# ebu/libear

Measured on AMD Instinct MI355X. Metric: Msamples/s, higher is better.
Workload: dtype f32 io / f16x2-split MFMA, f32 accumulate

## Files before the change

include/earhip.h:

```cpp
#ifndef EARHIP_H
#define EARHIP_H

#include <stddef.h>
#include <stdint.h>

#ifdef __cplusplus
extern "C" {
#endif

#define EARHIP_VERSION 100

#define EARHIP_OK 0
#define EARHIP_INVALID_ARGUMENT 1
#define EARHIP_INTERNAL_ERROR 2
#define EARHIP_DEVICE_ERROR 3
#define EARHIP_NOT_IMPLEMENTED 4
#define EARHIP_UNKNOWN_LAYOUT 5
#define EARHIP_ADM_ERROR 6

int earhip_version(void);
const char *earhip_last_error(void);
int earhip_device_count(int *count);

typedef struct earhip_ctx earhip_ctx;
// ... 97 lines not shown
                          double *elevation, int *is_lfe);
int earhip_layout_channel_ranges(const char *layout, int index, double azimuth_range[2],
                                 double elevation_range[2]);
int earhip_design_decorrelators_for_layout(const char *layout, int without_lfe, float *out);

typedef struct earhip_panner earhip_panner;
int earhip_panner_create(earhip_ctx *ctx, const char *layout, earhip_panner **out);
int earhip_panner_create_positions(earhip_ctx *ctx, const char *layout, int n_channels,
                                   const double *azimuth, const double *elevation,
                                   earhip_panner **out);
int earhip_panner_destroy(earhip_panner *p);
int earhip_panner_num_channels(const earhip_panner *p, int *n_channels);
int earhip_panner_calculate(earhip_panner *p, size_t npos, const double *azimuth,
                            const double *elevation, const double *distance, const double *gain,
                            const double *diffuse, float *direct, float *diffuse_out);
int earhip_panner_calculate_device(earhip_panner *p, size_t npos, const double *azimuth,
                                   const double *elevation, const double *distance,
                                   const double *gain, const double *diffuse, float *direct,
                                   float *diffuse_out);

int earhip_panner_calculate_extent(earhip_panner *p, size_t npos, const double *azimuth,
                                   const double *elevation, const double *distance,
                                   const double *width, const double *height, const double *depth,
                                   const double *gain, const double *diffuse, float *direct,
                                   float *diffuse_out);
int earhip_panner_calculate_extent_device(earhip_panner *p, size_t npos, const double *azimuth,
                                          const double *elevation, const double *distance,
                                          const double *width, const double *height,
                                          const double *depth, const double *gain,
                                          const double *diffuse, float *direct, float *diffuse_out);
int earhip_panner_missed(earhip_panner *p, unsigned *count);

int earhip_hoa_decode_matrix(earhip_ctx *ctx, const char *layout, int n_coef, const int *orders,
                             const int *degrees, const char *normalization, float *out);
int earhip_hoa_decode_matrix_positions(earhip_ctx *ctx, const char *layout, int n_channels,
                                       const double *azimuth, const double *elevation, int n_coef,
                                       const int *orders, const int *degrees,
                                       const char *normalization, float *out);

typedef struct earhip_direct_speakers earhip_direct_speakers;

typedef struct earhip_ds_metadata {
  int n_labels;
  const char *const *labels;
  int cartesian;
  double azimuth, elevation, distance;
  int has_azimuth_min, has_azimuth_max, has_elevation_min, has_elevation_max, has_distance_min,
      has_distance_max;
  double azimuth_min, azimuth_max, elevation_min, elevation_max, distance_min, distance_max;
  int screen_edge_lock_horizontal, screen_edge_lock_vertical;
  int has_low_pass, has_high_pass;
  double low_pass, high_pass;
  const char *audio_pack_format_id;
} earhip_ds_metadata;

int earhip_direct_speakers_create(earhip_ctx *ctx, const char *layout, int n_subst,
                                  const char *const *from, const char *const *to,
                                  earhip_direct_speakers **out);
int earhip_direct_speakers_create_positions(earhip_ctx *ctx, const char *layout, int n_channels,
                                            const double *azimuth, const double *elevation,
                                            int n_subst, const char *const *from,
                                            const char *const *to, earhip_direct_speakers **out);
int earhip_direct_speakers_destroy(earhip_direct_speakers *ds);
int earhip_direct_speakers_num_channels(const earhip_direct_speakers *ds, int *n_channels);
int earhip_direct_speakers_calculate(earhip_direct_speakers *ds, size_t n,
                                     const earhip_ds_metadata *md, float *gains,
                                     int *warnings_out);
int earhip_direct_speakers_missed(earhip_direct_speakers *ds, unsigned *count);

int earhip_conversion_to_polar(size_t n, const double *x, const double *y, const double *z,
                               const double *width, const double *height, const double *depth,
                               double *azimuth, double *elevation, double *distance,
                               double *width_out, double *height_out, double *depth_out);
int earhip_conversion_to_cartesian(size_t n, const double *azimuth, const double *elevation,
                                   const double *distance, const double *width,
                                   const double *height, const double *depth, double *x, double *y,
                                   double *z, double *width_out, double *height_out,
                                   double *depth_out);
int earhip_conversion_to_polar_device(earhip_ctx *ctx, size_t n, const double *x, const double *y,
                                      const double *z, const double *width, const double *height,
                                      const double *depth, double *azimuth, double *elevation,
                                      double *distance, double *width_out, double *height_out,
                                      double *depth_out, int *status);
int earhip_conversion_to_cartesian_device(earhip_ctx *ctx, size_t n, const double *azimuth,
                                          const double *elevation, const double *distance,
                                          const double *width, const double *height,
                                          const double *depth, double *x, double *y, double *z,
                                          double *width_out, double *height_out, double *depth_out,
                                          int *status);

typedef struct earhip_render earhip_render;

typedef struct earhip_render_config {
  int n_objects;
  int n_out;
  int block_size;
  int n_buses;
  const float *decorrelators;
  int n_taps;
  int delay;
  int max_blocks;
} earhip_render_config;

int earhip_render_create(earhip_ctx *ctx, const earhip_render_config *cfg,
                         earhip_render **out);
int earhip_render_destroy(earhip_render *r);
int earhip_render_set_object_points(earhip_render *r, int object, int npoints,
                                    const int64_t *times, const float *direct,
                                    const float *diffuse);
int earhip_render_commit(earhip_render *r);
int earhip_render_scratch_regrows(const earhip_render *r, long *count);
int earhip_render_reset(earhip_render *r, int64_t sample_time);
int earhip_render_process_device(earhip_render *r, size_t nblocks,
                                 const float *in_dev, size_t in_stride,
                                 float *out_dev, size_t out_stride);
int earhip_render_process(earhip_render *r, size_t nblocks, const float *const *in,
                          float *const *out);
typedef enum {
  EARHIP_PCM_S16 = 1,
  EARHIP_PCM_S24 = 2,
  EARHIP_PCM_S32 = 3,
  EARHIP_PCM_F32 = 4
} earhip_pcm_format;
int earhip_render_process_frames(earhip_render *r, size_t nblocks, const void *frames,
                                 earhip_pcm_format fmt, int frame_channels, int first_channel,
                                 float *const *out, int out_interleaved);
int earhip_render_process_frames_device(earhip_render *r, size_t nblocks, const void *frames_dev,
                                        earhip_pcm_format fmt, int frame_channels, int first_channel,
                                        float *out_dev, size_t out_stride, int out_interleaved);
typedef struct earhip_pcm_out {
  earhip_pcm_format format;
  int dither;
  uint32_t seed;
} earhip_pcm_out;
int earhip_render_process_frames_pcm(earhip_render *r, size_t nblocks, const void *frames,
                                     earhip_pcm_format fmt, int frame_channels, int first_channel,
                                     void *out_frames, const earhip_pcm_out *out);
int earhip_render_process_frames_pcm_device(earhip_render *r, size_t nblocks, const void *frames_dev,
                                            earhip_pcm_format fmt, int frame_channels,
                                            int first_channel, void *out_dev, size_t out_frame_bytes,
                                            size_t out_first_byte, const earhip_pcm_out *out);
int earhip_render_output_levels(earhip_render *r, float *peak, uint64_t *clipped, int reset);
int earhip_render_enable_timing(earhip_render *r, int enable);
int earhip_render_get_timing(earhip_render *r, double out[6]);
int earhip_render_gain_kernel(const earhip_render *r, int *kind);
int earhip_render_hinge_standby(earhip_render *r, int *standby);
int earhip_render_hinge_robust(earhip_render *r, int *robust);
int earhip_render_wide_form(earhip_render *r, int *wide);
int earhip_render_last_plan(const earhip_render *r, int out[4]);
int earhip_render_last_list_layout(const earhip_render *r, int *paired);
int earhip_render_last_tail_blocks(const earhip_render *r, int *blocks);
int earhip_render_last_host_chunks(const earhip_render *r, int *chunks);
int earhip_render_scratch_bytes(const earhip_render *r, size_t *bytes);

typedef struct earhip_comm earhip_comm;
int earhip_comm_unique_id(void *id128);
int earhip_comm_create(earhip_ctx *ctx, int rank, int world, const void *id128, earhip_comm **out);
int earhip_comm_destroy(earhip_comm *comm);
int earhip_comm_channel_range(int n_out, int rank, int world, int *padded_rows, int *lo, int *hi);
int earhip_render_exchange_device(earhip_comm *comm, int slot, const float *partial_dev,
                                  float *owned_dev, size_t rows_per_rank, size_t row_stride);
int earhip_comm_gather_device(earhip_comm *comm, int slot, const float *owned_dev, float *full_dev,
                              size_t rows_per_rank, size_t row_stride, int root);
int earhip_comm_wait(earhip_comm *comm, int slot);
int earhip_comm_last_exchange_ms(earhip_comm *comm, int slot, double *ms);
int earhip_comm_info(earhip_comm *comm, int info[4]);
int earhip_comm_link_probe(earhip_comm *comm, size_t bytes, int shift, int reps, double *GBps);

#ifdef __cplusplus
}
#endif
#endif
```

libear_amd/capi.py:

```python
import ctypes as C
import os

import numpy as np

from .build import lib_path

f32p = C.POINTER(C.c_float)
i64p = C.POINTER(C.c_int64)
pp_f32 = C.POINTER(f32p)

OK, INVALID_ARGUMENT, INTERNAL_ERROR, DEVICE_ERROR, NOT_IMPLEMENTED, UNKNOWN_LAYOUT, ADM_ERROR = 0, 1, 2, 3, 4, 5, 6


class EarHipError(Exception):
    def __init__(self, code, msg):
        super().__init__(msg)
        self.code = code


class InvalidArgument(EarHipError, ValueError):
    """maps to ear::invalid_argument"""


class InternalError(EarHipError, RuntimeError):
# ... 686 lines not shown
        self.h = C.c_void_p()
        check(load().earhip_render_create(ctx.h, C.byref(cfg), C.byref(self.h)))

    def set_object_points(self, obj, times, direct, diffuse=None):
        t = np.ascontiguousarray(times, dtype=np.int64)
        d = _f32(direct).reshape(len(t), self.N)
        f = _f32(diffuse).reshape(len(t), self.N) if diffuse is not None else None
        check(load().earhip_render_set_object_points(self.h, obj, len(t), _ptr(t, i64p), _ptr(d),
                                                     _ptr(f) if f is not None else None))

    def commit(self):
        check(load().earhip_render_commit(self.h))

    def reset(self, sample_time=0):
        check(load().earhip_render_reset(self.h, C.c_int64(sample_time)))

    def process(self, x):
        x = _f32(x).reshape(self.M, -1)
        nblocks = x.shape[1] // self.B
        assert nblocks * self.B == x.shape[1]
        out = np.empty((self.N, x.shape[1]), np.float32)
        check(load().earhip_render_process(self.h, C.c_size_t(nblocks), _chan_ptrs(x), _chan_ptrs(out)))
        return out

    def process_into(self, x, out):
        assert x.dtype == np.float32 and out.dtype == np.float32 and x.flags["C_CONTIGUOUS"] and out.flags["C_CONTIGUOUS"]
        nblocks = x.shape[1] // self.B
        assert x.shape == (self.M, nblocks * self.B) and out.shape == (self.N, nblocks * self.B)
        check(load().earhip_render_process(self.h, C.c_size_t(nblocks), _chan_ptrs(x), _chan_ptrs(out)))
        return out

    def process_device(self, nblocks, in_ptr, in_stride, out_ptr, out_stride):
        check(load().earhip_render_process_device(self.h, C.c_size_t(nblocks), C.c_void_p(in_ptr),
                                                  C.c_size_t(in_stride), C.c_void_p(out_ptr),
                                                  C.c_size_t(out_stride)))

    def _frames_shape(self, x, fmt):
        code, dtype, cols = pcm_format(fmt)
        assert x.dtype == dtype and x.ndim == 2 and x.flags["C_CONTIGUOUS"], (x.dtype, dtype, x.shape)
        assert x.shape[1] % cols == 0
        frames, channels = x.shape[0], x.shape[1] // cols
        nblocks = frames // self.B
        assert nblocks * self.B == frames, "frames must be whole blocks"
        return code, nblocks, channels

    def process_frames(self, x, fmt, first_channel=0, interleaved_out=False):
        x = np.ascontiguousarray(x)
        frames = x.shape[0]
        out = np.empty((frames, self.N) if interleaved_out else (self.N, frames), np.float32)
        return self.process_frames_into(x, out, fmt, first_channel, interleaved_out)

    def process_frames_into(self, x, out, fmt, first_channel=0, interleaved_out=False):
        code, nblocks, channels = self._frames_shape(x, fmt)
        frames = nblocks * self.B
        assert out.dtype == np.float32 and out.flags["C_CONTIGUOUS"]
        assert out.shape == ((frames, self.N) if interleaved_out else (self.N, frames)), out.shape
        ptrs = (f32p * 1)(_ptr(out)) if interleaved_out else _chan_ptrs(out)
        check(load().earhip_render_process_frames(self.h, C.c_size_t(nblocks), C.c_void_p(x.ctypes.data), C.c_int(code),
                                                  C.c_int(channels), C.c_int(first_channel), ptrs, int(bool(interleaved_out))))
        return out

    def process_frames_device(self, nblocks, frames_ptr, fmt, frame_channels, first_channel, out_ptr, out_stride,
                              interleaved_out=False):
        code = pcm_format(fmt)[0] if isinstance(fmt, str) else int(fmt)
        check(load().earhip_render_process_frames_device(self.h, C.c_size_t(nblocks), C.c_void_p(frames_ptr), C.c_int(code),
                                                         C.c_int(frame_channels), C.c_int(first_channel), C.c_void_p(out_ptr),
                                                         C.c_size_t(out_stride), int(bool(interleaved_out))))

    def process_frames_pcm(self, x, fmt, first_channel=0, out_fmt="s16", dither=False, seed=0):
        x = np.ascontiguousarray(x)
        _, dtype, cols = pcm_format(out_fmt)
        out = np.empty((x.shape[0], self.N * cols), dtype)
        return self.process_frames_pcm_into(x, out, fmt, first_channel, out_fmt, dither, seed)

    def process_frames_pcm_into(self, x, out, fmt, first_channel=0, out_fmt="s16", dither=False, seed=0):
        code, nblocks, channels = self._frames_shape(x, fmt)
        ocode, dtype, cols = pcm_format(out_fmt)
        assert out.dtype == dtype and out.flags["C_CONTIGUOUS"] and out.shape == (nblocks * self.B, self.N * cols), out.shape
        spec = PcmOut(ocode, int(dither), int(seed) & 0xFFFFFFFF)
        check(load().earhip_render_process_frames_pcm(self.h, C.c_size_t(nblocks), C.c_void_p(x.ctypes.data), C.c_int(code),
                                                      C.c_int(channels), C.c_int(first_channel), C.c_void_p(out.ctypes.data),
                                                      C.byref(spec)))
        return out

    def process_frames_pcm_device(self, nblocks, frames_ptr, fmt, frame_channels, first_channel, out_ptr, out_frame_bytes,
                                  out_first_byte=0, out_fmt="s16", dither=False, seed=0):
        code = pcm_format(fmt)[0] if isinstance(fmt, str) else int(fmt)
        ocode = pcm_format(out_fmt)[0] if isinstance(out_fmt, str) else int(out_fmt)
        spec = PcmOut(ocode, int(dither), int(seed) & 0xFFFFFFFF)
        check(load().earhip_render_process_frames_pcm_device(self.h, C.c_size_t(nblocks), C.c_void_p(frames_ptr), C.c_int(code),
                                                             C.c_int(frame_channels), C.c_int(first_channel), C.c_void_p(out_ptr),
                                                             C.c_size_t(out_frame_bytes), C.c_size_t(out_first_byte),
                                                             C.byref(spec)))

    def output_levels(self, reset=False):
        peak, clipped = np.zeros(self.N, np.float32), np.zeros(self.N, np.uint64)
        check(load().earhip_render_output_levels(self.h, _ptr(peak), C.c_void_p(clipped.ctypes.data), int(bool(reset))))
        return peak, clipped

    def enable_timing(self, on=True):
        check(load().earhip_render_enable_timing(self.h, int(on)))

    def get_timing(self):
        out = (C.c_double * 6)()
        check(load().earhip_render_get_timing(self.h, out))
        return {"gain_mix_ms": out[0], "gain_mix_launches": out[1], "decor_ms": out[2],
                "decor_launches": out[3], "prep_ms": out[4], "prep_launches": out[5]}

    def gain_kernel(self):
        kind = C.c_int(-1)
        check(load().earhip_render_gain_kernel(self.h, C.byref(kind)))
        return kind.value

    def hinge_standby(self):
        flag = C.c_int(0)
        check(load().earhip_render_hinge_standby(self.h, C.byref(flag)))
        return bool(flag.value)

    def hinge_robust(self):
        flag = C.c_int(0)
        check(load().earhip_render_hinge_robust(self.h, C.byref(flag)))
        return bool(flag.value)

    def wide_form(self):
        flag = C.c_int(1)
        check(load().earhip_render_wide_form(self.h, C.byref(flag)))
        return None if flag.value < 0 else bool(flag.value)

    def scratch_bytes(self):
        v = C.c_size_t(0)
        check(load().earhip_render_scratch_bytes(self.h, C.byref(v)))
        return v.value

    def scratch_regrows(self):
        v = C.c_long(0)
        check(load().earhip_render_scratch_regrows(self.h, C.byref(v)))
        return v.value

    def last_tail_blocks(self):
        v = C.c_int(0)
        check(load().earhip_render_last_tail_blocks(self.h, C.byref(v)))
        return v.value

    def last_host_chunks(self):
        v = C.c_int(0)
        check(load().earhip_render_last_host_chunks(self.h, C.byref(v)))
        return v.value

    def last_list_layout(self):
        v = C.c_int(0)
        check(load().earhip_render_last_list_layout(self.h, C.byref(v)))
        return None if v.value < 0 else bool(v.value)

    def last_plan(self):
        out = (C.c_int * 4)()
        check(load().earhip_render_last_plan(self.h, out))
        return {"kernel": out[0], "tile": out[1], "ntiles": out[2], "gsplit": out[3]}

    def close(self):
        if self.h:
            load().earhip_render_destroy(self.h)
            self.h = C.c_void_p()
```

libear_amd/csrc/api_core.hip:

```cpp
#include <cctype>
#include <cerrno>
#include <cmath>
#include <cstdlib>
#include <string>
#include <memory>
#include <mutex>

#include "common.h"
#include "curves.h"
#include "gain_kernels.h"
#include "gain_mfma.h"
#include "gain_h2.h"
#include "gain_h2_t1.h"
#include "gain_p2.h"
#include "gain_hg.h"
#include "gain_f32g.h"

namespace earhip {

static_assert(kSplitTile == 256, "MixLaunch::tile() and tiles_aligned(256, ...) assume the 4-wave tile");

static thread_local std::string g_last_error;
void set_last_error(const std::string &msg) { g_last_error = msg; }

size_t mix_lds_bytes(const ColumnPlan &cp, const MixLaunch &ml) {
  if (ml.wsplit <= 1 || ml.split || ml.pieces || ml.hinge) return 0;
  if (ml.mfma) return (size_t)cp.mgroups * ml.tpw * cp.nct * 16 * ml.tile() * sizeof(float);
  return (size_t)cp.ngroups * cp.nout * ml.tile() * sizeof(float);
}

template <int NCT, int NRT>
static void launch_mfma_t(const GainMixParams &P, dim3 grid, dim3 block, size_t lds,
                          hipStream_t s) {
  hipLaunchKernelGGL((k_gain_mix_mfma<NCT, NRT>), grid, block, lds, s, P);
}

template <int NOUT, int SPL, bool STRICT>
static void launch_mix_t(const GainMixParams &P, dim3 grid, dim3 block, size_t lds,
                         hipStream_t s) {
  hipLaunchKernelGGL((k_gain_mix<NOUT, SPL, STRICT>), grid, block, lds, s, P);
}

void launch_gain_mix(earhip_ctx *ctx, const CurveSet &cs, const MixLaunch &ml, bool strict,
                     int64_t t_call, int nsamples, const float *in_dev, size_t in_stride,
                     float *out_dev, size_t out_stride, size_t part_stride, SegDesc *desc,
                     hipEvent_t *ev) {
  const ColumnPlan &cp = cs.plan();
  const PointStore ps = cs.device();
  const int M = cs.M();
  const bool slots = ml.mfma && !ml.split && !ml.pieces && !ml.hinge && !ml.f32grid;
  if (slots && M > kMaxSlotObjects) fail_internal("slot lists address objects with 16 bits");
  if (ev) EARHIP_HIP(hipEventRecord(ev[0], ctx->stream));
  const bool fused_prep = slots && (size_t)ps.npoints <= (size_t)8 * M;
  LevelProbe probe;
  unsigned *level_cur = nullptr, *level_next = nullptr;
  unsigned *wide_cur = nullptr, *wide_next = nullptr;
  unsigned *gate = nullptr;
  ctx->last_gate_idx = -1;
  ctx->last_wide_idx = -1;
  unsigned *const record = ctx->record_slot;
  ctx->record_slot = nullptr;
  const bool hg_robust = ml.hinge && ctx->get(OPT_HG_ROBUST, 1) != 0;
  if ((ml.split || ml.pieces || ml.hinge) && ctx->x_scale_auto && in_stride % 4 == 0 && ((uintptr_t)in_dev & 15) == 0) {
    if (!ctx->level.p) ctx->level.alloc_zero(4, ctx->stream), ctx->lazy_allocs++;
    level_cur = ctx->level.p + ctx->level_idx;
    level_next = ctx->level.p + (ctx->level_idx ^ 1);
    if ((size_t)ml.ntiles * ml.gsplit >= 2 * (size_t)ctx->num_cus) wide_cur = ctx->level.p + 2 + ctx->level_idx;
    wide_next = ctx->level.p + 2 + (ctx->level_idx ^ 1);
    gate = ctx->level.p + 2 + ctx->level_idx;
    ctx->last_gate_idx = ml.hinge ? ctx->level_idx : -1;
    ctx->last_hinge_robust = hg_robust;
    ctx->last_wide_idx = wide_cur ? ctx->level_idx : -1;
    ctx->level_idx ^= 1;
    if (ctx->obj_level_cap < M) {
      EARHIP_HIP(hipStreamSynchronize(ctx->stream));
      ctx->obj_level_cap = M + M / 2 + 64;
      ctx->obj_level.alloc_zero(2 * (size_t)ctx->obj_level_cap, ctx->stream);
      ctx->lazy_allocs++;
    }
    probe.obj_level = ctx->obj_level.p;
    probe.level = level_cur;
    const int probe_runs = [&] {
      const int v = ctx->get(OPT_PROBE_RUNS);
      return v >= 1 && v <= 64 && (v & (v - 1)) == 0 ? v : 16;
    }();
    hipLaunchKernelGGL(k_level_probe, dim3((M + kProbeObjects - 1) / kProbeObjects), dim3(64 * kProbeObjects), 0, ctx->stream, in_dev,
                       in_stride, nsamples, M, level_cur, ctx->obj_level.p, ctx->obj_level_cap, probe_runs);
  }
  PieceLists pl;
  pl.pieces = reinterpret_cast<Piece *>(desc);
  pl.M = M;
  pl.paired = ml.paired ? 1 : 0;
  const int ptile = ml.hinge ? 64 * ml.pw : ml.tile();
  const int pnt = ml.hinge ? (nsamples + ptile - 1) / ptile : ml.ntiles;
  pl.slots = cs.piece_cap(ptile, ml.paired);
  pl.count = reinterpret_cast<int *>(pl.pieces + (size_t)pl.cap() * pnt);
  pl.ovf = pl.count + (size_t)8 * pnt;
  unsigned *slow_cur = nullptr, *slow_next = nullptr;
  if (ml.split) {
    if (ctx->tile_slow_cap < (size_t)ml.ntiles) {
      EARHIP_HIP(hipStreamSynchronize(ctx->stream));
      ctx->tile_slow_cap = std::max<size_t>(2 * (size_t)ml.ntiles, 1024);
      ctx->tile_slow.alloc_zero(2 * ctx->tile_slow_cap, ctx->stream);
      ctx->lazy_allocs++;
    }
    slow_cur = ctx->tile_slow.p + (size_t)ctx->tile_slow_idx * ctx->tile_slow_cap;
    slow_next = ctx->tile_slow.p + (size_t)(ctx->tile_slow_idx ^ 1) * ctx->tile_slow_cap;
    ctx->tile_slow_idx ^= 1;
  }
  HingeLists hl = hinge_lists(desc, M, ml.ntiles);
  if (ml.hinge) {
    if (M > kMaxHingeCached || (ml.tile() != 256 && ml.tile() != 512)) fail_internal("hinge lists: object count or tile out of range");
    if (!ps.kink_row0) fail_internal("hinge kernel: the curve set has no kink rows");
    if (!hinge_addressable(M, in_stride, nsamples, (size_t)ps.kink_row0 + ps.rows, ps.row)) fail_internal("hinge kernel: buffers beyond its 32-bit offsets");
    unsigned *obj_lv = probe.obj_level;
    if (gate) hipLaunchKernelGGL(k_hinge_gate, dim3((M + 255) / 256), dim3(256), 0, ctx->stream, obj_lv, ctx->obj_level_cap, M, level_cur, gate, wide_cur != nullptr, hg_robust);
    int tpw = 1;
    const size_t cached_max = std::min((size_t)kMaxHingeCached, ctx->hinge_build_lds / sizeof(HingeCached));
    if ((size_t)M > cached_max) fail_internal("hinge lists: more objects than the builder's LDS holds on this device");
    while (tpw < 8 && ml.ntiles / (2 * tpw) >= ctx->num_cus && (size_t)M * (2 * tpw) <= cached_max) tpw *= 2;
    if (ctx->has(OPT_HBUILD_TPW)) {
      const int v = ctx->get(OPT_HBUILD_TPW);
      if ((v == 1 || v == 2 || v == 4 || v == 8) && (size_t)M * v <= cached_max) tpw = v;
    }
    const HingeCached *stage = nullptr;
    if (ctx->get(OPT_BUILD_2K, 0) != 0) {
      HingeCached *st = reinterpret_cast<HingeCached *>(desc) + hinge_units((size_t)M, (size_t)ml.ntiles);
      stage = st;
      const dim3 cgrid((ml.ntiles + 63) / 64, (M + kClassifyObjects - 1) / kClassifyObjects);
      if (ml.tile() == 256)
        hipLaunchKernelGGL((k_hinge_classify<4>), cgrid, dim3(64 * kClassifyObjects), 0, ctx->stream, ps, M, ml.ntiles, t_call, t_call + nsamples, st,
                           obj_lv, level_cur, hg_robust ? nullptr : gate, hg_robust ? gate : nullptr);
      else
        hipLaunchKernelGGL((k_hinge_classify<8>), cgrid, dim3(64 * kClassifyObjects), 0, ctx->stream, ps, M, ml.ntiles, t_call, t_call + nsamples, st,
                           obj_lv, level_cur, hg_robust ? nullptr : gate, hg_robust ? gate : nullptr);
      if (!ctx->has(OPT_HBUILD_TPW)) {
        tpw = 1;
        while (tpw < 8 && ml.ntiles / (2 * tpw) >= 2 * ctx->num_cus) tpw *= 2;
      }
    }
    const dim3 bgrid((ml.ntiles + tpw - 1) / tpw);
    const size_t lds = stage ? 0 : sizeof(HingeCached) * (size_t)M * tpw;
#define EARHIP_HBUILD_ONE(T_, NW_)                                                                                    \
  hipLaunchKernelGGL((k_hinge_build<T_, NW_>), bgrid, dim3(kHingeBuildThreads), lds, ctx->stream, ps, M, ml.ntiles, t_call, \
                     t_call + nsamples, hl, obj_lv, level_cur, hg_robust ? nullptr : gate, hg_robust ? gate : nullptr, stage);
#define EARHIP_HBUILD_CASE(T_)                                                                                        \
  if (tpw == T_) {                                                                                                    \
    if (ml.tile() == 256) EARHIP_HBUILD_ONE(T_, 4)                                                                    \
    else EARHIP_HBUILD_ONE(T_, 8)                                                                                     \
  }
    EARHIP_HBUILD_CASE(1) EARHIP_HBUILD_CASE(2) EARHIP_HBUILD_CASE(4) EARHIP_HBUILD_CASE(8)
#undef EARHIP_HBUILD_CASE
#undef EARHIP_HBUILD_ONE
  }
  const bool one_pass = ml.pieces || ml.hinge;
  if (ml.pieces || (ml.hinge && gate && !hg_robust)) {
    if (M > kMaxPieceObjects || ptile > kPieceMaxTile) fail_internal("piece lists: object index or tile out of range");
    unsigned *obj_lv = probe.obj_level;
    int tpw = 1;
    while (tpw < 8 && pnt / (2 * tpw) >= ctx->num_cus) tpw *= 2;
    if (ctx->has(OPT_BUILD_TPW)) {
      const int v = ctx->get(OPT_BUILD_TPW);
      if (v == 1 || v == 2 || v == 4 || v == 8) tpw = v;
    }
    const dim3 bgrid((pnt + tpw - 1) / tpw);
    PairRec *stage = nullptr;
    if (ctx->has(OPT_BUILD_2K) ? ctx->get(OPT_BUILD_2K) != 0 : ml.paired) {
      stage = reinterpret_cast<PairRec *>(desc) + piece_units((size_t)M, (size_t)pnt, (size_t)pl.slots);
      hipLaunchKernelGGL(k_piece_classify, dim3((pnt + 63) / 64, (M + kClassifyObjects - 1) / kClassifyObjects), dim3(64 * kClassifyObjects), 0,
                         ctx->stream, ps, M, pnt, ptile, t_call, t_call + nsamples, pl.paired, stage, obj_lv, level_cur,
                         ml.hinge ? gate : nullptr);
    }
#define EARHIP_BUILD_CASE(T_)                                                                                          \
  if (tpw == T_)                                                                                                       \
    hipLaunchKernelGGL(k_piece_build<T_>, bgrid, dim3(kBuildThreads), 0, ctx->stream, ps, M, pnt, ptile, t_call, \
                       t_call + nsamples, pl, obj_lv, level_cur, ml.hinge ? gate : nullptr, ctx->obj_level_cap, wide_cur, stage);
    EARHIP_BUILD_CASE(1) EARHIP_BUILD_CASE(2) EARHIP_BUILD_CASE(4) EARHIP_BUILD_CASE(8)
#undef EARHIP_BUILD_CASE
  }
  if (!fused_prep && !one_pass) {
    const dim3 ogrid((M + 15) / 16);
    QuietMark qm;
    if (probe.obj_level) {
      qm.obj_level = probe.obj_level, qm.cap = ctx->obj_level_cap, qm.level = level_cur;
      qm.wide = ml.split ? wide_cur : nullptr;
    }
    if (ml.ntiles >= 2048)
      hipLaunchKernelGGL(k_seg_prep<4>, dim3((ml.ntiles + 63) / 64, ogrid.x), dim3(256), 0, ctx->stream, ps, M,
                         ml.ntiles, ml.tile(), t_call, t_call + nsamples, desc, qm, slow_cur);
    else
      hipLaunchKernelGGL(k_seg_prep<2>, dim3((ml.ntiles + 31) / 32, ogrid.x), dim3(256), 0, ctx->stream, ps, M,
                         ml.ntiles, ml.tile(), t_call, t_call + nsamples, desc, qm, slow_cur);
  }
  SlotLists sl;
  sl.slots = reinterpret_cast<Slot *>(desc + (size_t)M * ml.ntiles);
  sl.count = reinterpret_cast<int *>(sl.slots + (size_t)kTileSlots * M * ml.ntiles);
  sl.ovf = sl.count + (size_t)4 * ml.ntiles;
  sl.M = M;
  if (slots)
    hipLaunchKernelGGL(k_slot_list, dim3(ml.ntiles), dim3(256), 0, ctx->stream, ps, M, ml.tile(),
                       t_call, t_call + nsamples, fused_prep ? nullptr : desc, sl);
  if (ev) EARHIP_HIP(hipEventRecord(ev[1], ctx->stream));
  GainMixParams P;
  P.mode_word = gate;
  P.record = gate ? record : nullptr;
  P.sl = sl;
  P.in = in_dev;
  P.in_stride = in_stride;
  P.out = out_dev;
  P.out_stride = out_stride;
  P.part_stride = part_stride;
  P.desc = desc;
  P.ps = ps;
  P.t_call = t_call;
  P.nsamples = nsamples;
  P.ntiles = ml.ntiles;
  P.M = M;
  P.ncols = cs.ncols();
  P.ngroups = ml.mfma ? cp.mgroups : cp.ngroups;
  P.wsplit = ml.wsplit;
  P.tiles_per_wg = ml.mfma ? ml.tpw : 1;
  P.vec_ok = (in_stride % 4 == 0 && out_stride % 4 == 0 && part_stride % 4 == 0 &&
              ((uintptr_t)in_dev & 15) == 0 && ((uintptr_t)out_dev & 15) == 0)
                 ? 1
                 : 0;
  const dim3 grid(ml.mfma ? (ml.ntiles + ml.tpw - 1) / ml.tpw : ml.ntiles, ml.gsplit,
                  ml.mfma ? cp.mnz : cp.nz);
  const dim3 block(64 * P.ngroups * P.tiles_per_wg * ml.wsplit);
  const size_t lds = mix_lds_bytes(cp, ml);
  if (ev) EARHIP_HIP(hipEventRecord(ev[2], ctx->stream));
  bool launched = false;
  if (ml.hinge) {
    const dim3 bgrid(ml.ntiles, ml.gsplit, cp.mnz * cp.mgroups);
    const float xs = std::ldexp(1.0f, ctx->x_scale_log2);
    const float *gs = cs.column_scales();
#define EARHIP_HG_LAUNCH(NCT_, NW_)                                                                                  \
  hipLaunchKernelGGL((k_gain_mix_hg<NCT_, NW_>), bgrid, dim3(64 * NW_), 0, ctx->stream, P, hl, xs, gs, level_cur,     \
                     level_next, wide_cur, wide_next, hg_robust ? nullptr : gate, hg_robust ? gate : nullptr);
#define EARHIP_HG_CASE(NCT_)                                                                                          \
  if (cp.nct == NCT_) {                                                                                               \
    if (ml.tile() == 256) EARHIP_HG_LAUNCH(NCT_, 4)                                                                   \
    else EARHIP_HG_LAUNCH(NCT_, 8)                                                                                    \
  }
    EARHIP_HG_CASE(1) EARHIP_HG_CASE(2) EARHIP_HG_CASE(3)
#undef EARHIP_HG_CASE
#undef EARHIP_HG_LAUNCH
    launched = true;
  }
  if (ml.pieces || (ml.hinge && gate && !hg_robust)) {
    int wgs = std::max(8, (ctx->num_cus * (ml.pw == 4 ? 2 : 1) / std::max(1, ml.gsplit * cp.mnz * cp.mgroups)) & ~7);
    if (ctx->has(OPT_P2_WGS)) wgs = ctx->get(OPT_P2_WGS) > 0 ? ctx->get(OPT_P2_WGS) : pnt;
    if (!p2_persistent(cp.nct, ml.pw, ml.paired)) wgs = pnt;
    const dim3 bgrid(std::min(pnt, wgs), ml.gsplit, cp.mnz * cp.mgroups);
    const float xs = std::ldexp(1.0f, ctx->x_scale_log2);
    const float *gs = cs.column_scales();
#define EARHIP_P2_LAUNCH(NCT_, NW_, PR_)                                                                             \
  hipLaunchKernelGGL((k_gain_mix_p2<NCT_, NW_, PR_>), bgrid, dim3(64 * NW_), 0, ctx->stream, P, pl, xs, gs,         \
                     level_cur, level_next, wide_cur, wide_next, ml.hinge ? gate : nullptr, pnt);
#define EARHIP_P2_CASE(NCT_, PR_)                                                                                   \
  if (cp.nct == NCT_ && ml.paired == PR_) {                                                                         \
    if (ml.pw == 4) EARHIP_P2_LAUNCH(NCT_, 4, PR_)                                                                  \
    else EARHIP_P2_LAUNCH(NCT_, 8, PR_)                                                                             \
  }
    EARHIP_P2_CASE(1, false) EARHIP_P2_CASE(2, false) EARHIP_P2_CASE(3, false)
    EARHIP_P2_CASE(1, true) EARHIP_P2_CASE(2, true) EARHIP_P2_CASE(3, true)
#undef EARHIP_P2_CASE
#undef EARHIP_P2_LAUNCH
    launched = true;
  }
  if (ml.f32grid) {
    if (nsamples % kF32GridTile != 0) fail_internal("f32 grid kernel: the call is not whole tiles");
    const dim3 bgrid(ml.ntiles, ml.gsplit, cp.mnz * cp.mgroups);
#define EARHIP_F32G_CASE(NCT_)                                                                       \
  if (cp.nct == NCT_) hipLaunchKernelGGL((k_gain_mix_f32g<NCT_>), bgrid, dim3(512), 0, ctx->stream, P, ps.zero_row);
    EARHIP_F32G_CASE(1) EARHIP_F32G_CASE(2) EARHIP_F32G_CASE(3)
#undef EARHIP_F32G_CASE
    launched = true;
  }
  if (ml.split) {
    const int per_cu = ml.tile() == 512 ? 1 : (cp.nct == 1 ? 3 : 2);
    int wgs = std::max(8, (ctx->num_cus * per_cu / std::max(1, ml.gsplit * cp.mnz * cp.mgroups)) & ~7);
    if (ctx->has(OPT_H2_WGS)) wgs = std::max(1, ctx->get(OPT_H2_WGS));
    wgs = std::max(wgs, ((ml.ntiles + 63) / 64 + 7) & ~7);
    P.tile_runs = ctx->has(OPT_H2_RUNS) ? (ctx->get(OPT_H2_RUNS) != 0) : 0;
    if (!h2_persistent(cp.nct, ml.tile() == 512 ? 8 : 4)) wgs = ml.ntiles;
    const dim3 bgrid(std::min(ml.ntiles, wgs), ml.gsplit, cp.mnz * cp.mgroups);
    const float xs = std::ldexp(1.0f, ctx->x_scale_log2);
    const float *gs = cs.column_scales();
    const bool two_launches = ctx->get(OPT_H2_PAIR, 0) != 0;
#define EARHIP_H2_LAUNCH(NCT_, NW_, WIDE_)                                                                          \
  hipLaunchKernelGGL((k_gain_mix_h2<NCT_, NW_, WIDE_>), bgrid, dim3(64 * NW_), 0, ctx->stream, P, ps.zero_row, xs,  \
                     gs, level_cur, level_next, slow_cur, slow_next, wide_cur, wide_next);
#define EARHIP_H2T1_LAUNCH(NCT_, NW_, WIDE_)                                                                        \
  hipLaunchKernelGGL((k_gain_mix_h2_t1<NCT_, NW_, WIDE_>), bgrid, dim3(64 * NW_), 0, ctx->stream, P, ps.zero_row, xs, \
                     gs, level_cur, level_next, slow_cur, slow_next, wide_cur, wide_next);
#define EARHIP_H2_CASE(NCT_)                                                                                        \
  if (cp.nct == NCT_) {                                                                                             \
    if (ml.tile() == 512) {                                                                                         \
      if (wide_cur && !two_launches) EARHIP_H2_LAUNCH(NCT_, 8, 2)                                                   \
      else {                                                                                                        \
        if (wide_cur) EARHIP_H2_LAUNCH(NCT_, 8, 0)                                                                  \
        EARHIP_H2_LAUNCH(NCT_, 8, 1)                                                                                \
      }                                                                                                             \
    } else if (NCT_ == 1) {                                                                                         \
      if (wide_cur) EARHIP_H2_LAUNCH(1, 4, 0)                                                                       \
      EARHIP_H2_LAUNCH(1, 4, 1)                                                                                     \
    } else {                                                                                                        \
      if (wide_cur) EARHIP_H2T1_LAUNCH(NCT_, 4, false)                                                              \
      EARHIP_H2T1_LAUNCH(NCT_, 4, true)                                                                             \
    }                                                                                                               \
  }
    EARHIP_H2_CASE(1) EARHIP_H2_CASE(2) EARHIP_H2_CASE(3)
#undef EARHIP_H2_CASE
#undef EARHIP_H2_LAUNCH
#undef EARHIP_H2T1_LAUNCH
    launched = true;
  }
#define EARHIP_MIX_CASE(NOUT_, SPL_, STRICT_)                                   \
  if (cp.nout == NOUT_ && ml.spl == SPL_ && strict == STRICT_) {                 \
    launch_mix_t<NOUT_, SPL_, STRICT_>(P, grid, block, lds, ctx->stream);        \
    launched = true;                                                             \
  }
#define EARHIP_MFMA_CASE(NCT_, NRT_)                                            \
  if (slots && cp.nct == NCT_ && ml.nrt == NRT_) {                                          \
    launch_mfma_t<NCT_, NRT_>(P, grid, block, lds, ctx->stream);                 \
    launched = true;                                                             \
  }
  EARHIP_MFMA_CASE(1, 8) EARHIP_MFMA_CASE(2, 8) EARHIP_MFMA_CASE(3, 8)
  EARHIP_MFMA_CASE(1, 4) EARHIP_MFMA_CASE(2, 4) EARHIP_MFMA_CASE(3, 4)
#undef EARHIP_MFMA_CASE
  if (!ml.mfma && !launched) {
  EARHIP_MIX_CASE(8, 4, false) EARHIP_MIX_CASE(8, 4, true)
  EARHIP_MIX_CASE(16, 4, false) EARHIP_MIX_CASE(16, 4, true)
  EARHIP_MIX_CASE(24, 4, false) EARHIP_MIX_CASE(24, 4, true)
  EARHIP_MIX_CASE(8, 2, false) EARHIP_MIX_CASE(8, 2, true)
  EARHIP_MIX_CASE(16, 2, false) EARHIP_MIX_CASE(16, 2, true)
  EARHIP_MIX_CASE(24, 2, false) EARHIP_MIX_CASE(24, 2, true)
  }
#undef EARHIP_MIX_CASE
  if (!launched) fail_internal("no gain_mix instantiation for this column plan");
  if (ev) EARHIP_HIP(hipEventRecord(ev[3], ctx->stream));
  EARHIP_HIP(hipGetLastError());
}

void reserve_call_words(earhip_ctx *ctx, int M, size_t max_samples) {
  if (!ctx->level.p) ctx->level.alloc_zero(4, ctx->stream);
  const size_t ntiles = (max_samples + 255) / 256;
  const bool grow_obj = ctx->obj_level_cap < M, grow_tiles = ctx->tile_slow_cap < ntiles;
  if (grow_obj || grow_tiles) EARHIP_HIP(hipStreamSynchronize(ctx->stream));
  if (grow_obj) {
    ctx->obj_level_cap = M + M / 2 + 64;
    ctx->obj_level.alloc_zero(2 * (size_t)ctx->obj_level_cap, ctx->stream);
  }
  if (grow_tiles) {
    ctx->tile_slow_cap = std::max<size_t>(ntiles + ntiles / 4, 1024);
    ctx->tile_slow.alloc_zero(2 * ctx->tile_slow_cap, ctx->stream);
    ctx->tile_slow_idx = 0;
  }
}

size_t hinge_build_allow_lds(const hipDeviceProp_t &prop) {
  const size_t want = 128 * 1024, dflt = 64 * 1024;
  const size_t device_max = std::max((size_t)prop.sharedMemPerBlock, (size_t)prop.maxSharedMemoryPerMultiProcessor);
  size_t ask = std::min(want, device_max > 4096 ? device_max - 4096 : dflt);
  if (ask <= dflt) return dflt;
  bool ok = true;
#define EARHIP_HBUILD_ATTR(T_, NW_)                                                                       \
  ok = ok && hipFuncSetAttribute(reinterpret_cast<const void *>(&k_hinge_build<T_, NW_>),                 \
                                 hipFuncAttributeMaxDynamicSharedMemorySize, (int)ask) == hipSuccess;
  EARHIP_HBUILD_ATTR(1, 4) EARHIP_HBUILD_ATTR(2, 4) EARHIP_HBUILD_ATTR(4, 4) EARHIP_HBUILD_ATTR(8, 4)
  EARHIP_HBUILD_ATTR(1, 8) EARHIP_HBUILD_ATTR(2, 8) EARHIP_HBUILD_ATTR(4, 8) EARHIP_HBUILD_ATTR(8, 8)
#undef EARHIP_HBUILD_ATTR
  if (!ok) (void)hipGetLastError();
  return ok ? ask : dflt;
}

struct GainStage {
  earhip_ctx *ctx;
  int n_in, n_out;
  CurveSet curves;
  DevBuf<SegDesc> desc;
  DevBuf<float> parts;
  std::vector<float> rows;
  bool force_ramp;
  GainStage(earhip_ctx *c, int ni, int no, bool ramp = false)
      : ctx(c), n_in(ni), n_out(no), curves(ni, no, 1, ramp), force_ramp(ramp) {}

  void run_device(int64_t t_call, int nsamples, const float *in_dev, size_t in_stride,
                  float *out_dev, size_t out_stride) {
    curves.commit(ctx);
    const bool strict = ctx->strict || n_in == 1 || force_ramp;
    MixLaunch ml = plan_mix(ctx, curves.plan(), n_in, nsamples, strict, 32,
                            curves.aligned_tile(t_call), curves.ramp_share(), curves.gain_scale(), curves.point_density_all(),
                            curves.pair_waste(256), curves.pair_waste(512), curves.hinge_exact_share(in_stride, (size_t)nsamples), false,
                            curves.deltas_per_pair(256));
    if (ml.hinge) curves.ensure_kinks(ctx);
    desc.reserve(scratch_units(curves, ml, n_in));
    if (ml.gsplit == 1) {
      launch_gain_mix(ctx, curves, ml, strict, t_call, nsamples, in_dev, in_stride, out_dev,
                      out_stride, 0, desc.p, nullptr);
    } else {
      const size_t row_stride = ((size_t)nsamples + 3) & ~(size_t)3;
      const size_t part_stride = row_stride * n_out;
      parts.reserve(part_stride * ml.gsplit);
      launch_gain_mix(ctx, curves, ml, strict, t_call, nsamples, in_dev, in_stride, parts.p,
                      row_stride, part_stride, desc.p, nullptr);
      hipLaunchKernelGGL(k_sum_parts, dim3((nsamples + 255) / 256, n_out), dim3(256), 0,
                         ctx->stream, parts.p, part_stride, ml.gsplit, row_stride, n_out,
                         nsamples, out_dev, out_stride);
      EARHIP_HIP(hipGetLastError());
    }
  }

  void run_host(int64_t t_call, const float *const *in, float *const *out, int64_t r0,
                int64_t r1) {
    const int n = (int)(r1 - r0);
    if (n <= 0) return;
    const size_t stride = ((size_t)n + 3) & ~(size_t)3;
    ctx->pin_in.reserve(stride * n_in);
    ctx->pin_out.reserve(stride * n_out);
    ctx->dev_in.reserve(stride * n_in);
    ctx->dev_out.reserve(stride * n_out);
    for (int c = 0; c < n_in; c++)
      std::memcpy(ctx->pin_in.p + c * stride, in[c] + r0, sizeof(float) * n);
    EARHIP_HIP(hipMemcpyAsync(ctx->dev_in.p, ctx->pin_in.p, sizeof(float) * stride * n_in,
                              hipMemcpyHostToDevice, ctx->stream));
    run_device(t_call, n, ctx->dev_in.p, stride, ctx->dev_out.p, stride);
    EARHIP_HIP(hipMemcpyAsync(ctx->pin_out.p, ctx->dev_out.p, sizeof(float) * stride * n_out,
                              hipMemcpyDeviceToHost, ctx->stream));
    EARHIP_HIP(hipStreamSynchronize(ctx->stream));
    for (int c = 0; c < n_out; c++)
      std::memcpy(out[c] + r0, ctx->pin_out.p + c * stride, sizeof(float) * n);
  }
};

}

using namespace earhip;

static const char *const kOptNames[OPT_COUNT] = {
    "SPL", "MFMA", "XSCALE", "WAVES", "TPW", "NRT", "H2_TILE", "H2_WGS", "H2_RUNS", "P2_TILE", "P2_PAIRS", "P2_WGS", "HINGE", "HG_TILE", "HBUILD_TPW",
    "BUILD_TPW", "K2_WG", "K2_OWN_BLOCK", "RUN", "GSPLIT", "PROBE_RUNS", "BLOCK_GROUPS", "DEBUG_TIMING", "TAILCUT", "HOST_CHUNK_MB", "HOST_THREADS", "HG_ROBUST", "BUILD_2K", "HOST_BIND", "HOST_NT", "HOST_FIRST", "H2_PAIR"};

static int parse_option_value(const std::string &key, const char *text) {
  char *end = nullptr;
  errno = 0;
  const long v = std::strtol(text, &end, 10);
  while (end && *end && std::isspace((unsigned char)*end)) end++;
  if (end == text || (end && *end) || errno == ERANGE || v < -(1L << 30) || v > (1L << 30))
    fail_invalid("option '" + key + "': '" + std::string(text) + "' is not an integer");
  return (int)v;
}

void earhip_ctx::apply_options() {
  spl = 4, use_mfma = 3, x_scale_log2 = 14, x_scale_auto = true, max_waves = 4, tiles_per_wg = 4, tiles_per_wg_forced = false, nrt = 8;
  if (has(OPT_SPL) && (get(OPT_SPL) == 2 || get(OPT_SPL) == 4)) spl = get(OPT_SPL);
  if (has(OPT_MFMA)) use_mfma = get(OPT_MFMA);
  if (has(OPT_XSCALE) && get(OPT_XSCALE) >= -64 && get(OPT_XSCALE) <= 64)
    x_scale_log2 = get(OPT_XSCALE), x_scale_auto = false;
  if (has(OPT_WAVES) && get(OPT_WAVES) >= 1 && get(OPT_WAVES) <= 8) max_waves = get(OPT_WAVES);
  if (has(OPT_TPW) && get(OPT_TPW) >= 1 && get(OPT_TPW) <= 8) tiles_per_wg = get(OPT_TPW), tiles_per_wg_forced = true;
  if (has(OPT_NRT) && (get(OPT_NRT) == 4 || get(OPT_NRT) == 8)) nrt = get(OPT_NRT);
}

struct earhip_gain_interp {
  std::unique_ptr<GainStage> stage;
};

struct PolicyCache {
  std::vector<std::unique_ptr<GainStage>> stages;
  GainStage *get(earhip_ctx *ctx, int n_in, int n_out, bool ramp) {
    for (auto &s : stages)
      if (s->n_in == n_in && s->n_out == n_out && s->force_ramp == ramp) return s.get();
    stages.emplace_back(new GainStage(ctx, n_in, n_out, ramp));
    return stages.back().get();
  }
};
static std::vector<std::pair<earhip_ctx *, std::unique_ptr<PolicyCache>>> g_policy;
static std::mutex g_policy_mutex;
static PolicyCache *policy_cache(earhip_ctx *ctx) {
  std::lock_guard<std::mutex> lock(g_policy_mutex);
  for (auto &p : g_policy)
    if (p.first == ctx) return p.second.get();
  g_policy.emplace_back(ctx, std::unique_ptr<PolicyCache>(new PolicyCache));
  return g_policy.back().second.get();
}

static __global__ void k_clock_probe(unsigned long long *out) {
  out[0] = clock64();
  out[1] = wall_clock64();
}

static __global__ void __launch_bounds__(256) k_read_linear(const f32x4 *in, float *out, size_t n4) {
  f32x4 acc = {0.0f, 0.0f, 0.0f, 0.0f};
  size_t i = (size_t)blockIdx.x * 256 + threadIdx.x;
  const size_t step = (size_t)gridDim.x * 256;
  for (; i + 3 * step < n4; i += 4 * step) {
    const f32x4 a = __builtin_nontemporal_load(in + i), b = __builtin_nontemporal_load(in + i + step);
    const f32x4 c = __builtin_nontemporal_load(in + i + 2 * step), d = __builtin_nontemporal_load(in + i + 3 * step);
    acc += (a + b) + (c + d);
  }
  for (; i < n4; i += step) acc += __builtin_nontemporal_load(in + i);
  if (acc[0] + acc[1] + acc[2] + acc[3] == 123.456f) out[0] = 1.0f;
}
static __global__ void __launch_bounds__(256) k_read_rows(const float *in, float *out, int rows, size_t stride) {
  constexpr int DEPTH = 4;
  const int lane = threadIdx.x & 63, w = threadIdx.x >> 6, li = lane & 15, kg = lane >> 4;
  const float *base = in + (size_t)blockIdx.x * 256 + w * 64 + li * 4;
  auto row = [&](int r) { return base + (size_t)min(r, rows - 1) * stride; };
  f32x4 acc = {0.0f, 0.0f, 0.0f, 0.0f};
  f32x4 ring[DEPTH][8];
#pragma unroll
  for (int d = 0; d < DEPTH; d++)
#pragma unroll
    for (int q = 0; q < 8; q++)
      ring[d][q] = __builtin_nontemporal_load((const f32x4 *)row(d * 32 + kg * 8 + q));
  for (int r0 = 0; r0 < rows; r0 += 32 * DEPTH) {
#pragma unroll
    for (int d = 0; d < DEPTH; d++) {
#pragma unroll
      for (int q = 0; q < 8; q++) acc += ring[d][q];
      const int rn = r0 + 32 * DEPTH + d * 32;
      if (rn < rows)
#pragma unroll
        for (int q = 0; q < 8; q++)
          ring[d][q] = __builtin_nontemporal_load((const f32x4 *)row(rn + kg * 8 + q));
    }
  }
  if (acc[0] + acc[1] + acc[2] + acc[3] == 123.456f) out[0] = 1.0f;
}

extern "C" {

int earhip_debug_read_bandwidth(earhip_ctx *ctx, const float *in_dev, size_t rows, size_t stride,
                                size_t nsamples, int reps, double ms[2]) {
  return guarded([&] {
    require(ctx != nullptr && in_dev != nullptr && ms != nullptr, "NULL argument");
    require(rows >= 1 && rows < ((size_t)1 << 24) && reps >= 1 && reps <= 1000, "rows / reps out of range");
    require(stride % 256 == 0 && nsamples % 256 == 0 && nsamples >= 256 && nsamples <= stride &&
                ((uintptr_t)in_dev & 15) == 0,
            "buffer must be 16-byte aligned with stride and nsamples multiples of 256");
    ctx->use();
    if (!ctx->level.p) ctx->level.alloc_zero(4, ctx->stream);
    float *sink = reinterpret_cast<float *>(ctx->level.p);
    hipEvent_t e[4];
    for (auto &x : e) EARHIP_HIP(hipEventCreate(&x));
    const size_t n4 = rows * stride / 4;
    const unsigned lin_blocks = (unsigned)std::min<size_t>((n4 + 255) / 256, (size_t)ctx->num_cus * 32);
    auto linear = [&] {
      hipLaunchKernelGGL(k_read_linear, dim3(lin_blocks), dim3(256), 0, ctx->stream,
                         reinterpret_cast<const f32x4 *>(in_dev), sink, n4);
    };
    auto pattern = [&] {
      hipLaunchKernelGGL(k_read_rows, dim3((unsigned)(nsamples / 256)), dim3(256), 0, ctx->stream, in_dev, sink,
                         (int)rows, stride);
    };
    linear();
    EARHIP_HIP(hipEventRecord(e[0], ctx->stream));
    for (int i = 0; i < reps; i++) linear();
    EARHIP_HIP(hipEventRecord(e[1], ctx->stream));
    pattern();
    EARHIP_HIP(hipEventRecord(e[2], ctx->stream));
    for (int i = 0; i < reps; i++) pattern();
    EARHIP_HIP(hipEventRecord(e[3], ctx->stream));
    EARHIP_HIP(hipGetLastError());
    EARHIP_HIP(hipEventSynchronize(e[3]));
    float t = 0.0f;
    EARHIP_HIP(hipEventElapsedTime(&t, e[0], e[1]));
    ms[0] = (double)t / reps;
    EARHIP_HIP(hipEventElapsedTime(&t, e[2], e[3]));
    ms[1] = (double)t / reps;
    for (auto &x : e) (void)hipEventDestroy(x);
  });
}

int earhip_debug_copy_bandwidth(earhip_ctx *ctx, void *host, size_t bytes, int reps, double ms[2]) {
  return guarded([&] {
    require(ctx != nullptr && host != nullptr && ms != nullptr, "NULL argument");
    require(bytes >= 4 && reps >= 1 && reps <= 1000, "bytes / reps out of range");
    ctx->use();
    DevBuf<char> dev;
    dev.alloc(bytes);
    hipEvent_t e[2];
    for (auto &x : e) EARHIP_HIP(hipEventCreate(&x));
    for (int dir = 0; dir < 2; dir++) {
      auto copy = [&] {
        if (dir == 0) EARHIP_HIP(hipMemcpyAsync(dev.p, host, bytes, hipMemcpyHostToDevice, ctx->stream));
        else EARHIP_HIP(hipMemcpyAsync(host, dev.p, bytes, hipMemcpyDeviceToHost, ctx->stream));
      };
      copy();
      EARHIP_HIP(hipEventRecord(e[0], ctx->stream));
      for (int i = 0; i < reps; i++) copy();
      EARHIP_HIP(hipEventRecord(e[1], ctx->stream));
      EARHIP_HIP(hipEventSynchronize(e[1]));
      float t = 0.0f;
// ... 336 lines not shown
```

libear_amd/csrc/api_render.hip:

```cpp
#include <cmath>
#include <cstdlib>
#include <atomic>
#include <chrono>
#include <condition_variable>
#include <memory>
#include <mutex>
#include <thread>
#include <vector>


#include "common.h"
#include "curves.h"
#include "host_gather.h"
#include "pcm_kernels.h"
#include "pcm_out_kernels.h"
#include "fft_kernels.h"
#include "render_kernels.h"

using namespace earhip;

namespace earhip {
std::vector<cf> make_twiddles(int L) {
  std::vector<cf> tw(L);
  const double pi = 3.14159265358979323846264338327950288;
// ... 218 lines not shown
      (void)hipEventDestroy(ev_in[i]);
      (void)hipEventDestroy(ev_k[i]);
      (void)hipEventDestroy(ev_out[i]);
    }
    (void)hipStreamDestroy(in);
    (void)hipStreamDestroy(out);
  }
};

struct earhip_render {
  earhip_ctx *ctx = nullptr;
  int M = 0, N = 0, B = 0, K = 1, D = 0, T = 0;
  int Bk = 0, Lk = 0;
  int NP = 1;
  std::unique_ptr<CurveSet> curves;
  int64_t t = 0;
  int last_plan[3] = {0, 0, 0};
  int last_paired = -1;
  size_t last_scratch_bytes = 0;
  long scratch_regrows = 0;
  DevBuf<unsigned> rec;
  bool last_gated = false;
  bool last_device_form = false;
  bool last_hg_robust = false;
  int last_kind = -1;
  int run_len = 11;
  bool run_len_set = false;

  DevBuf<SegDesc> desc;
  DevBuf<float> bus;
  int max_gsplit = 1;
  DevBuf<cf> H, tw;
  DevBuf<float> tail[2], dly[2], hist[2];
  DevBuf<float> ztail, zdly, zhist;
  bool fresh = true;
  int cur = 0;
  DevBuf<float> d_in, d_out;
  PinBuf<float> p_in, p_out;
  std::unique_ptr<GatherPool> gather;
  StreamPipe pipe;
  int last_host_chunks = 0;
  PinBuf<unsigned char> p_bytes;
  DevBuf<unsigned char> d_bytes;
  DevBuf<float> d_ilv, d_rows, d_rows_out;
  DevBuf<unsigned char> d_pcm;
  PinBuf<unsigned char> p_pcm;
  DevBuf<unsigned> d_peak;
  DevBuf<unsigned long long> d_clip;
  bool timing = false;
  bool last_timed = false;
  int timing_every = 1;
  long timing_calls = 0;
  hipEvent_t ev[6] = {nullptr, nullptr, nullptr, nullptr, nullptr, nullptr};
  struct Pending { hipEvent_t e[6]; bool has_k2; bool continues; };
  std::vector<Pending> pending;
  std::vector<hipEvent_t> pool;
  double acc_ms[3] = {0, 0, 0};
  double acc_n[3] = {0, 0, 0};

  ~earhip_render() {
    for (auto &p : pending)
      for (auto e : p.e)
        if (e) (void)hipEventDestroy(e);
    for (auto e : pool) (void)hipEventDestroy(e);
  }

  hipEvent_t get_event() {
    if (!pool.empty()) {
      hipEvent_t e = pool.back();
      pool.pop_back();
      return e;
    }
    hipEvent_t e;
    EARHIP_HIP(hipEventCreate(&e));
    return e;
  }

  void drain_timing() {
    EARHIP_HIP(hipStreamSynchronize(ctx->stream));
    for (auto &p : pending) {
      float ms = 0;
      const double one = p.continues ? 0.0 : 1.0;
      EARHIP_HIP(hipEventElapsedTime(&ms, p.e[0], p.e[1]));
      acc_ms[2] += ms; acc_n[2] += one;
      EARHIP_HIP(hipEventElapsedTime(&ms, p.e[2], p.e[3]));
      acc_ms[0] += ms; acc_n[0] += one;
      if (p.has_k2) {
        EARHIP_HIP(hipEventElapsedTime(&ms, p.e[4], p.e[5]));
        acc_ms[1] += ms; acc_n[1] += one;
      }
      for (auto e : p.e)
        if (e) pool.push_back(e);
    }
    pending.clear();
  }

  size_t direct_stride(const float *const *ch, int count, size_t n) const {
    if (ctx->host_ranges.empty() || count < 1) return 0;
    const uintptr_t a0 = (uintptr_t)ch[0];
    const uintptr_t step = count > 1 ? (uintptr_t)ch[1] - a0 : sizeof(float) * n;
    if ((a0 & 15) != 0 || step % 16 != 0 || step < sizeof(float) * n || step > ((uintptr_t)1 << 40)) return 0;
    for (int c = 1; c < count; c++)
      if ((uintptr_t)ch[c] - (uintptr_t)ch[c - 1] != step) return 0;
    return ctx->host_reachable(ch[0], step * (count - 1) + sizeof(float) * n) ? (size_t)(step / sizeof(float)) : 0;
  }

  void reserve_levels() {
    if (d_peak.p) return;
    EARHIP_HIP(hipStreamSynchronize(ctx->stream));
    d_peak.alloc_zero((size_t)kLevelSlots * N, ctx->stream);
    d_clip.alloc_zero((size_t)kLevelSlots * N, ctx->stream);
  }
  void zero_levels() {
    if (!d_peak.p) return;
    EARHIP_HIP(hipMemsetAsync(d_peak.p, 0, sizeof(unsigned) * kLevelSlots * N, ctx->stream));
    EARHIP_HIP(hipMemsetAsync(d_clip.p, 0, sizeof(unsigned long long) * kLevelSlots * N, ctx->stream));
  }
  void reserve_pcm_out(size_t bytes, bool pinned) {
    reserve_levels();
    d_pcm.reserve(bytes);
    if (pinned) p_pcm.reserve(bytes);
  }

  HostChunkPlan host_plan(size_t nblocks, bool direct) const {
    return plan_host_chunks(nblocks, B, M, direct, ctx->has(OPT_HOST_CHUNK_MB), ctx->get(OPT_HOST_CHUNK_MB), ctx->get(OPT_HOST_FIRST, 0));
  }

  MixLaunch plan_call(size_t nblocks, size_t in_stride) {
    const int nsamples = (int)(nblocks * (size_t)B);
    MixLaunch ml = plan_mix(ctx, curves->plan(), M, nsamples, ctx->strict, max_gsplit, curves->aligned_tile(t),
                            curves->ramp_share(), curves->gain_scale(), curves->point_density_all(), curves->pair_waste(256), curves->pair_waste(512),
                            curves->hinge_exact_share(in_stride, (size_t)nsamples), curves->tiles_aligned(kF32GridTile, t),
                            curves->deltas_per_pair(256));
    const size_t bus_stride = ((size_t)nsamples + 3) & ~(size_t)3;
    while (ml.gsplit > 1 && bus_stride * K * N * ml.gsplit > bus.n) ml.gsplit /= 2;
    return ml;
  }

  size_t last_in_stride = 0;
  void reserve_for_curves() {
    size_t need = 0;
    bool hinge = false;
    const size_t lens[3] = {(size_t)T, (size_t)std::max(1, T / 2), (size_t)1};
    for (size_t nb : lens) {
      const MixLaunch ml = plan_call(nb, last_in_stride ? last_in_stride : nb * (size_t)B);
      need = std::max(need, scratch_units(*curves, ml, M));
      hinge = hinge || ml.hinge;
    }
    if (hinge) curves->ensure_kinks(ctx);
    if (need > desc.n) {
      EARHIP_HIP(hipStreamSynchronize(ctx->stream));
      desc.reserve(need + need / 4);
    }
  }

  int resident_workgroups(const MixLaunch &ml) const {
    if (!(ml.split || ml.pieces || ml.hinge)) return 0;
    return ctx->num_cus * (ml.tile() >= 512 ? 1 : 2);
  }

  void process_device(size_t nblocks, const float *in_dev, size_t in_stride, float *out_dev, size_t out_stride) {
    MixLaunch whole;
    bool have_plan = false;
    if (!ctx->strict && ctx->get(OPT_TAILCUT, 1) != 0 && nblocks >= 2) {
      last_in_stride = in_stride;
      if (curves->dirty()) {
        curves->commit(ctx);
        reserve_for_curves();
      }
      const MixLaunch ml = whole = plan_call(nblocks, in_stride);
      have_plan = true;
      const int W = resident_workgroups(ml);
      if (W > 0 && ml.gsplit == 1 && ml.ntiles > W) {
        const size_t tile = (size_t)ml.tile();
        const size_t full = (size_t)ml.ntiles / (size_t)W, rest = (size_t)ml.ntiles % (size_t)W;
        const size_t main_samples = full * (size_t)W * tile;
        const size_t eighths = (size_t)std::min(std::max(ctx->get(OPT_TAILCUT, 2), 0), 7);
        if (rest > 0 && rest <= (size_t)W * eighths / 8 && main_samples % (size_t)B == 0) {
          const size_t main_blocks = main_samples / (size_t)B;
          process_span(main_blocks, in_dev, in_stride, out_dev, out_stride, false);
          const int kind = last_kind, plan3[3] = {last_plan[0], last_plan[1], last_plan[2]};
          const size_t scratch = last_scratch_bytes;
          const bool gated = last_gated, device_form = last_device_form, hg_robust = last_hg_robust;
          const int paired = last_paired;
          process_span(nblocks - main_blocks, in_dev + main_samples, in_stride, out_dev + main_samples, out_stride, true);
          last_kind = kind;
          last_gated = gated, last_device_form = device_form, last_paired = paired, last_hg_robust = hg_robust;
          for (int i = 0; i < 3; i++) last_plan[i] = plan3[i];
          last_scratch_bytes = scratch;
          last_tail_blocks = (int)(nblocks - main_blocks);
          return;
        }
      }
    }
    last_tail_blocks = 0;
    process_span(nblocks, in_dev, in_stride, out_dev, out_stride, false, have_plan ? &whole : nullptr);
  }
  int last_tail_blocks = 0;

  void process_span(size_t nblocks, const float *in_dev, size_t in_stride, float *out_dev,
                    size_t out_stride, bool continues, const MixLaunch *planned = nullptr) {
    const int nsamples = (int)(nblocks * (size_t)B);
    last_in_stride = in_stride;
    if (curves->dirty()) {
      curves->commit(ctx);
      reserve_for_curves();
    }
    const bool strict = ctx->strict;
    MixLaunch ml = planned ? *planned : plan_call(nblocks, in_stride);
    if (ml.hinge) curves->ensure_kinks(ctx);

    last_kind = ml.f32grid ? 2 : ml.hinge ? 5 : ml.pieces ? 4 : ml.split ? 3 : ml.mfma ? 1 : 0;
    {
      const size_t need = scratch_units(*curves, ml, M);
      if (need > desc.n) {
        EARHIP_HIP(hipStreamSynchronize(ctx->stream));
        desc.reserve(need + need / 2);
        scratch_regrows++;
      }
      last_scratch_bytes = need * 16;
    }
    const size_t bus_stride = ((size_t)nsamples + 3) & ~(size_t)3;
    const size_t part_stride = bus_stride * K * N;
    if (part_stride * ml.gsplit > bus.n) fail_internal("bus buffer too small for this launch plan");
    last_paired = (ml.pieces || ml.hinge) ? (ml.paired ? 1 : 0) : -1;
    last_plan[0] = ml.tile();
    last_plan[1] = ml.ntiles;
    last_plan[2] = ml.gsplit;
    Pending pd;
    hipEvent_t *evp = nullptr;
    const bool timed = timing && (continues ? last_timed : (timing_calls++ % timing_every) == 0);
    last_timed = timed;
    if (timed) {
      for (int i = 0; i < 6; i++) pd.e[i] = get_event();
      pd.has_k2 = K == 2;
      pd.continues = continues;
      evp = pd.e;
    }
    const long lazy_before = ctx->lazy_allocs;
    ctx->record_slot = rec.p + (continues ? 1 : 0);
    if (K == 1) {
      if (ml.gsplit == 1) {
        launch_gain_mix(ctx, *curves, ml, strict, t, nsamples, in_dev, in_stride, out_dev,
                        out_stride, 0, desc.p, evp);
      } else {
        launch_gain_mix(ctx, *curves, ml, strict, t, nsamples, in_dev, in_stride, bus.p,
                        bus_stride, part_stride, desc.p, evp);
        hipLaunchKernelGGL(k_sum_parts, dim3((nsamples + 255) / 256, N), dim3(256), 0,
                           ctx->stream, bus.p, part_stride, ml.gsplit, bus_stride, N, nsamples,
                           out_dev, out_stride);
        EARHIP_HIP(hipGetLastError());
      }
    } else {
      launch_gain_mix(ctx, *curves, ml, strict, t, nsamples, in_dev, in_stride, bus.p,
                      bus_stride, part_stride, desc.p, evp);
      DecorParams P;
      P.bus = bus.p;
      P.bus_stride = bus_stride;
      P.part_stride = part_stride;
      P.nparts = ml.gsplit;
      const bool wave_k2 = Lk == 1024 && NP == 1 && !ctx->get(OPT_K2_WG);
      const int kblocks = (int)(nblocks * (size_t)(B / Bk));
      if (wave_k2 && ml.gsplit > 1) {
        if (evp) EARHIP_HIP(hipEventRecord(evp[4], ctx->stream));
        hipLaunchKernelGGL(k_sum_parts, dim3((nsamples + 255) / 256, K * N), dim3(256), 0, ctx->stream, bus.p,
                           part_stride, ml.gsplit, bus_stride, K * N, nsamples, bus.p, bus_stride);
        EARHIP_HIP(hipGetLastError());
        P.nparts = 1;
      }
      P.out = out_dev;
      P.out_stride = out_stride;
      P.tw = tw.p;
      P.dly_in = fresh ? zdly.p : dly[cur].p;
      P.dly_out = dly[cur ^ 1].p;
      P.N = N;
      P.T = kblocks;
      const int R = wave_k2 && !run_len_set ? wave_run_len(kblocks, N, ctx->num_cus) : run_len;
      P.R = R;
      P.D = D;
      P.hist_len = (NP - 1) * Bk;
      P.hist_in = fresh ? zhist.p : hist[cur].p;
      P.hist_out = hist[cur ^ 1].p;
      const dim3 grid((unsigned)((kblocks + R - 1) / R), N);
      if (evp && P.nparts == ml.gsplit) EARHIP_HIP(hipEventRecord(evp[4], ctx->stream));
      for (int part = 0; part < NP; part++) {
        P.H = H.p + (size_t)part * N * Lk;
        P.tail_in = (fresh ? ztail.p : tail[cur].p) + (fresh ? 0 : (size_t)part * N * Bk);
        P.tail_out = tail[cur ^ 1].p + (size_t)part * N * Bk;
        P.shift = part * Bk;
        P.accumulate = part > 0 ? 1 : 0;
        if (wave_k2) {
          hipLaunchKernelGGL(k_decorrelate_wave, dim3((grid.x + kDecorWaves - 1) / kDecorWaves, grid.y), dim3(64 * kDecorWaves),
                             0, ctx->stream, P);
          EARHIP_HIP(hipGetLastError());
        } else {
          launch_decor(Lk, P, grid, ctx->stream, true);
        }
      }
      if (evp) EARHIP_HIP(hipEventRecord(evp[5], ctx->stream));
      cur ^= 1;
      fresh = false;
    }
    if (timed) pending.push_back(pd);
    last_gated = ctx->last_gate_idx >= 0;
    last_device_form = ctx->last_wide_idx >= 0;
    last_hg_robust = last_gated && ctx->last_hinge_robust;
    if (ctx->lazy_allocs != lazy_before) scratch_regrows++;
    t += nsamples;
  }
};

extern "C" {

int earhip_render_create(earhip_ctx *ctx, const earhip_render_config *cfg, earhip_render **out) {
  return guarded([&] {
    require(ctx != nullptr && cfg != nullptr && out != nullptr, "NULL argument");
    require(cfg->n_objects >= 1 && cfg->n_out >= 1, "n_objects and n_out must be >= 1");
    require(cfg->n_buses == 1 || cfg->n_buses == 2, "n_buses must be 1 or 2");
    FftShape shape;
    require(cfg->block_size >= 16 && cfg->block_size <= 4096 && fft_make_shape(2 * cfg->block_size, &shape),
            "block_size must be in [16, 4096]");
    require(cfg->max_blocks >= 1, "max_blocks must be >= 1");
    require((int64_t)cfg->max_blocks * cfg->block_size < ((int64_t)1 << 30),
            "max_blocks * block_size too large");
    require(cfg->delay >= 0, "delay must be >= 0");
    if (cfg->n_buses == 2) {
      require(cfg->decorrelators != nullptr && cfg->n_taps >= 1,
              "n_buses == 2 needs decorrelator filters");
      require((cfg->n_taps + cfg->block_size - 1) / cfg->block_size <= 64,
              "decorrelator filters of more than 64 blocks are not supported by the fused render "
              "(use BlockConvolver)");
    } else {
      require(cfg->delay == 0, "delay needs n_buses == 2");
    }
    ctx->use();
    std::unique_ptr<earhip_render> r(new earhip_render);
    r->ctx = ctx;
    r->M = cfg->n_objects;
    r->N = cfg->n_out;
    r->B = cfg->block_size;
    r->K = cfg->n_buses;
    r->D = cfg->delay;
    r->T = cfg->max_blocks;
    r->Bk = r->B;
    if (r->K == 2 && r->B > 512 && r->B % 512 == 0 && cfg->n_taps <= 512 && !ctx->get(OPT_K2_OWN_BLOCK)) r->Bk = 512;
    r->Lk = 2 * r->Bk;
    if (r->Lk == 2048) r->run_len = 7;
    if (ctx->has(OPT_RUN)) {
      const int v = ctx->get(OPT_RUN);
      if (v >= 1 && v <= 255) r->run_len = v | 1, r->run_len_set = true;
    }
    r->curves.reset(new CurveSet(r->M, r->K * r->N, r->K, false));
    const size_t max_samples = (size_t)r->T * r->B;
    reserve_call_words(ctx, r->M, max_samples);
    r->rec.alloc_zero(2, ctx->stream);
    const size_t min_tile = (size_t)std::min(16 * ctx->nrt, std::min(64 * ctx->spl, 256));
    const size_t max_tiles = (max_samples + min_tile - 1) / min_tile;
    r->desc.alloc((size_t)r->M * ((max_samples + 255) / 256) + 1);
    (void)max_tiles;
    r->max_gsplit = 16;
    if (ctx->has(OPT_GSPLIT)) {
      const int v = ctx->get(OPT_GSPLIT);
      if (v >= 1 && v <= 32) r->max_gsplit = v;
    }
    r->bus.alloc_zero((size_t)r->K * r->N * bus_samples_bound(ctx, max_samples, r->max_gsplit), ctx->stream);
    if (r->K == 2) {
      const auto tw = make_twiddles(r->Lk);
      r->tw.alloc(r->Lk);
      EARHIP_HIP(hipMemcpy(r->tw.p, tw.data(), sizeof(cf) * r->Lk, hipMemcpyHostToDevice));
      r->NP = (cfg->n_taps + r->Bk - 1) / r->Bk;
      const size_t rows = (size_t)r->NP * r->N;
      std::vector<float> parts(rows * r->Bk, 0.0f);
      for (int n = 0; n < r->N; n++)
        for (int t = 0; t < cfg->n_taps; t++)
          parts[((size_t)(t / r->Bk) * r->N + n) * r->Bk + t % r->Bk] = cfg->decorrelators[(size_t)n * cfg->n_taps + t];
      DevBuf<float> taps;
      taps.alloc(parts.size());
      EARHIP_HIP(hipMemcpy(taps.p, parts.data(), sizeof(float) * parts.size(), hipMemcpyHostToDevice));
      r->H.alloc(rows * r->Lk);
      launch_spectrum(r->Lk, taps.p, r->Bk, r->Bk, r->tw.p, r->H.p, (int)rows, ctx->stream);
      EARHIP_HIP(hipStreamSynchronize(ctx->stream));
      std::vector<cf> h(rows * r->Lk);
      EARHIP_HIP(hipMemcpy(h.data(), r->H.p, sizeof(cf) * h.size(), hipMemcpyDeviceToHost));
      for (size_t n = 0; n < rows; n++) {
        cf *hn = h.data() + n * r->Lk;
        hn[0].y = 0.0f;
        hn[r->Bk].y = 0.0f;
        for (int k = 1; k < r->Bk; k++) hn[r->Lk - k] = cf_conj(hn[k]);
      }
      EARHIP_HIP(hipMemcpy(r->H.p, h.data(), sizeof(cf) * h.size(), hipMemcpyHostToDevice));
      const size_t hist_n = (size_t)r->N * std::max((r->NP - 1) * r->Bk, 1);
      for (int i = 0; i < 2; i++) {
        r->tail[i].alloc_zero(rows * r->Bk, ctx->stream);
        r->dly[i].alloc_zero((size_t)r->N * std::max(r->D, 1), ctx->stream);
        r->hist[i].alloc_zero(hist_n, ctx->stream);
        if (i == 0) {
          r->ztail.alloc_zero((size_t)r->N * r->Bk, ctx->stream);
          r->zdly.alloc_zero((size_t)r->N * std::max(r->D, 1), ctx->stream);
          r->zhist.alloc_zero(hist_n, ctx->stream);
        }
      }
    }
    EARHIP_HIP(hipStreamSynchronize(ctx->stream));
    *out = r.release();
  });
}

int earhip_render_destroy(earhip_render *r) {
// ... 465 lines not shown
}

int earhip_render_output_levels(earhip_render *r, float *peak, uint64_t *clipped, int reset) {
  return guarded([&] {
    require(r != nullptr, "render must not be NULL");
    require(peak != nullptr && clipped != nullptr, "peak and clipped must not be NULL");
    earhip_ctx *ctx = r->ctx;
    ctx->use();
    EARHIP_HIP(hipStreamSynchronize(ctx->stream));
    if (!r->d_peak.p) {
      for (int c = 0; c < r->N; c++) peak[c] = 0.f, clipped[c] = 0;
      return;
    }
    const size_t cnt = (size_t)kLevelSlots * r->N;
    std::vector<unsigned> pk(cnt);
    std::vector<unsigned long long> cl(cnt);
    EARHIP_HIP(hipMemcpy(pk.data(), r->d_peak.p, sizeof(unsigned) * cnt, hipMemcpyDeviceToHost));
    EARHIP_HIP(hipMemcpy(cl.data(), r->d_clip.p, sizeof(unsigned long long) * cnt, hipMemcpyDeviceToHost));
    for (int c = 0; c < r->N; c++) {
      unsigned m = 0;
      uint64_t sum = 0;
      for (int k = 0; k < kLevelSlots; k++) m = std::max(m, pk[(size_t)k * r->N + c]), sum += cl[(size_t)k * r->N + c];
      std::memcpy(&peak[c], &m, sizeof(float));
      clipped[c] = sum;
    }
    if (reset) r->zero_levels();
  });
}

int earhip_debug_k2_prof(earhip_ctx *ctx, unsigned long long *out64) {
  return guarded([&] {
    require(ctx != nullptr && out64 != nullptr, "NULL argument");
#ifdef EARHIP_K2_PROF
    ctx->use();
    EARHIP_HIP(hipStreamSynchronize(ctx->stream));
    EARHIP_HIP(hipMemcpyFromSymbol(out64, HIP_SYMBOL(g_k2_prof), sizeof(unsigned long long) * 64));
#else
    fail_invalid("this build has no K2 phase stamps (-DEARHIP_K2_PROF)");
#endif
  });
}

int earhip_render_enable_timing(earhip_render *r, int enable) {
  return guarded([&] {
    require(r != nullptr, "render must not be NULL");
    r->ctx->use();
    if (r->timing) r->drain_timing();
    r->timing = enable != 0;
    r->timing_every = enable > 1 ? enable : 1;
    r->timing_calls = 0;
    for (int i = 0; i < 3; i++) r->acc_ms[i] = r->acc_n[i] = 0;
  });
}

int earhip_render_get_timing(earhip_render *r, double out[6]) {
  return guarded([&] {
    require(r != nullptr && out != nullptr, "NULL argument");
    r->ctx->use();
    r->drain_timing();
    out[0] = r->acc_ms[0]; out[1] = r->acc_n[0];
    out[2] = r->acc_ms[1]; out[3] = r->acc_n[1];
    out[4] = r->acc_ms[2]; out[5] = r->acc_n[2];
  });
}

int earhip_render_gain_kernel(const earhip_render *r, int *kind) {
  return guarded([&] {
    require(r != nullptr && kind != nullptr, "NULL argument");
    *kind = r->last_kind;
  });
}

int earhip_render_hinge_standby(earhip_render *r, int *standby) {
  return guarded([&] {
    require(r != nullptr && standby != nullptr, "NULL argument");
    *standby = 0;
    earhip_ctx *ctx = r->ctx;
    if (r->last_kind != 5 || !r->last_gated || r->last_hg_robust) return;
    ctx->use();
    unsigned word = 0;
    EARHIP_HIP(hipMemcpyAsync(&word, r->rec.p, sizeof(word), hipMemcpyDeviceToHost, ctx->stream));
    EARHIP_HIP(hipStreamSynchronize(ctx->stream));
    if (!(word & kModeRecorded)) fail_internal("no gain kernel recorded the call's mode word");
    *standby = (word & kGateHingeUnsafe) ? 1 : 0;
  });
}

int earhip_render_hinge_robust(earhip_render *r, int *robust) {
  return guarded([&] {
    require(r != nullptr && robust != nullptr, "NULL argument");
    *robust = 0;
    earhip_ctx *ctx = r->ctx;
    if (r->last_kind != 5 || !r->last_hg_robust) return;
    ctx->use();
    unsigned word = 0;
    EARHIP_HIP(hipMemcpyAsync(&word, r->rec.p, sizeof(word), hipMemcpyDeviceToHost, ctx->stream));
    EARHIP_HIP(hipStreamSynchronize(ctx->stream));
    if (!(word & kModeRecorded)) fail_internal("no gain kernel recorded the call's mode word");
    *robust = hinge_span_exceeded(word, r->M) ? 1 : 0;
  });
}

int earhip_render_wide_form(earhip_render *r, int *wide) {
  return guarded([&] {
    require(r != nullptr && wide != nullptr, "NULL argument");
    *wide = 1;
    earhip_ctx *ctx = r->ctx;
    if (r->last_kind < 3) *wide = -1;
    if (r->last_kind < 3 || !r->last_device_form) return;
    ctx->use();
    unsigned word = 0;
    EARHIP_HIP(hipMemcpyAsync(&word, r->rec.p, sizeof(word), hipMemcpyDeviceToHost, ctx->stream));
    EARHIP_HIP(hipStreamSynchronize(ctx->stream));
    if (!(word & kModeRecorded)) fail_internal("no gain kernel recorded the call's mode word");
    *wide = (word & 1u) ? 1 : 0;
  });
}

int earhip_render_scratch_bytes(const earhip_render *r, size_t *bytes) {
  return guarded([&] {
    require(r != nullptr && bytes != nullptr, "NULL argument");
    *bytes = r->last_scratch_bytes;
  });
}

int earhip_render_scratch_regrows(const earhip_render *r, long *count) {
  return guarded([&] {
    require(r != nullptr && count != nullptr, "NULL argument");
    *count = r->scratch_regrows;
  });
}

int earhip_render_last_tail_blocks(const earhip_render *r, int *blocks) {
  return guarded([&] {
    require(r != nullptr && blocks != nullptr, "NULL argument");
    *blocks = r->last_tail_blocks;
  });
}

int earhip_render_last_host_chunks(const earhip_render *r, int *chunks) {
  return guarded([&] {
    require(r != nullptr && chunks != nullptr, "NULL argument");
    *chunks = r->last_host_chunks;
  });
}

int earhip_render_last_list_layout(const earhip_render *r, int *paired) {
  return guarded([&] {
    require(r != nullptr && paired != nullptr, "NULL argument");
    *paired = r->last_paired;
  });
}

int earhip_render_last_plan(const earhip_render *r, int out[4]) {
  return guarded([&] {
    require(r != nullptr && out != nullptr, "NULL argument");
    out[0] = r->last_kind;
    for (int i = 0; i < 3; i++) out[1 + i] = r->last_plan[i];
  });
}

}
```

libear_amd/csrc/common.h:

```cpp
#pragma once

#include <hip/hip_runtime.h>

#include <cstdint>
#include <cstdio>
#include <string>
#include <vector>

#include "../../include/earhip.h"

namespace earhip {

struct Error {
  int code;
  std::string msg;
};

void set_last_error(const std::string &msg);

template <typename F>
int guarded(F &&f) {
  try {
    f();
    return EARHIP_OK;
  } catch (const Error &e) {
    set_last_error(e.msg);
    return e.code;
  } catch (const std::bad_alloc &) {
    set_last_error("out of host memory");
    return EARHIP_INTERNAL_ERROR;
  } catch (const std::exception &e) {
    set_last_error(e.what());
    return EARHIP_INTERNAL_ERROR;
  }
}

[[noreturn]] inline void fail_invalid(const std::string &m) {
  throw Error{EARHIP_INVALID_ARGUMENT, m};
}
[[noreturn]] inline void fail_internal(const std::string &m) {
  throw Error{EARHIP_INTERNAL_ERROR, "internal error: " + m};
}
inline void require(bool ok, const char *m) {
  if (!ok) fail_invalid(m);
}

#define EARHIP_HIP(expr)                                                        \
  do {                                                                          \
    hipError_t e_ = (expr);                                                     \
    if (e_ != hipSuccess)                                                       \
      throw ::earhip::Error{EARHIP_DEVICE_ERROR,                                \
                            std::string("internal error: HIP: ") +              \
                                hipGetErrorString(e_) + " in " #expr};          \
  } while (0)

inline bool is_pow2(size_t v) { return v && !(v & (v - 1)); }

template <typename T>
struct DevBuf {
  T *p = nullptr;
  size_t n = 0;
  DevBuf() = default;
  DevBuf(const DevBuf &) = delete;
  DevBuf &operator=(const DevBuf &) = delete;
  ~DevBuf() { release(); }
  void release() {
    if (p) (void)hipFree(p);
    p = nullptr;
    n = 0;
  }
  void alloc(size_t count) {
    release();
    if (count == 0) count = 1;
    EARHIP_HIP(hipMalloc((void **)&p, count * sizeof(T)));
    n = count;
  }
  void alloc_zero(size_t count, hipStream_t s) {
    alloc(count);
    EARHIP_HIP(hipMemsetAsync(p, 0, n * sizeof(T), s));
  }
  void reserve(size_t count) {
    if (count > n) alloc(count);
  }
};

template <typename T>
struct PinBuf {
  T *p = nullptr;
  size_t n = 0;
  PinBuf() = default;
  PinBuf(const PinBuf &) = delete;
  PinBuf &operator=(const PinBuf &) = delete;
  ~PinBuf() {
    if (p) (void)hipHostFree(p);
  }
  void reserve(size_t count) {
    if (count <= n) return;
    if (p) (void)hipHostFree(p);
    p = nullptr;
    n = 0;
    EARHIP_HIP(hipHostMalloc((void **)&p, count * sizeof(T), hipHostMallocDefault));
    n = count;
  }
};

}

struct earhip_vbs;
namespace earhip {
void vbs_orphan(earhip_vbs *v);
}

namespace earhip {
enum Opt {
  OPT_SPL, OPT_MFMA, OPT_XSCALE, OPT_WAVES, OPT_TPW, OPT_NRT,
  OPT_H2_TILE, OPT_H2_WGS, OPT_H2_RUNS, OPT_P2_TILE, OPT_P2_PAIRS, OPT_P2_WGS, OPT_HINGE, OPT_HG_TILE, OPT_HBUILD_TPW, OPT_BUILD_TPW,
  OPT_K2_WG, OPT_K2_OWN_BLOCK, OPT_RUN, OPT_GSPLIT,
  OPT_PROBE_RUNS, OPT_BLOCK_GROUPS, OPT_DEBUG_TIMING, OPT_TAILCUT, OPT_HOST_CHUNK_MB, OPT_HOST_THREADS, OPT_HG_ROBUST, OPT_BUILD_2K,
  OPT_HOST_BIND, OPT_HOST_NT, OPT_HOST_FIRST, OPT_H2_PAIR, OPT_COUNT
};
struct OptVal {
  bool set = false;
  int v = 0;
};
}

struct earhip_ctx {
  earhip::OptVal opt[earhip::OPT_COUNT];
  bool has(earhip::Opt o) const { return opt[o].set; }
  int get(earhip::Opt o, int dflt = 0) const { return opt[o].set ? opt[o].v : dflt; }
  void apply_options();
  int device = 0;
  hipStream_t stream = nullptr;
  bool own_stream = false;
  bool strict = false;
  int spl = 4;
  int use_mfma = 3;
  int x_scale_log2 = 14;
  bool x_scale_auto = true;
  earhip::DevBuf<unsigned> level;
  int level_idx = 0;
  int last_gate_idx = -1;
  bool last_hinge_robust = false;
  int last_wide_idx = -1;
  earhip::DevBuf<unsigned> tile_slow;
  size_t tile_slow_cap = 0;
  int tile_slow_idx = 0;
  earhip::DevBuf<unsigned> obj_level;
  int obj_level_cap = 0;
  long lazy_allocs = 0;
  unsigned *record_slot = nullptr;
  int max_waves = 4;
  int tiles_per_wg = 4;
  bool tiles_per_wg_forced = false;
  int nrt = 8;
  int num_cus = 256;
  size_t hinge_build_lds = 64 * 1024;
  struct HostRange {
    const char *base;
    size_t bytes;
    bool owned;
  };
  std::vector<HostRange> host_ranges;
  std::vector<earhip_vbs *> pinned_adapters;
  bool host_reachable(const void *p, size_t bytes) const {
    const char *c = static_cast<const char *>(p);
    for (const auto &r : host_ranges)
      if (c >= r.base && c + bytes <= r.base + r.bytes) return true;
    return false;
  }
  earhip::PinBuf<float> pin_in, pin_out;
  earhip::DevBuf<float> dev_in, dev_out, dev_pts;
  void use() const { EARHIP_HIP(hipSetDevice(device)); }
};

namespace earhip {
int panner_create(earhip_ctx *ctx, const char *layout, int n_channels, const double *azimuth, const double *elevation,
                  earhip_panner **out, bool with_extent);
}
```

libear_amd/csrc/curves.h:

```cpp
#pragma once

#include <chrono>
#include <cmath>
#include <cstdio>
#include <cstdlib>

#include <algorithm>
#include <cstring>
#include <vector>

#include "common.h"
#include "gain_kernels.h"
#include "gain_p2.h"
#include "gain_hg.h"
#include "gain_f32g.h"

namespace earhip {

struct ColumnPlan {
  int nout = 24;
  int ngroups = 1;
  int nz = 1;
  int nct = 1;
  int mgroups = 1;
// ... 113 lines not shown
    }
    if (!o.dirty) o.dirty = true, dirty_list_.push_back(m);
  }

  void commit(earhip_ctx *ctx) {
    if (dirty_list_.empty()) return;
#ifdef EARHIP_COMMIT_TIMING
    static double acc[6] = {0, 0, 0, 0, 0, 0};
    static long ncalls = 0;
    auto now = [] { return std::chrono::duration<double, std::micro>(std::chrono::steady_clock::now().time_since_epoch()).count(); };
    double tq = now();
    auto lap = [&](int i) { const double t = now(); acc[i] += t - tq; tq = t; };
    struct Print { ~Print() { if (ncalls) fprintf(stderr, "commit timing (us/call over %ld): sync %.2f regions %.2f mirror+stats %.2f finish %.2f upload %.2f tail %.2f\n", ncalls, acc[0]/ncalls, acc[1]/ncalls, acc[2]/ncalls, acc[3]/ncalls, acc[4]/ncalls, acc[5]/ncalls); } };
    static Print printer;
    ncalls++;
#define EARHIP_LAP(i) lap(i)
#else
#define EARHIP_LAP(i)
#endif
    const size_t row = (size_t)plan_.row;
    if (staged_) EARHIP_HIP(hipEventSynchronize(staged_));
    EARHIP_LAP(0);
    bool full_upload = !uploaded_once_;
    for (int m : dirty_list_) {
      Obj &o = obj_[m];
      const int n = (int)o.t.size();
      if (n > o.cap) {
        abandoned_ += (size_t)o.cap;
        o.cap = std::max(16, n + n / 2);
        o.off = (int)arena_used_;
        arena_used_ += (size_t)o.cap;
      }
    }
    if (abandoned_ > arena_used_ / 2 && abandoned_ > 4096) {
      arena_used_ = 2;
      abandoned_ = 0;
      for (int m = 0; m < M_; m++) {
        Obj &o = obj_[m];
        o.cap = std::max(16, (int)o.t.size() + (int)o.t.size() / 2);
        o.off = (int)arena_used_;
        arena_used_ += (size_t)o.cap;
        if (!o.dirty) o.dirty = true, dirty_list_.push_back(m);
      }
      full_upload = true;
    }
    if (arena_used_ >= ((size_t)1 << 31)) fail_invalid("too many interpolation points");
    if (arena_used_ > arena_cap_) {
      const size_t cap = arena_used_ + arena_used_ / 2 + 64;
      EARHIP_HIP(hipStreamSynchronize(ctx->stream));
      PinBuf<int64_t> nt;
      PinBuf<uint8_t> nf;
      PinBuf<PointRec> nr;
      PinBuf<float> ng;
      nt.reserve(cap), nf.reserve(cap), nr.reserve(cap), ng.reserve(cap * row);
      if (arena_cap_) {
        std::memcpy(nt.p, h_time_.p, arena_cap_ * sizeof(int64_t));
        std::memcpy(nf.p, h_flat_.p, arena_cap_);
        std::memcpy(nr.p, h_rec_.p, arena_cap_ * sizeof(PointRec));
        std::memcpy(ng.p, h_gain_.p, arena_cap_ * row * sizeof(float));
      } else {
        std::memset(ng.p, 0, 2 * row * sizeof(float));
        std::memset(nt.p, 0, 2 * sizeof(int64_t));
        std::memset(nf.p, 0, 2);
        std::memset(nr.p, 0, 2 * sizeof(PointRec));
      }
      std::swap(h_time_.p, nt.p), std::swap(h_time_.n, nt.n);
      std::swap(h_flat_.p, nf.p), std::swap(h_flat_.n, nf.n);
      std::swap(h_rec_.p, nr.p), std::swap(h_rec_.n, nr.n);
      std::swap(h_gain_.p, ng.p), std::swap(h_gain_.n, ng.n);
      d_time_.alloc(cap), d_flat_.alloc(cap), d_rec_.alloc(cap), d_gain_.alloc(cap * row * (kinks_ ? 2 : 1));
      arena_cap_ = cap;
      full_upload = true;
    }
    if (!h_off_.p) {
      h_off_.reserve(M_), h_cnt_.reserve(M_), h_changed_.reserve(M_), h_gcol_.reserve(row), h_hdr_.reserve(M_);
      d_off_.alloc(M_), d_cnt_.alloc(M_), d_gcol_.alloc(row), d_hdr_.alloc(M_);
    }
    EARHIP_LAP(1);
    const float old_scale = gain_scale();
    bool cmax_shrunk = false;
    for (int m : dirty_list_) {
      Obj &o = obj_[m];
      const int n = (int)o.t.size();
      h_off_.p[m] = o.off;
      h_cnt_.p[m] = n;
      h_hdr_.p[m] = ObjHdr{o.off, n, o.t[0], o.t[n - 1], 0};
      std::memcpy(h_time_.p + o.off, o.t.data(), (size_t)n * sizeof(int64_t));
      std::memcpy(h_flat_.p + o.off, o.flat.data(), (size_t)n);
      std::memcpy(h_gain_.p + (size_t)o.off * row, o.g.data(), (size_t)n * row * sizeof(float));
      for (int k = 0; k < n; k++) {
        PointRec &r = h_rec_.p[o.off + k];
        r.time = o.t[k];
        const int64_t len = k ? o.t[k] - o.t[k - 1] : 0;
        r.scale = len > 0 ? 1.0f / (float)len : 0.0f;
        r.flat = o.flat[k];
      }
      float *cm = obj_cmax_.data() + (size_t)m * row;
      if (o.has_stats) cmax_shrunk = retire(o.st, cm) || cmax_shrunk;
      o.st = stats_of(o, cm);
      admit(o.st, cm);
      o.has_stats = true;
    }
    if (cmax_shrunk) {
      for (size_t c = 0; c < row; c++) {
        if (!shrunk_cols_[c]) continue;
        shrunk_cols_[c] = 0;
        float v = 0.0f;
        for (int m = 0; m < M_; m++) {
          const float a = obj_cmax_[(size_t)m * row + c];
          v = a <= v ? v : a;
        }
        cmax_[c] = v;
      }
    }
    EARHIP_LAP(2);
    finish_stats();
    const float set_scale = gain_scale();
    bool gcol_changed = !uploaded_once_ || set_scale != old_scale;
    for (size_t c = 0; c < row; c++) {
      const float cm = cmax_[c];
      int e;
      std::frexp(cm, &e);
      const float v = (cm >= 1e-30f && cm < 1e30f) ? std::ldexp(1.0f, 14 - e) : (set_scale > 0.0f ? set_scale : 1.0f);
      gcol_changed = gcol_changed || v != h_gcol_.p[c];
      h_gcol_.p[c] = v;
    }
    EARHIP_LAP(3);
    if (gcol_changed) EARHIP_HIP(hipMemcpyAsync(d_gcol_.p, h_gcol_.p, row * sizeof(float), hipMemcpyHostToDevice, ctx->stream));
    if (full_upload || dirty_list_.size() > (size_t)M_ / 4) {
      EARHIP_HIP(hipMemcpyAsync(d_off_.p, h_off_.p, M_ * sizeof(int32_t), hipMemcpyHostToDevice, ctx->stream));
      EARHIP_HIP(hipMemcpyAsync(d_cnt_.p, h_cnt_.p, M_ * sizeof(int32_t), hipMemcpyHostToDevice, ctx->stream));
      EARHIP_HIP(hipMemcpyAsync(d_hdr_.p, h_hdr_.p, M_ * sizeof(ObjHdr), hipMemcpyHostToDevice, ctx->stream));
      EARHIP_HIP(hipMemcpyAsync(d_time_.p, h_time_.p, arena_used_ * sizeof(int64_t), hipMemcpyHostToDevice, ctx->stream));
      EARHIP_HIP(hipMemcpyAsync(d_flat_.p, h_flat_.p, arena_used_, hipMemcpyHostToDevice, ctx->stream));
      EARHIP_HIP(hipMemcpyAsync(d_rec_.p, h_rec_.p, arena_used_ * sizeof(PointRec), hipMemcpyHostToDevice, ctx->stream));
      EARHIP_HIP(hipMemcpyAsync(d_gain_.p, h_gain_.p, arena_used_ * row * sizeof(float), hipMemcpyHostToDevice, ctx->stream));
    } else {
      for (size_t i = 0; i < dirty_list_.size(); i++) h_changed_.p[i] = dirty_list_[i];
      CurveImage src{h_hdr_.p, h_off_.p, h_cnt_.p, h_time_.p, h_flat_.p, h_rec_.p, h_gain_.p};
      CurveImage dst{d_hdr_.p, d_off_.p, d_cnt_.p, d_time_.p, d_flat_.p, d_rec_.p, d_gain_.p};
      hipLaunchKernelGGL(k_curve_upload, dim3((unsigned)dirty_list_.size()), dim3(256), 0, ctx->stream, src, dst, h_changed_.p,
                         (int)row);
      EARHIP_HIP(hipGetLastError());
    }
    EARHIP_LAP(4);
    if (kinks_) {
      const bool all = full_upload || gcol_changed || dirty_list_.size() > (size_t)M_ / 4;
      if (!all)
        for (size_t i = 0; i < dirty_list_.size(); i++) h_changed_.p[i] = dirty_list_[i];
      derive_kinks(ctx, all ? nullptr : h_changed_.p, all ? M_ : (int)dirty_list_.size());
    }
    if (!staged_) EARHIP_HIP(hipEventCreateWithFlags(&staged_, hipEventDisableTiming));
    EARHIP_HIP(hipEventRecord(staged_, ctx->stream));
    for (int m : dirty_list_) obj_[m].dirty = false;
    dirty_list_.clear();
    uploaded_once_ = true;
    EARHIP_LAP(5);
  }
#undef EARHIP_LAP

  void ensure_kinks(earhip_ctx *ctx) {
    if (kinks_) return;
    kinks_ = true;
    const size_t row = (size_t)plan_.row;
    EARHIP_HIP(hipStreamSynchronize(ctx->stream));
    d_gain_.alloc(arena_cap_ * row * 2);
    EARHIP_HIP(hipMemcpyAsync(d_gain_.p, h_gain_.p, arena_used_ * row * sizeof(float), hipMemcpyHostToDevice, ctx->stream));
    derive_kinks(ctx, nullptr, M_);
    if (!staged_) EARHIP_HIP(hipEventCreateWithFlags(&staged_, hipEventDisableTiming));
    EARHIP_HIP(hipEventRecord(staged_, ctx->stream));
  }
  bool has_kinks() const { return kinks_; }
  bool dirty() const { return !dirty_list_.empty(); }

  bool tiles_aligned(int tile, int64_t t_call) const {
    const int64_t d = t_call >= t_ref_ ? t_call - t_ref_ : t_ref_ - t_call;
    return d % tile == 0 && grid_ % (uint64_t)tile == 0;
  }

  int aligned_tile(int64_t t_call) const {
    const int grids[2] = {512, 256};
    for (int gi = 0; gi < 2; gi++) {
      const int64_t G = grids[gi];
      const int si = 1 - gi;
      int off_grid_limit = M_ / 64;
      if (ramp_share() < 0.5) {
        const double deltas = deltas_per_pair(si ? 512 : 256);
        off_grid_limit = (int)(M_ * std::min(1.0 / 64, deltas / 200.0));
      }
      if (tiles_aligned((int)G, t_call)) return (int)G;
      if (grid_off_[gi] <= off_grid_limit && (((t_call - grid_phase_[gi]) % G) + G) % G == 0) return (int)G;
    }
    return 0;
  }

  double deltas_per_pair(int tile) const {
    const int gi = tile >= 512 ? 1 : 0;
    return tot_.tiles[gi] > 0 ? tot_.incid[gi] / tot_.tiles[gi] * moving_share() : 0.0;
  }
  double moving_share() const { return M_ > 0 ? (double)tot_.moving / M_ : 0.0; }
  double point_density_all() const { return point_density() * moving_share(); }
  double ramp_share() const { return tot_.span > 0 ? tot_.ramp / tot_.span : 0.0; }
  double point_density() const { return tot_.span > 0 ? tot_.npts / tot_.span : 0.0; }
  double pair_waste(int tile) const {
    const int gi = tile >= 512 ? 1 : 0;
    return (tot_.incid[gi] - tot_.touched[gi]) / std::max(1.0, tot_.tiles[gi] + tot_.incid[gi]);
  }
  double hinge_exact_share(size_t in_stride, size_t nsamples) const {
    if (force_ramp_ || !hinge_addressable((size_t)M_, in_stride, nsamples, 2 * arena_cap_, (size_t)plan_.row)) return 2.0;
    return tot_.span > 0 ? std::min(1.0, tot_.bad / std::max(1.0, tot_.span / kHingeTile)) : 0.0;
  }

  int piece_cap(int tile, bool paired) const {
    const int gi = tile >= 512 ? 1 : 0;
    const long slots = paired ? (long)((M_ + 63) & ~63) + 2 * tot_.sum_r7[gi] : (long)M_ + tot_.sum_r15[gi];
    return (int)std::min<long>(slots + 128, (long)kPieceCapPerObject * M_ + 128);
  }

  float gain_scale() const {
    if (!(gain_max_ < 1e30f)) return 0.0f;
    if (gain_max_ < 1e-18f) return 1.0f;
    int e;
    std::frexp(gain_max_, &e);
    return std::ldexp(1.0f, 14 - e);
  }

  const float *column_scales() const { return d_gcol_.p; }

  PointStore device() const {
    PointStore ps;
    ps.hdr = d_hdr_.p;
    ps.off = d_off_.p;
    ps.cnt = d_cnt_.p;
    ps.time = d_time_.p;
    ps.flat = d_flat_.p;
    ps.rec = d_rec_.p;
    ps.gain = d_gain_.p;
    ps.row = plan_.row;
    ps.bus_cols = ncols_ / nbus_;
    ps.nbus = nbus_;
    ps.zero_row = 0;
    ps.npoints = (int)tot_.points;
    ps.rows = (int)arena_used_;
    ps.kink_row0 = kinks_ ? (int)arena_cap_ : 0;
    ps.force_ramp = force_ramp_ ? 1 : 0;
    return ps;
  }

 private:
  void derive_kinks(earhip_ctx *ctx, const int32_t *objects, int count) {
    const size_t row = (size_t)plan_.row;
    uint32_t *kink = reinterpret_cast<uint32_t *>(d_gain_.p + arena_cap_ * row);
    EARHIP_HIP(hipMemsetAsync(kink, 0, 2 * row * sizeof(uint32_t), ctx->stream));
    hipLaunchKernelGGL(k_kink_rows, dim3((unsigned)count), dim3(256), 0, ctx->stream, d_off_.p, d_cnt_.p, d_rec_.p, d_gain_.p, kink,
                       d_gcol_.p, objects, (int)row, nbus_);
    EARHIP_HIP(hipGetLastError());
  }
  struct ObjStats {
    uint64_t gcd = 0;
    int64_t first = 0;
    int64_t phase[2] = {-1, -1};
    double span = 0, ramp = 0, npts = 0, bad = 0, points = 0;
    double incid[2] = {0, 0}, touched[2] = {0, 0}, tiles[2] = {0, 0};
    int maxr[2] = {0, 0};
  };
  struct Obj {
    std::vector<int64_t> t;
    std::vector<float> g;
    std::vector<uint8_t> flat;
    int off = 0, cap = 0;
    bool dirty = false, has_stats = false;
    ObjStats st;
  };

  ObjStats stats_of(const Obj &o, float *cm) const {
    ObjStats s;
    const auto &t = o.t;
    const size_t row = (size_t)plan_.row, n = t.size();
    const int allflat = (1 << nbus_) - 1;
    s.first = t[0];
    s.points = (double)n;
    for (size_t k = 1; k < n && s.gcd != 1; k++) {
      uint64_t a = (uint64_t)(t[k] - t[k - 1]), b = s.gcd;
      while (a) {
        const uint64_t r = b % a;
        b = a;
        a = r;
      }
      s.gcd = b;
    }
    const int64_t grids[2] = {512, 256};
    for (int gi = 0; gi < 2; gi++) {
      const int64_t G = grids[gi];
      const int64_t p0 = ((t[0] % G) + G) % G;
      bool same = s.gcd % (uint64_t)G == 0;
      s.phase[gi] = same ? p0 : -1;
    }
    for (size_t k = 1; k < n; k++) {
      const int64_t len = t[k] - t[k - 1];
      const bool is_ramp = (o.flat[k] & allflat) != allflat;
      s.span += (double)len;
      if (is_ramp) s.ramp += (double)len;
      if (len < kHingeMinLen) s.bad += is_ramp ? 1.0 + (double)len / kHingeTile : 0.5;
    }
    if (n > 1) s.npts = (double)(n - 1);
    for (int gi = 0; gi < 2; gi++) {
      const int64_t T = gi ? 512 : 256;
      auto tile_of = [T](int64_t a) { return a >= 0 ? a / T : -((-a + T - 1) / T); };
      if (n > 1) s.tiles[gi] = (double)(t.back() - t.front()) / (double)T;
      int64_t last_tile = INT64_MIN;
      for (size_t k = 1; k < n; k++) {
        if ((o.flat[k] & allflat) == allflat) continue;
        const int64_t a = t[k] > t[k - 1] ? t[k - 1] : t[k] - 1, b = t[k];
        const int64_t ta = tile_of(a), tb = tile_of(b - 1);
        s.incid[gi] += (double)(tb - ta + 1);
        s.touched[gi] += (double)(tb - ta + 1) - (ta == last_tile ? 1.0 : 0.0);
        last_tile = tb;
      }
    }
    for (int gi = 0; gi < 2; gi++) {
      const int64_t T = gi ? 512 : 256;
      auto is_r = [&](size_t k) { return (o.flat[k] & allflat) != allflat; };
      auto ra = [&](size_t k) { return t[k] > t[k - 1] ? t[k - 1] : t[k] - 1; };
      int best = 0, inside = 0;
      size_t j = 1;
      for (size_t i = 1; i < n; i++) {
        if (!is_r(i)) continue;
        if (j < i) j = i, inside = 0;
        while (j < n && (!is_r(j) || ra(j) < t[i] - 1 + T)) {
          if (is_r(j)) inside++;
          j++;
        }
        best = std::max(best, inside);
        inside--;
      }
      s.maxr[gi] = force_ramp_ ? 1 : best;
    }
    for (size_t c = 0; c < row; c++) cm[c] = 0.0f;
    for (size_t k = 0; k < n; k++) {
      const float *g = o.g.data() + k * row;
      for (size_t c = 0; c < row; c++) {
        const float a = std::fabs(g[c]);
        cm[c] = a <= cm[c] ? cm[c] : a;
      }
    }
    return s;
  }
  bool retire(const ObjStats &s, const float *cm) {
    tot_.span -= s.span, tot_.ramp -= s.ramp, tot_.npts -= s.npts, tot_.bad -= s.bad, tot_.points -= s.points;
    tot_.moving -= s.npts > 0 ? 1 : 0;
    for (int gi = 0; gi < 2; gi++) {
      tot_.incid[gi] -= s.incid[gi], tot_.touched[gi] -= s.touched[gi], tot_.tiles[gi] -= s.tiles[gi];
      tot_.sum_r15[gi] -= std::min(s.maxr[gi], kPieceMaxPerObject), tot_.sum_r7[gi] -= std::min(s.maxr[gi], kPairMaxPerObject);
      if (s.phase[gi] >= 0) phases_[gi].add(s.phase[gi], -1);
    }
    grid_stale_ = true;
    bool shrunk = false;
    for (size_t c = 0; c < cmax_.size(); c++) {
      const bool was_max = cm[c] != cm[c] || (cm[c] > 0.0f && !(cm[c] < cmax_[c]));
      if (was_max) shrunk_cols_[c] = 1, shrunk = true;
    }
    return shrunk;
  }
  void admit(const ObjStats &s, const float *cm) {
    tot_.span += s.span, tot_.ramp += s.ramp, tot_.npts += s.npts, tot_.bad += s.bad, tot_.points += s.points;
    tot_.moving += s.npts > 0 ? 1 : 0;
    for (int gi = 0; gi < 2; gi++) {
      tot_.incid[gi] += s.incid[gi], tot_.touched[gi] += s.touched[gi], tot_.tiles[gi] += s.tiles[gi];
      tot_.sum_r15[gi] += std::min(s.maxr[gi], kPieceMaxPerObject), tot_.sum_r7[gi] += std::min(s.maxr[gi], kPairMaxPerObject);
      if (s.phase[gi] >= 0) phases_[gi].add(s.phase[gi], +1);
    }
    grid_stale_ = true;
    for (size_t c = 0; c < cmax_.size(); c++) cmax_[c] = cm[c] <= cmax_[c] ? cmax_[c] : cm[c];
  }
  void finish_stats() {
    if (grid_stale_) {
      t_ref_ = obj_[0].st.first;
      uint64_t g = 0;
      auto fold = [&g](uint64_t a) {
        uint64_t b = g;
        while (a) {
          const uint64_t r = b % a;
          b = a;
          a = r;
        }
        g = b;
      };
      for (int m = 0; m < M_ && g != 1; m++) {
        const ObjStats &s = obj_[m].st;
        fold(s.gcd);
        fold((uint64_t)(s.first >= t_ref_ ? s.first - t_ref_ : t_ref_ - s.first));
      }
      grid_ = g;
      grid_stale_ = false;
    }
    for (int gi = 0; gi < 2; gi++) {
      int64_t best = 0;
      int best_n = 0;
      for (const auto &kv : phases_[gi].items)
        if (kv.second > best_n) best_n = kv.second, best = kv.first;
      grid_phase_[gi] = best;
      grid_off_[gi] = M_ - best_n;
    }
    float gmax = 0.0f;
    for (float v : cmax_) gmax = v <= gmax ? gmax : v;
    gain_max_ = gmax;
  }

  int M_, ncols_, nbus_;
  bool force_ramp_;
  ColumnPlan plan_;
  std::vector<Obj> obj_;
  std::vector<int> dirty_list_;
  bool uploaded_once_ = false;
  size_t arena_used_ = 2, arena_cap_ = 0, abandoned_ = 0;
  struct Totals {
    double span = 0, ramp = 0, npts = 0, bad = 0, points = 0;
    long moving = 0;
    double incid[2] = {0, 0}, touched[2] = {0, 0}, tiles[2] = {0, 0};
    long sum_r15[2] = {0, 0}, sum_r7[2] = {0, 0};
  } tot_;
  struct PhaseCounts {
    std::vector<std::pair<int64_t, int>> items;
    void add(int64_t phase, int d) {
      for (size_t i = 0; i < items.size(); i++)
        if (items[i].first == phase) {
          items[i].second += d;
          if (items[i].second <= 0) items[i] = items.back(), items.pop_back();
          return;
        }
      if (d > 0) items.emplace_back(phase, d);
    }
  } phases_[2];
  std::vector<float> obj_cmax_;
  std::vector<float> cm_scratch_;
  std::vector<uint8_t> shrunk_cols_;
  bool grid_stale_ = true;
  int64_t t_ref_ = 0;
  uint64_t grid_ = 0;
  int64_t grid_phase_[2] = {0, 0};
  int grid_off_[2] = {0, 0};
  std::vector<float> cmax_;
  float gain_max_ = 0;
  DevBuf<int32_t> d_off_, d_cnt_;
  DevBuf<ObjHdr> d_hdr_;
  PinBuf<ObjHdr> h_hdr_;
  DevBuf<int64_t> d_time_;
  DevBuf<uint8_t> d_flat_;
  DevBuf<PointRec> d_rec_;
  DevBuf<float> d_gcol_, d_gain_;
  bool kinks_ = false;
  PinBuf<float> h_gcol_, h_gain_;
  PinBuf<int32_t> h_off_, h_cnt_, h_changed_;
  PinBuf<int64_t> h_time_;
  PinBuf<uint8_t> h_flat_;
  PinBuf<PointRec> h_rec_;
  hipEvent_t staged_ = nullptr;
};

struct MixLaunch {
  bool mfma;
  bool split = false;
  bool wide = false;
  bool pieces = false;
  int pw = 2;
  bool paired = false;
  bool f32grid = false;
  bool hinge = false;
  int hinge_tile = 512;
  int spl;
  int nrt;
  int ntiles, wsplit, gsplit;
  int tpw = 1;
  int tile() const { return f32grid ? kF32GridTile : hinge ? hinge_tile : pieces ? 64 * pw : split ? (wide ? 512 : 256) : mfma ? 16 * nrt : 64 * spl; }
};

inline MixLaunch plan_mix(const earhip_ctx *ctx, const ColumnPlan &cp, int M, int nsamples,
                          bool strict, int max_gsplit, int aligned_tile = 0, double ramp_share = 1.0,
                          float gain_scale = 0.0f, double point_density = 0.0, double pair_waste256 = 1.0,
                          double pair_waste512 = 1.0, double hinge_exact_share = 2.0, bool grid512_strict = false,
                          double deltas256 = 0.0) {
  const bool aligned = aligned_tile >= 256;
  MixLaunch L;
  L.mfma = !strict && ctx->use_mfma;
  L.split = L.mfma && M >= 32 && gain_scale > 0.0f && ctx->use_mfma != 5 && ctx->use_mfma != 6 &&
            (ctx->use_mfma == 4 || (ctx->use_mfma == 3 && aligned));
  const int forced = ctx->get(OPT_H2_TILE);
  L.pieces = L.mfma && !L.split && M >= 32 && M <= kMaxPieceObjects && gain_scale > 0.0f &&
             (ctx->use_mfma == 3 || ctx->use_mfma == 5 || ctx->use_mfma == 6);
  if ((ctx->use_mfma == 5 || ctx->use_mfma == 6) && L.pieces) L.split = false;
  if (L.pieces) {
    const int ptile = ctx->get(OPT_P2_TILE);
    const double kPairWaste = 0.06;
    const double kMostlyRamping = cp.nct == 3 && M <= 1024 ? 0.7 : 0.5;
    const bool paired_by_rule = pair_waste256 < kPairWaste && ramp_share < kMostlyRamping;
    L.paired = paired_by_rule;
    if (ctx->has(OPT_P2_PAIRS)) L.paired = ctx->get(OPT_P2_PAIRS) != 0;
    const bool long_call = nsamples / 512 >= 2 * ctx->num_cus;
    L.pw = ptile == 512 ? 8 : ptile == 256 ? 4 : (L.paired && long_call && pair_waste512 < kPairWaste) ? 8 : 4;
    const double kHingeExact = 0.005, kHingeRamps = 0.5;
    const int hinge_max = (int)std::min((size_t)kMaxHingeCached, ctx->hinge_build_lds / 16);
    L.hinge = M <= hinge_max && hinge_exact_share <= kHingeExact && ramp_share >= kHingeRamps && !(paired_by_rule && L.paired);
    if (ctx->has(OPT_HINGE)) L.hinge = ctx->get(OPT_HINGE) != 0 && M <= hinge_max && hinge_exact_share <= 1.0;
    if (ctx->use_mfma == 6) L.hinge = M <= hinge_max && hinge_exact_share <= 1.0;
    if (ctx->use_mfma == 5) L.hinge = false;
    if (L.hinge && !ctx->has(OPT_HINGE) && ctx->use_mfma == 3 && cp.nct == 3 && deltas256 > 0.0 && point_density > 0.0) {
      const double hinge_est = 0.56 + 0.077 * (point_density * 512.0), lists_est = 0.151 + 0.238 * (1.0 + deltas256);
      if (lists_est < 0.97 * hinge_est) L.hinge = false;
    }
    if (L.hinge) {
      if (ctx->has(OPT_HG_TILE)) L.hinge_tile = ctx->get(OPT_HG_TILE) == 256 ? 256 : 512;
      L.pieces = false, L.paired = false, L.pw = 4;
    }
  }
  L.wide = L.split && aligned_tile >= 512 && forced != 256 && (forced == 512 || nsamples / 512 >= 2 * ctx->num_cus);
  L.f32grid = L.mfma && !L.split && !L.pieces && !L.hinge && ctx->use_mfma == 1 && grid512_strict && gain_scale > 0.0f &&
              nsamples % kF32GridTile == 0 && M >= 16;
  if (L.mfma && !L.split && !L.pieces && !L.hinge && !L.f32grid && M > kMaxSlotObjects) L.mfma = false;
  L.spl = ctx->spl;
  L.nrt = ctx->nrt;
  L.ntiles = (nsamples + L.tile() - 1) / L.tile();
  if (L.split || L.pieces || L.hinge || L.f32grid) {
    L.wsplit = 1;
    L.tpw = 1;
    int g = 1;
    const int nz = cp.mnz * cp.mgroups;
    while (g < max_gsplit && L.ntiles * nz * g < 2 * ctx->num_cus && M / (g * 2) >= 64) g *= 2;
    L.gsplit = g;
    return L;
  }
  if (strict) {
    L.wsplit = 1;
    L.gsplit = 1;
    return L;
  }
  const int groups = L.mfma ? cp.mgroups : cp.ngroups;
  if (L.mfma) L.tpw = std::max(1, std::min(std::min(ctx->tiles_per_wg, L.ntiles), ctx->max_waves / groups));
  if (L.mfma && !ctx->tiles_per_wg_forced) L.tpw = std::max(1, std::min(L.tpw, (ctx->max_waves / groups) / std::max(1, (M + 127) / 128)));
  L.wsplit = std::max(1, std::min(std::max(1, ctx->max_waves / (groups * L.tpw)), std::max(1, M / 8)));
  const int per_wg = std::max(1, M / L.wsplit);
  int g = 1;
  const int want = 2 * ctx->num_cus;
  while (g < max_gsplit && (L.ntiles / L.tpw) * (L.mfma ? cp.mnz : cp.nz) * g < want && per_wg / (g * 2) >= 8) g *= 2;
  L.gsplit = g;
  return L;
}

inline size_t bus_samples_bound(const earhip_ctx *ctx, size_t max_samples, int max_gsplit) {
  const size_t pad = (max_samples + 3) & ~(size_t)3;
  const size_t tpw_max = (size_t)std::max(1, std::min(ctx->tiles_per_wg, ctx->max_waves));
  const size_t split_tiles = (size_t)4 * ctx->num_cus + max_gsplit;
  const size_t split = std::max(split_tiles * 512, split_tiles * tpw_max * 16 * (size_t)ctx->nrt) + 4 * (size_t)max_gsplit;
  return std::max(pad, std::min(pad * (size_t)max_gsplit, split));
}

size_t mix_lds_bytes(const ColumnPlan &cp, const MixLaunch &ml);
void reserve_call_words(earhip_ctx *ctx, int M, size_t max_samples);

inline size_t scratch_units(const CurveSet &cs, const MixLaunch &ml, int M) {
  const size_t nt = (size_t)ml.ntiles;
  if (ml.hinge) {
    const size_t pnt = nt * (size_t)std::max(1, ml.tile() / (64 * ml.pw));
    return std::max(hinge_units((size_t)M, nt) + (size_t)M * nt,
                    piece_units((size_t)M, pnt, (size_t)cs.piece_cap(64 * ml.pw, ml.paired)) + (size_t)M * pnt);
  }
  if (ml.pieces) return piece_units((size_t)M, nt, (size_t)cs.piece_cap(ml.tile(), ml.paired)) + (size_t)M * nt;
  if (ml.split || ml.f32grid || !ml.mfma) return (size_t)M * nt + 1;
  return desc_units((size_t)M, nt);
}

void launch_gain_mix(earhip_ctx *ctx, const CurveSet &cs, const MixLaunch &ml, bool strict,
                     int64_t t_call, int nsamples, const float *in_dev, size_t in_stride,
                     float *out_dev, size_t out_stride, size_t part_stride, SegDesc *desc,
                     hipEvent_t *ev );

}
```

libear_amd/csrc/gain_h2.h:

```cpp
#pragma once

#include <hip/hip_runtime.h>

#include <type_traits>

#include "gain_kernels.h"
#include "gain_mfma.h"

namespace earhip {

typedef uint32_t u32x4 __attribute__((ext_vector_type(4)));
typedef float f32x2 __attribute__((ext_vector_type(2)));

constexpr int kSplitTile = 256;
constexpr int kSplitChunk = 32;

typedef _Float16 f16x8 __attribute__((ext_vector_type(8)));
typedef _Float16 f16x2_t __attribute__((ext_vector_type(2)));

__device__ __forceinline__ uint32_t pack_f16(float a, float b) {
  const f32x2 v = {a, b};
  return __builtin_bit_cast(uint32_t, __builtin_convertvector(v, f16x2_t));
}
__device__ __forceinline__ float f16_lo(uint32_t u) { return (float)__builtin_bit_cast(f16x2_t, u)[0]; }
__device__ __forceinline__ float f16_hi(uint32_t u) { return (float)__builtin_bit_cast(f16x2_t, u)[1]; }
__device__ __forceinline__ float sub_f16_lo(float v, uint32_t u) {
  float r;
  asm("v_fma_mix_f32 %0, %1, -1.0, %2 op_sel:[0,0,0] op_sel_hi:[1,0,0]" : "=v"(r) : "v"(u), "v"(v));
  return r;
}
__device__ __forceinline__ float sub_f16_hi(float v, uint32_t u) {
  float r;
  asm("v_fma_mix_f32 %0, %1, -1.0, %2 op_sel:[1,0,0] op_sel_hi:[1,0,0]" : "=v"(r) : "v"(u), "v"(v));
  return r;
}

constexpr float kLowPieceScale = 2048.0f;
__device__ __forceinline__ uint32_t scale_f16x2_down(uint32_t h) {
  const f16x2_t k = {(_Float16)0.00048828125f, (_Float16)0.00048828125f};
  return __builtin_bit_cast(uint32_t, __builtin_bit_cast(f16x2_t, h) * k);
}

__device__ __forceinline__ f32x4 mfma_f16(const u32x4 &a, const u32x4 &b, const f32x4 &c) {
  return __builtin_amdgcn_mfma_f32_16x16x32_f16(__builtin_bit_cast(f16x8, a), __builtin_bit_cast(f16x8, b), c,
                                                0, 0, 0);
}

constexpr bool h2_persistent(int nct, int nw) { return nw == 8 || nct == 1; }
template <int NCT, int NW, int FORM>
__global__ void __launch_bounds__(64 * NW, NCT == 1 && NW == 8 ? 2 : (NW == 4 ? 2 : 1))
k_gain_mix_h2(GainMixParams P, int zero_row, float x_scale, const float *__restrict__ gcol, const unsigned *level_cur,
              unsigned *level_next, const unsigned *slow_cur, unsigned *slow_next, const unsigned *wide_cur, unsigned *wide_next) {
  if (FORM != 2 && wide_cur && ((*wide_cur & 1u) != 0u) != (FORM == 1)) return;
  constexpr int NRT = 4, TS = 16 * NRT, CH = kSplitChunk;
  constexpr int NQ = CH / NW;
  constexpr int NFRAG = 2 * NCT * 3;
  __shared__ u32x4 bfrag[2][NFRAG + 6][64];
  constexpr int OP = TS + 4;
  __shared__ __attribute__((aligned(16))) float otile[NW][16 * OP];
  __shared__ float inv_gcol[16 * NCT];
  __shared__ unsigned long long redo_tiles[NW];
  auto body = [&](auto wide_tag) __attribute__((always_inline)) {
  constexpr bool WIDE = decltype(wide_tag)::value;
  if (threadIdx.x < 16 * NCT) inv_gcol[threadIdx.x] = 1.0f / gcol[blockIdx.z * 16 * NCT + threadIdx.x];
  __syncthreads();
  const int lane = threadIdx.x & 63;
  const int w = __builtin_amdgcn_readfirstlane(threadIdx.x >> 6);
  const int li = lane & 15, kg = lane >> 4;
  const int ntl = P.ntiles, gx = gridDim.x;
  const bool runs = P.tile_runs != 0;
  const int run_first = (int)(((int64_t)ntl * blockIdx.x) / gx), run_end = (int)(((int64_t)ntl * (blockIdx.x + 1)) / gx);
  const int vb0 = runs ? run_first : (int)blockIdx.x, vstep = runs ? 1 : gx;
  const int vb_last = runs ? max(run_end - 1, run_first) : ntl - 1;
  const int my_tiles = runs ? run_end - run_first : (ntl - (int)blockIdx.x + gx - 1) / gx;
  auto tile_at = [&](int vb) { return runs ? min(vb, ntl - 1) : xcd_tile(vb, ntl); };
  if (blockIdx.x == 0 && blockIdx.y == 0 && blockIdx.z == 0 && threadIdx.x == 0) {
    if (wide_next) *wide_next = 0u;
    record_mode(P, wide_cur != nullptr);
  }
  if (level_cur) {
    const unsigned lv = *level_cur;
    if (lv) {
      const int E = max(-60, min(20, (int)(lv >> 23) - 127));
      x_scale = __uint_as_float((unsigned)(127 + 7 - E) << 23);
    }
    if (blockIdx.x == 0 && blockIdx.y == 0 && blockIdx.z == 0 && threadIdx.x == 0) *level_next = 0;
  }
  const int nparts = gridDim.y;
  const int part = blockIdx.y;
  const int m_lo = (int)(((int64_t)P.M * part) / nparts);
  const int m_hi = (int)(((int64_t)P.M * (part + 1)) / nparts);
  const int col0 = blockIdx.z * 16 * NCT;
  const float *__restrict__ gain = P.ps.gain;
  const unsigned rowlen = (unsigned)P.ps.row;
  auto tile_first = [&](int t) { return t * (TS * NW) + w * TS; };
  auto tile_length = [&](int t) { return max(0, min(TS, P.nsamples - tile_first(t))); };
  auto opaque_lane = [&]() __attribute__((always_inline)) {
    int l = lane;
    asm volatile("" : "+v"(l));
    return l;
  };

  f32x4 tot0[NRT][NCT], tot1[NRT][NCT];
  auto clear_totals = [&]() {
#pragma unroll
    for (int r = 0; r < NRT; r++)
#pragma unroll
      for (int c = 0; c < NCT; c++) tot0[r][c] = tot1[r][c] = f32x4{0.0f, 0.0f, 0.0f, 0.0f};
  };
  clear_totals();

  auto single_object = [&](int t, int m, float sx, bool sg, int khint = -1) __attribute__((always_inline)) {
    const int tile_s0 = tile_first(t), tile_len = tile_length(t);
    if (tile_len <= 0) return;
    const int64_t tile_t0 = P.t_call + tile_s0, tile_t1 = tile_t0 + tile_len;
    const int ol = opaque_lane(), li = ol & 15, kg = ol >> 4;
    float gsc[NCT];
#pragma unroll
    for (int c = 0; c < NCT; c++) gsc[c] = sg ? gcol[col0 + c * 16 + li] : 1.0f;
    const int base = P.ps.off[m], n = P.ps.cnt[m];
    const float *row = P.in + (size_t)m * P.in_stride + tile_s0;
    const bool is_b = kg & 1;
    const bool slot0 = kg < 2;
    int k;
    if (khint >= 0) {
      k = min(khint, n);
      while (k < n && P.ps.time[base + k] <= tile_t0) k++;
    } else {
      k = upper_bound_time(P.ps.time + base, n, tile_t0);
    }
    int cur = 0;
    while (cur < tile_len) {
      const SegDesc dk = describe_segment(P.ps, base, n, k, tile_t0, tile_t1);
      const int r1 = min(seg_r1(dk.info), tile_len);
      if (r1 > cur) {
        const bool ramp = dk.info & kSegRamp;
        float a[NRT], gv[NCT];
#pragma unroll
        for (int r = 0; r < NRT; r++) {
          const int s = li * NRT + r;
          const float x = row[min(s, tile_len - 1)];
          const float p = (float)(dk.d0 + s) * dk.scale;
          float coef = ramp ? (is_b ? p : 1.0f - p) : (is_b ? 0.0f : 1.0f);
          coef = (slot0 && s >= cur && s < r1) ? coef : 0.0f;
          a[r] = (x * coef) * sx;
        }
        const int grow = dk.row + ((ramp && is_b && slot0) ? 1 : 0);
        const float *gp = gain + (size_t)grow * rowlen + col0 + li;
#pragma unroll
        for (int c = 0; c < NCT; c++) gv[c] = gp[c * 16] * gsc[c];
#pragma unroll
        for (int r = 0; r < NRT; r++)
#pragma unroll
          for (int c = 0; c < NCT; c++)
            tot0[r][c] = __builtin_amdgcn_mfma_f32_16x16x4f32(a[r], gv[c], tot0[r][c], 0, 0, 0);
        cur = r1;
      }
      if (!(dk.info & kSegMulti)) break;
      k++;
    }
  };

  const int nobj = m_hi - m_lo;
  const int nch = (P.vec_ok && nobj >= CH) ? (nobj + CH - 1) / CH : 0;
  auto flush_tile = [&](int t, float inv_x, bool col_scaled) __attribute__((always_inline)) {
    const int tile_s0 = tile_first(t), tile_len = tile_length(t);
    if (tile_len > 0) {
      const int ol = opaque_lane(), li = ol & 15, kg = ol >> 4;
      const float wf0 = (float)(w * TS + kg * 16 - (TS * NW) / 2);
      float inv_gc[NCT];
#pragma unroll
      for (int c = 0; c < NCT; c++) inv_gc[c] = col_scaled ? inv_gcol[c * 16 + li] : 1.0f;
      float *op = P.out + (size_t)blockIdx.y * P.part_stride + tile_s0;
      const bool whole = P.vec_ok && tile_len == TS;
#pragma unroll
      for (int c = 0; c < NCT; c++) {
        if (whole) {
          float *ot = otile[w];
#pragma unroll
          for (int e = 0; e < 4; e++) {
            f32x4 v;
#pragma unroll
            for (int r = 0; r < NRT; r++)
              v[r] = (__builtin_fmaf(wf0 + (float)(4 * e + r), tot1[r][c][e], tot0[r][c][e]) * inv_x) * inv_gc[c];
            *reinterpret_cast<f32x4 *>(ot + li * OP + kg * 16 + e * 4) = v;
          }
#pragma unroll
          for (int j = 0; j < 4; j++) {
            const int cl = 4 * j + kg, col = col0 + c * 16 + cl;
            const f32x4 v = *reinterpret_cast<const f32x4 *>(ot + cl * OP + li * 4);
            if (col < P.ncols) __builtin_nontemporal_store(v, reinterpret_cast<f32x4 *>(op + (size_t)col * P.out_stride + li * 4));
          }
          continue;
        }
        const int col = col0 + c * 16 + li;
        if (col >= P.ncols) continue;
        float *o = op + (size_t)col * P.out_stride;
#pragma unroll
        for (int e = 0; e < 4; e++) {
          const int s = kg * 16 + e * 4;
          f32x4 v;
#pragma unroll
          for (int r = 0; r < NRT; r++)
            v[r] = (__builtin_fmaf(wf0 + (float)(4 * e + r), tot1[r][c][e], tot0[r][c][e]) * inv_x) * inv_gc[c];
          if (P.vec_ok && s + 3 < tile_len) {
            *reinterpret_cast<f32x4 *>(o + s) = v;
          } else {
#pragma unroll
            for (int i = 0; i < 4; i++)
              if (s + i < tile_len) o[s + i] = v[i];
          }
        }
      }

    }
    clear_totals();
  };

  if (lane == 0) redo_tiles[w] = 0ull;
  if (nch > 0) {
    const int nvec = (P.nsamples + 3) & ~3;
    const unsigned xrow = (unsigned)(kg * 8) * (unsigned)P.in_stride * 4u;
    const int xsl = w * TS + li * NRT;
    struct Stage {
      int tile, c;
    };
    int left = my_tiles * nch;
    int vb_c = vb0;
    auto next_stage = [&](const Stage &s) __attribute__((always_inline)) {
      Stage n;
      const bool wrap = s.c + 1 == nch;
      n.c = wrap ? 0 : s.c + 1;
      if (wrap) vb_c = min(vb_c + vstep, vb_last);
      n.tile = wrap ? tile_at(vb_c) : s.tile;
      return n;
    };
    const unsigned bcol_e = (unsigned)(col0 + min(lane, 16 * NCT - 1));
    const float g_scale = gcol[bcol_e];
    const int blane = (w * NQ / 8) * 16 + (lane & 15);
    const int bfr = lane < 16 * NCT ? (lane >> 4) * 3 : NFRAG;
    const int bfr1 = lane < 16 * NCT ? NCT * 3 : 3;
    auto chunk_base = [&](int c) { return min(m_lo + c * CH, m_hi - CH); };

    auto load_x_part = [&](const Stage &st, bool live, f32x4 (&x)[8], int q0, int n) {
      const int ts0 = st.tile * (TS * NW);
      const char *bp = reinterpret_cast<const char *>(P.in + (live ? (size_t)chunk_base(st.c) * P.in_stride + ts0 : 0));
      const size_t rstride = live ? P.in_stride * sizeof(float) : 0;
      const unsigned xo = live ? xrow + 4u * (unsigned)min(xsl, nvec - 4 - ts0) : 0u;
#pragma unroll
      for (int q = 0; q < 8; q++)
        if (q >= q0 && q < q0 + n)
          x[q] = __builtin_nontemporal_load(reinterpret_cast<const f32x4 *>(bp + (size_t)q * rstride + xo));
    };
    auto load_x = [&](const Stage &st, bool live, f32x4 (&x)[8]) { load_x_part(st, live, x, 0, 8); };
    typedef const SegDesc __attribute__((address_space(4))) *ConstDesc;
    struct ChunkDesc {
      SegDesc d[NQ];
    };
    auto load_desc = [&](const Stage &st) {
      ConstDesc dp = (ConstDesc)(P.desc + (size_t)st.tile * P.M + chunk_base(st.c) + w * NQ);
      ChunkDesc D;
#pragma unroll
      for (int q = 0; q < NQ; q++) {
        D.d[q].row = dp[q].row;
        D.d[q].d0 = dp[q].d0;
        D.d[q].scale = dp[q].scale;
        D.d[q].info = dp[q].info;
      }
      return D;
    };
    struct ChunkCoef {
      float p0[NQ], scale[NQ];
    };
    auto load_gains = [&](const ChunkDesc &R, int cc, ChunkCoef &D, float (&S)[NQ], float (&E)[NQ]) {
      const int m0 = chunk_base(cc) + w * NQ;
#pragma unroll
      for (int q = 0; q < NQ; q++) {
        const SegDesc d = R.d[q];
        const bool valid = m0 + q >= m_lo + cc * CH && !(d.info & (kSegMulti | kSegQuiet));
        const unsigned rs = (unsigned)(valid ? d.row : zero_row);
        const unsigned re = (valid && (d.info & kSegRamp)) ? (unsigned)d.row + 1u : rs;
        D.p0[q] = d.scale != 0.0f ? (float)(d.d0 + (TS * NW) / 2) * d.scale : 0.0f;
        D.scale[q] = d.scale;
        const float *rps = gain + (size_t)rs * rowlen, *rpe = gain + (size_t)re * rowlen;
        S[q] = rps[bcol_e];
        E[q] = rpe[bcol_e];
      }
    };
    auto store_b = [&](const ChunkCoef &D, const float (&S)[NQ], const float (&E)[NQ], int buf, int part) {
      uint32_t h[NQ / 2], l[NQ / 2], hs[NQ / 2];
#pragma unroll
      for (int i = 0; i < NQ / 2; i++) {
        float v[2];
#pragma unroll
        for (int j = 0; j < 2; j++) {
          const int q = 2 * i + j;
          v[j] = (part == 0 ? __builtin_fmaf(1.0f - D.p0[q], S[q], D.p0[q] * E[q]) : D.scale[q] * (E[q] - S[q])) *
                 g_scale;
        }
        const uint32_t H = pack_f16(v[0], v[1]);
        h[i] = H;
        l[i] = pack_f16(sub_f16_lo(v[0], H), sub_f16_hi(v[1], H));
        hs[i] = WIDE ? scale_f16x2_down(H) : 0u;
      }
      u32x4 *f = &bfrag[buf][bfr][blane] + (part ? bfr1 * 64 : 0);
      if constexpr (NQ == 8) {
        f[0] = u32x4{h[0], h[1], h[2], h[3]};
        f[64] = u32x4{l[0], l[1], l[2], l[3]};
        if constexpr (WIDE) f[128] = u32x4{hs[0], hs[1], hs[2], hs[3]};
      } else {
        typedef uint32_t u32x2 __attribute__((ext_vector_type(2)));
        u32x2 *g = reinterpret_cast<u32x2 *>(f) + (w & 1);
        g[0] = u32x2{h[0], h[1]};
        g[128] = u32x2{l[0], l[1]};
        if constexpr (WIDE) g[256] = u32x2{hs[0], hs[1]};
      }
    };

    f32x4 X0[8], X1[8];
    ChunkDesc L;
    Stage sa, sb, sc;
    sa.tile = tile_at(vb_c);
    sa.c = 0;
    sb = next_stage(sa);
    sc = next_stage(sb);
    int ka = 0;
    {
      float S[NQ], E[NQ];
      ChunkCoef D;
      L = load_desc(sa);
      load_gains(L, 0, D, S, E);
      load_x(sa, true, X0);
      load_x(sb, left > 1, X1);
      store_b(D, S, E, 0, 0);
      store_b(D, S, E, 0, 1);
      L = load_desc(sb);
    }
    auto chunk = [&](int buf, f32x4 (&xc)[8]) __attribute__((always_inline)) {
      __syncthreads();
      float S[NQ], E[NQ];
      ChunkCoef D;
      load_gains(L, sb.c, D, S, E);
      L = load_desc(sc);
      __builtin_amdgcn_sched_barrier(0);

      u32x4 ah[NRT], al[NRT];
#pragma unroll
      for (int qp = 0; qp < 4; qp++)
#pragma unroll
        for (int rp = 0; rp < NRT; rp += 2) {
          const f32x2 s0 = f32x2{xc[2 * qp][rp], xc[2 * qp][rp + 1]} * x_scale;
          const f32x2 s1 = f32x2{xc[2 * qp + 1][rp], xc[2 * qp + 1][rp + 1]} * x_scale;
          const uint32_t H0 = pack_f16(s0[0], s1[0]), H1 = pack_f16(s0[1], s1[1]);
          constexpr float LOW = WIDE ? kLowPieceScale : 1.0f;
          const f32x2 r0 = f32x2{sub_f16_lo(s0[0], H0), sub_f16_lo(s0[1], H1)} * LOW;
          const f32x2 r1 = f32x2{sub_f16_hi(s1[0], H0), sub_f16_hi(s1[1], H1)} * LOW;
          ah[rp][qp] = H0;
          ah[rp + 1][qp] = H1;
          al[rp][qp] = pack_f16(r0[0], r1[0]);
          al[rp + 1][qp] = pack_f16(r0[1], r1[1]);
        }
      constexpr int XB = 2 * NCT >= 4 ? 4 : 2 * NCT;
      __builtin_amdgcn_sched_barrier(0);
      constexpr int NBLK = 2 * NCT;
      u32x4 b[2][2], b2;
      auto load_b = [&](int blk, u32x4 (&bb)[2]) {
#pragma unroll
        for (int q = 0; q < 2; q++) bb[q] = bfrag[buf][((blk & 1) * NCT + (blk >> 1)) * 3 + q][lane];
      };
      load_b(0, b[0]);
      __builtin_amdgcn_sched_group_barrier(0x100, 2, 0);
#pragma unroll
      for (int blk = 0; blk < NBLK; blk++) {
        u32x4(&bc)[2] = b[blk & 1];
        const int ct = blk >> 1;
        if constexpr (WIDE) b2 = bfrag[buf][((blk & 1) * NCT + (blk >> 1)) * 3 + 2][lane];
        if (blk + 1 < NBLK) load_b(blk + 1, b[(blk + 1) & 1]);
        f32x4(&tt)[NRT][NCT] = (blk & 1) == 0 ? tot0 : tot1;
        if constexpr (WIDE) {
#pragma unroll
          for (int r = 0; r < NRT; r++) tt[r][ct] = mfma_f16(ah[r], bc[1], tt[r][ct]);
#pragma unroll
          for (int r = 0; r < NRT; r++) tt[r][ct] = mfma_f16(al[r], b2, tt[r][ct]);
        } else {
#pragma unroll
          for (int r = 0; r < NRT; r++) tt[r][ct] = mfma_f16(al[r], bc[0], tt[r][ct]);
#pragma unroll
          for (int r = 0; r < NRT; r++) tt[r][ct] = mfma_f16(ah[r], bc[1], tt[r][ct]);
        }
#pragma unroll
        for (int r = 0; r < NRT; r++) tt[r][ct] = mfma_f16(ah[r], bc[0], tt[r][ct]);
        if (blk < XB) load_x_part(sc, left > 2, xc, blk * (8 / XB), 8 / XB);
        const bool conv0 = blk == NBLK - 2, conv1 = blk == NBLK - 1;
        if (conv0) store_b(D, S, E, buf ^ 1, 0);
        if (conv1) store_b(D, S, E, buf ^ 1, 1);
        if constexpr (WIDE) {
          if (blk + 1 < NBLK) __builtin_amdgcn_sched_group_barrier(0x100, 3, 0);
          else __builtin_amdgcn_sched_group_barrier(0x100, 1, 0);
        } else {
          if (blk + 1 < NBLK) __builtin_amdgcn_sched_group_barrier(0x100, 2, 0);
        }
        if (conv0 || conv1) {
#pragma unroll
          for (int k = 0; k < 12; k++) {
            __builtin_amdgcn_sched_group_barrier(0x008, 1, 0);
            __builtin_amdgcn_sched_group_barrier(0x002, 5, 0);
          }
        } else if (blk < XB) {
#pragma unroll
          for (int k = 0; k < 8 / XB; k++) {
            __builtin_amdgcn_sched_group_barrier(0x008, 12 / (8 / XB), 0);
            __builtin_amdgcn_sched_group_barrier(0x002, 2, 0);
            __builtin_amdgcn_sched_group_barrier(0x020, 1, 0);
          }
        } else {
          __builtin_amdgcn_sched_group_barrier(0x008, 12, 0);
        }
      }
    };
    auto tile_end = [&](int t) __attribute__((always_inline)) {
      {
        typedef const unsigned __attribute__((address_space(4))) *ConstWord;
        const bool any_slow = !slow_cur || ((ConstWord)slow_cur)[t] != 0u;
        if (slow_next && blockIdx.y == 0 && blockIdx.z == 0 && threadIdx.x == 0) slow_next[t] = 0u;
        for (int b0 = 0; any_slow && b0 < nobj; b0 += 64) {
          const int ol = opaque_lane();
          const SegDesc db = (P.desc + (size_t)t * P.M)[min(m_lo + b0 + ol, m_hi - 1)];
          unsigned long long multi = __ballot((db.info & (kSegMulti | kSegQuiet)) && b0 + ol < nobj);
          while (multi) {
            const int j = __builtin_ctzll(multi);
            multi &= multi - 1;
            single_object(t, m_lo + b0 + j, x_scale, true, seg_k(__shfl(db.info, j)));
          }
        }
        bool bad = false;
#pragma unroll
        for (int r = 0; r < NRT; r++)
#pragma unroll
          for (int c = 0; c < NCT; c++)
#pragma unroll
            for (int e = 0; e < 4; e++) bad |= !(__builtin_fabsf(tot0[r][c][e]) < INFINITY) || !(__builtin_fabsf(tot1[r][c][e]) < INFINITY);
        if (__ballot(bad)) {
          if (lane == 0) redo_tiles[w] |= 1ull << ka;
          clear_totals();
        } else {
          flush_tile(t, 1.0f / x_scale, true);
        }
        ka++;
      }
    };
    auto advance = [&]() __attribute__((always_inline)) {
      if (sa.c == nch - 1) tile_end(sa.tile);
      sa = sb;
      sb = sc;
      sc = next_stage(sc);
      left--;
    };
#pragma unroll 1
    while (left > 0) {
      chunk(0, X0);
      advance();
      if (left <= 0) break;
      chunk(1, X1);
      advance();
    }
  }
  for (int k = 0; k < my_tiles; k++) {
    if (nch > 0 && !((redo_tiles[w] >> (k & 63)) & 1ull)) continue;
    const int t = tile_at(vb0 + k * vstep);
    if (nch == 0 && slow_next && blockIdx.y == 0 && blockIdx.z == 0 && threadIdx.x == 0) slow_next[t] = 0u;
    for (int m = m_lo; m < m_hi; m++) single_object(t, m, 1.0f, false);
    flush_tile(t, 1.0f, false);
  }
  };
  if constexpr (FORM == 2) {
    if (!wide_cur || (*wide_cur & 1u) != 0u) body(std::true_type{});
    else body(std::false_type{});
  } else {
    body(std::integral_constant<bool, FORM == 1>{});
  }
}

}
```

libear_amd/csrc/gain_h2_t1.h:

```cpp
#pragma once

#include "gain_h2.h"

namespace earhip {

template <int NCT, int NW, bool WIDE>
__global__ void __launch_bounds__(64 * NW, 2)
k_gain_mix_h2_t1(GainMixParams P, int zero_row, float x_scale, const float *__restrict__ gcol, const unsigned *level_cur,
              unsigned *level_next, const unsigned *slow_cur, unsigned *slow_next, const unsigned *wide_cur, unsigned *wide_next) {
  if (wide_cur && ((*wide_cur & 1u) != 0u) != WIDE) return;
  constexpr int NRT = 4, TS = 16 * NRT, CH = kSplitChunk;
  constexpr int NQ = CH / NW;
  constexpr int NFRAG = 2 * NCT * 3;
  __shared__ u32x4 bfrag[2][NFRAG + 6][64];
  constexpr int OP = TS + 4;
  __shared__ __attribute__((aligned(16))) float otile[NW][16 * OP];
  __shared__ float inv_gcol[16 * NCT];
  if (threadIdx.x < 16 * NCT) inv_gcol[threadIdx.x] = 1.0f / gcol[blockIdx.z * 16 * NCT + threadIdx.x];
  __syncthreads();
  const int lane = threadIdx.x & 63;
  const int w = __builtin_amdgcn_readfirstlane(threadIdx.x >> 6);
  const int li = lane & 15, kg = lane >> 4;
  const int wgtile = xcd_tile(blockIdx.x, gridDim.x);
  if (blockIdx.x == 0 && blockIdx.y == 0 && blockIdx.z == 0 && threadIdx.x == 0) {
    if (wide_next) *wide_next = 0u;
    record_mode(P, wide_cur != nullptr);
  }
  if (level_cur) {
    const unsigned lv = *level_cur;
    if (lv) {
      const int E = max(-60, min(20, (int)(lv >> 23) - 127));
      x_scale = __uint_as_float((unsigned)(127 + 7 - E) << 23);
    }
    if (blockIdx.x == 0 && blockIdx.y == 0 && blockIdx.z == 0 && threadIdx.x == 0) *level_next = 0;
  }
  const bool any_slow = !slow_cur || slow_cur[wgtile] != 0u;
  if (slow_next && blockIdx.y == 0 && blockIdx.z == 0 && threadIdx.x == 0) slow_next[wgtile] = 0u;
  const int nparts = gridDim.y;
  const int part = blockIdx.y;
  const int m_lo = (int)(((int64_t)P.M * part) / nparts);
  const int m_hi = (int)(((int64_t)P.M * (part + 1)) / nparts);
  const int col0 = blockIdx.z * 16 * NCT;
  const int tile_s0 = wgtile * (TS * NW) + w * TS;
  const int tile_len = max(0, min(TS, P.nsamples - tile_s0));
  const int64_t tile_t0 = P.t_call + tile_s0;
  const int64_t tile_t1 = tile_t0 + tile_len;
  const SegDesc *__restrict__ dtile = P.desc + (size_t)wgtile * P.M;
  const float *__restrict__ gain = P.ps.gain;
  const unsigned rowlen = (unsigned)P.ps.row;

  f32x4 tot0[NRT][NCT], tot1[NRT][NCT];
  auto clear_totals = [&]() {
#pragma unroll
    for (int r = 0; r < NRT; r++)
#pragma unroll
      for (int c = 0; c < NCT; c++) tot0[r][c] = tot1[r][c] = f32x4{0.0f, 0.0f, 0.0f, 0.0f};
  };
  clear_totals();

  auto single_object = [&](int m, float sx, bool sg, int khint = -1) {
    if (tile_len <= 0) return;
    float gsc[NCT];
#pragma unroll
    for (int c = 0; c < NCT; c++) gsc[c] = sg ? gcol[col0 + c * 16 + li] : 1.0f;
    const int base = P.ps.off[m], n = P.ps.cnt[m];
    const float *row = P.in + (size_t)m * P.in_stride + tile_s0;
    const bool is_b = kg & 1;
    const bool slot0 = kg < 2;
    int k;
    if (khint >= 0) {
      k = min(khint, n);
      while (k < n && P.ps.time[base + k] <= tile_t0) k++;
    } else {
      k = upper_bound_time(P.ps.time + base, n, tile_t0);
    }
    int cur = 0;
    while (cur < tile_len) {
      const SegDesc dk = describe_segment(P.ps, base, n, k, tile_t0, tile_t1);
      const int r1 = min(seg_r1(dk.info), tile_len);
      if (r1 > cur) {
        const bool ramp = dk.info & kSegRamp;
        float a[NRT], gv[NCT];
#pragma unroll
        for (int r = 0; r < NRT; r++) {
          const int s = li * NRT + r;
          const float x = row[min(s, tile_len - 1)];
          const float p = (float)(dk.d0 + s) * dk.scale;
          float coef = ramp ? (is_b ? p : 1.0f - p) : (is_b ? 0.0f : 1.0f);
          coef = (slot0 && s >= cur && s < r1) ? coef : 0.0f;
          a[r] = (x * coef) * sx;
        }
        const int grow = dk.row + ((ramp && is_b && slot0) ? 1 : 0);
        const float *gp = gain + (size_t)grow * rowlen + col0 + li;
#pragma unroll
        for (int c = 0; c < NCT; c++) gv[c] = gp[c * 16] * gsc[c];
#pragma unroll
        for (int r = 0; r < NRT; r++)
#pragma unroll
          for (int c = 0; c < NCT; c++)
            tot0[r][c] = __builtin_amdgcn_mfma_f32_16x16x4f32(a[r], gv[c], tot0[r][c], 0, 0, 0);
        cur = r1;
      }
      if (!(dk.info & kSegMulti)) break;
      k++;
    }
  };

  const int nobj = m_hi - m_lo;
  const int nch = (P.vec_ok && nobj >= CH) ? (nobj + CH - 1) / CH : 0;
  float inv_x = 1.0f / x_scale;
  bool col_scaled = true;

  if (nch > 0) {
    const int nvec = (P.nsamples + 3) & ~3;
    const unsigned xs = (unsigned)min(tile_s0 + li * NRT, nvec - 4);
    const unsigned xlane = ((unsigned)(kg * 8) * (unsigned)P.in_stride + xs) * 4u;
    const unsigned bcol_e = (unsigned)(col0 + min(lane, 16 * NCT - 1));
    const float g_scale = gcol[bcol_e];
    const int blane = (w * NQ / 8) * 16 + (lane & 15);
    const int bfr = lane < 16 * NCT ? (lane >> 4) * 3 : NFRAG;
    const int bfr1 = lane < 16 * NCT ? NCT * 3 : 3;
    auto chunk_base = [&](int c) { return min(m_lo + c * CH, m_hi - CH); };

    auto load_x_part = [&](int c, f32x4 (&x)[8], int q0, int n) {
      const bool live = c < nch;
      const char *bp = reinterpret_cast<const char *>(P.in + (live ? (size_t)chunk_base(c) * P.in_stride : 0));
      const size_t rstride = live ? P.in_stride * sizeof(float) : 0;
      const unsigned xo = live ? xlane : 0u;
#pragma unroll
      for (int q = 0; q < 8; q++)
        if (q >= q0 && q < q0 + n)
          x[q] = __builtin_nontemporal_load(reinterpret_cast<const f32x4 *>(bp + (size_t)q * rstride + xo));
    };
    auto load_x = [&](int c, f32x4 (&x)[8]) { load_x_part(c, x, 0, 8); };
    typedef const SegDesc __attribute__((address_space(4))) *ConstDesc;
    struct ChunkDesc {
      SegDesc d[NQ];
    };
    auto load_desc = [&](int c) {
      const int cc = min(c, nch - 1);
      ConstDesc dp = (ConstDesc)(dtile + chunk_base(cc) + w * NQ);
      ChunkDesc D;
#pragma unroll
      for (int q = 0; q < NQ; q++) {
        D.d[q].row = dp[q].row;
        D.d[q].d0 = dp[q].d0;
        D.d[q].scale = dp[q].scale;
        D.d[q].info = dp[q].info;
      }
      return D;
    };
    struct ChunkCoef {
      float p0[NQ], scale[NQ];
    };
    auto load_gains = [&](const ChunkDesc &R, int c, ChunkCoef &D, float (&S)[NQ], float (&E)[NQ]) {
      const int cc = min(c, nch - 1);
      const int m0 = chunk_base(cc) + w * NQ;
#pragma unroll
      for (int q = 0; q < NQ; q++) {
        const SegDesc d = R.d[q];
        const bool valid = m0 + q >= m_lo + cc * CH && !(d.info & (kSegMulti | kSegQuiet));
        const unsigned rs = (unsigned)(valid ? d.row : zero_row);
        const unsigned re = (valid && (d.info & kSegRamp)) ? (unsigned)d.row + 1u : rs;
        D.p0[q] = d.scale != 0.0f ? (float)(d.d0 + (TS * NW) / 2) * d.scale : 0.0f;
        D.scale[q] = d.scale;
        const float *rps = gain + (size_t)rs * rowlen, *rpe = gain + (size_t)re * rowlen;
        S[q] = rps[bcol_e];
        E[q] = rpe[bcol_e];
      }
    };
    auto store_b = [&](const ChunkCoef &D, const float (&S)[NQ], const float (&E)[NQ], int buf, int part) {
      uint32_t h[NQ / 2], l[NQ / 2], hs[NQ / 2];
#pragma unroll
      for (int i = 0; i < NQ / 2; i++) {
        float v[2];
#pragma unroll
        for (int j = 0; j < 2; j++) {
          const int q = 2 * i + j;
          v[j] = (part == 0 ? __builtin_fmaf(1.0f - D.p0[q], S[q], D.p0[q] * E[q]) : D.scale[q] * (E[q] - S[q])) *
                 g_scale;
        }
        const uint32_t H = pack_f16(v[0], v[1]);
        h[i] = H;
        l[i] = pack_f16(sub_f16_lo(v[0], H), sub_f16_hi(v[1], H));
        hs[i] = WIDE ? scale_f16x2_down(H) : 0u;
      }
      u32x4 *f = &bfrag[buf][bfr][blane] + (part ? bfr1 * 64 : 0);
      if constexpr (NQ == 8) {
        f[0] = u32x4{h[0], h[1], h[2], h[3]};
        f[64] = u32x4{l[0], l[1], l[2], l[3]};
        if constexpr (WIDE) f[128] = u32x4{hs[0], hs[1], hs[2], hs[3]};
      } else {
        typedef uint32_t u32x2 __attribute__((ext_vector_type(2)));
        u32x2 *g = reinterpret_cast<u32x2 *>(f) + (w & 1);
        g[0] = u32x2{h[0], h[1]};
        g[128] = u32x2{l[0], l[1]};
        if constexpr (WIDE) g[256] = u32x2{hs[0], hs[1]};
      }
    };

    f32x4 X0[8], X1[8];
    ChunkDesc L;
    {
      float S[NQ], E[NQ];
      ChunkCoef D;
      L = load_desc(0);
      load_gains(L, 0, D, S, E);
      load_x(0, X0);
      load_x(1, X1);
      store_b(D, S, E, 0, 0);
      store_b(D, S, E, 0, 1);
      L = load_desc(1);
    }
    auto chunk = [&](int c, int buf, f32x4 (&xc)[8]) {
      __syncthreads();
      float S[NQ], E[NQ];
      ChunkCoef D;
      load_gains(L, c + 1, D, S, E);
      L = load_desc(c + 2);
      __builtin_amdgcn_sched_barrier(0);

      u32x4 ah[NRT], al[NRT];
#pragma unroll
      for (int qp = 0; qp < 4; qp++)
#pragma unroll
        for (int rp = 0; rp < NRT; rp += 2) {
          const f32x2 s0 = f32x2{xc[2 * qp][rp], xc[2 * qp][rp + 1]} * x_scale;
          const f32x2 s1 = f32x2{xc[2 * qp + 1][rp], xc[2 * qp + 1][rp + 1]} * x_scale;
          const uint32_t H0 = pack_f16(s0[0], s1[0]), H1 = pack_f16(s0[1], s1[1]);
          constexpr float LOW = WIDE ? kLowPieceScale : 1.0f;
          const f32x2 r0 = f32x2{sub_f16_lo(s0[0], H0), sub_f16_lo(s0[1], H1)} * LOW;
          const f32x2 r1 = f32x2{sub_f16_hi(s1[0], H0), sub_f16_hi(s1[1], H1)} * LOW;
          ah[rp][qp] = H0;
          ah[rp + 1][qp] = H1;
          al[rp][qp] = pack_f16(r0[0], r1[0]);
          al[rp + 1][qp] = pack_f16(r0[1], r1[1]);
        }
      constexpr int XB = 2 * NCT >= 4 ? 4 : 2 * NCT;
      __builtin_amdgcn_sched_barrier(0);
      constexpr int NBLK = 2 * NCT;
      u32x4 b[2][2], b2;
      auto load_b = [&](int blk, u32x4 (&bb)[2]) {
#pragma unroll
        for (int q = 0; q < 2; q++) bb[q] = bfrag[buf][((blk & 1) * NCT + (blk >> 1)) * 3 + q][lane];
      };
      load_b(0, b[0]);
      __builtin_amdgcn_sched_group_barrier(0x100, 2, 0);
#pragma unroll
      for (int blk = 0; blk < NBLK; blk++) {
        u32x4(&bc)[2] = b[blk & 1];
        const int ct = blk >> 1;
        if constexpr (WIDE) b2 = bfrag[buf][((blk & 1) * NCT + (blk >> 1)) * 3 + 2][lane];
        if (blk + 1 < NBLK) load_b(blk + 1, b[(blk + 1) & 1]);
        f32x4(&tt)[NRT][NCT] = (blk & 1) == 0 ? tot0 : tot1;
        if constexpr (WIDE) {
#pragma unroll
          for (int r = 0; r < NRT; r++) tt[r][ct] = mfma_f16(ah[r], bc[1], tt[r][ct]);
#pragma unroll
          for (int r = 0; r < NRT; r++) tt[r][ct] = mfma_f16(al[r], b2, tt[r][ct]);
        } else {
#pragma unroll
          for (int r = 0; r < NRT; r++) tt[r][ct] = mfma_f16(al[r], bc[0], tt[r][ct]);
#pragma unroll
          for (int r = 0; r < NRT; r++) tt[r][ct] = mfma_f16(ah[r], bc[1], tt[r][ct]);
        }
#pragma unroll
        for (int r = 0; r < NRT; r++) tt[r][ct] = mfma_f16(ah[r], bc[0], tt[r][ct]);
        if (blk < XB) load_x_part(c + 2, xc, blk * (8 / XB), 8 / XB);
        const bool conv0 = blk == NBLK - 2, conv1 = blk == NBLK - 1;
        if (conv0) store_b(D, S, E, buf ^ 1, 0);
        if (conv1) store_b(D, S, E, buf ^ 1, 1);
        if constexpr (WIDE) {
          if (blk + 1 < NBLK) __builtin_amdgcn_sched_group_barrier(0x100, 3, 0);
          else __builtin_amdgcn_sched_group_barrier(0x100, 1, 0);
        } else {
          if (blk + 1 < NBLK) __builtin_amdgcn_sched_group_barrier(0x100, 2, 0);
        }
        if (conv0 || conv1) {
#pragma unroll
          for (int k = 0; k < 12; k++) {
            __builtin_amdgcn_sched_group_barrier(0x008, 1, 0);
            __builtin_amdgcn_sched_group_barrier(0x002, 5, 0);
          }
        } else if (blk < XB) {
#pragma unroll
          for (int k = 0; k < 8 / XB; k++) {
            __builtin_amdgcn_sched_group_barrier(0x008, 12 / (8 / XB), 0);
            __builtin_amdgcn_sched_group_barrier(0x002, 2, 0);
            __builtin_amdgcn_sched_group_barrier(0x020, 1, 0);
          }
        } else {
          __builtin_amdgcn_sched_group_barrier(0x008, 12, 0);
        }
      }
    };
#pragma unroll 1
    for (int c = 0; c < nch; c += 2) {
      chunk(c, 0, X0);
      if (c + 1 < nch) chunk(c + 1, 1, X1);
    }

    for (int b0 = 0; any_slow && b0 < nobj; b0 += 64) {
      const SegDesc db = dtile[min(m_lo + b0 + lane, m_hi - 1)];
      unsigned long long multi = __ballot((db.info & (kSegMulti | kSegQuiet)) && b0 + lane < nobj);
      while (multi) {
        const int j = __builtin_ctzll(multi);
        multi &= multi - 1;
        single_object(m_lo + b0 + j, x_scale, true, seg_k(__shfl(db.info, j)));
      }
    }
    bool bad = false;
#pragma unroll
    for (int r = 0; r < NRT; r++)
#pragma unroll
      for (int c = 0; c < NCT; c++)
#pragma unroll
        for (int e = 0; e < 4; e++) bad |= !(__builtin_fabsf(tot0[r][c][e]) < INFINITY) || !(__builtin_fabsf(tot1[r][c][e]) < INFINITY);
    if (__ballot(bad)) {
      clear_totals();
      inv_x = 1.0f;
      col_scaled = false;
      for (int m = m_lo; m < m_hi; m++) single_object(m, 1.0f, false);
    }
  } else {
    inv_x = 1.0f;
    col_scaled = false;
    for (int m = m_lo; m < m_hi; m++) single_object(m, 1.0f, false);
  }

  if (tile_len <= 0) return;
  const float wf0 = (float)(w * TS + kg * 16 - (TS * NW) / 2);
  float inv_gc[NCT];
#pragma unroll
  for (int c = 0; c < NCT; c++) inv_gc[c] = col_scaled ? inv_gcol[c * 16 + li] : 1.0f;
  float *op = P.out + (size_t)blockIdx.y * P.part_stride + tile_s0;
  const bool whole = P.vec_ok && tile_len == TS;
#pragma unroll
  for (int c = 0; c < NCT; c++) {
    if (whole) {
      float *ot = otile[w];
#pragma unroll
      for (int e = 0; e < 4; e++) {
        f32x4 v;
#pragma unroll
        for (int r = 0; r < NRT; r++)
          v[r] = (__builtin_fmaf(wf0 + (float)(4 * e + r), tot1[r][c][e], tot0[r][c][e]) * inv_x) * inv_gc[c];
        *reinterpret_cast<f32x4 *>(ot + li * OP + kg * 16 + e * 4) = v;
      }
#pragma unroll
      for (int j = 0; j < 4; j++) {
        const int cl = 4 * j + kg, col = col0 + c * 16 + cl;
        const f32x4 v = *reinterpret_cast<const f32x4 *>(ot + cl * OP + li * 4);
        if (col < P.ncols) __builtin_nontemporal_store(v, reinterpret_cast<f32x4 *>(op + (size_t)col * P.out_stride + li * 4));
      }
      continue;
    }
    const int col = col0 + c * 16 + li;
    if (col >= P.ncols) continue;
    float *o = op + (size_t)col * P.out_stride;
#pragma unroll
    for (int e = 0; e < 4; e++) {
      const int s = kg * 16 + e * 4;
      f32x4 v;
#pragma unroll
      for (int r = 0; r < NRT; r++)
        v[r] = (__builtin_fmaf(wf0 + (float)(4 * e + r), tot1[r][c][e], tot0[r][c][e]) * inv_x) * inv_gc[c];
      if (P.vec_ok && s + 3 < tile_len) {
        *reinterpret_cast<f32x4 *>(o + s) = v;
      } else {
#pragma unroll
        for (int i = 0; i < 4; i++)
          if (s + i < tile_len) o[s + i] = v[i];
      }
    }
  }
}

}
```

libear_amd/csrc/gain_kernels.h:

```cpp
#pragma once

#include <hip/hip_runtime.h>

#include <cstdint>

#include "search.h"

namespace earhip {

struct PointRec {
  int64_t time;
  float scale;
  uint32_t flat;
};
static_assert(sizeof(PointRec) == 16, "PointRec is loaded as one dwordx4");

struct ObjHdr {
  int32_t off, cnt;
  int64_t first, last;
  int64_t reserved;
};
static_assert(sizeof(ObjHdr) == 32, "an object's header is two dwordx4 loads");
struct PointStore {
  const ObjHdr *hdr;
  const int32_t *off;
  const int32_t *cnt;
  const int64_t *time;
  const uint8_t *flat;
  const PointRec *rec;
  const float *gain;
  int row;
  int bus_cols;
  int nbus;
  int zero_row;
  int npoints;
  int rows;
  int kink_row0;
  int force_ramp;
};

struct SegDesc {
  int32_t row;
  int32_t d0;
  float scale;
  int32_t info;
};
static_assert(sizeof(SegDesc) == 16, "SegDesc is loaded as one dwordx4");

constexpr int kSegRamp = 1;
constexpr int kSegMulti = 2;
constexpr int kSegQuiet = (int)0x80000000u;
constexpr int kMaxPointsPerObject = (1 << 18) - 1;
static_assert((((unsigned)kMaxPointsPerObject << 13) & (unsigned)kSegQuiet) == 0u, "the segment index must not reach the quiet flag");
__host__ __device__ __forceinline__ int seg_r1(int info) { return (info >> 4) & 0x1ff; }
__host__ __device__ __forceinline__ int seg_k(int info) { return (info >> 13) & 0x3ffff; }


__device__ __forceinline__ int xcd_tile(int b, int n) {
  const int per = n >> 3;
  if (b >= per * 8) return b;
  return (b & 7) * per + (b >> 3);
}

__device__ __forceinline__ SegDesc describe_segment(const PointStore &ps, int base,
                                                    int n, int k, int64_t t0,
                                                    int64_t t_end) {
  SegDesc d;
  if (ps.force_ramp) k = 1;
  const int allflat = (1 << ps.nbus) - 1;
  const int fb = (k > 0 && k < n) ? (ps.flat[base + k] & allflat) : allflat;
  const bool ramp = ps.force_ramp || fb != allflat;
  const bool multi = !ps.force_ramp && k < n && ps.time[base + k] < t_end;
  const int r1 = min((int)((multi ? ps.time[base + k] : t_end) - t0), 511);
  d.info = (k << 13) | (r1 << 4) | (fb << 2) | (multi ? kSegMulti : 0) | (ramp ? kSegRamp : 0);
  if (ramp) {
    const int64_t start = ps.time[base + k - 1], end = ps.time[base + k];
    d.row = base + k - 1;
    d.d0 = (int32_t)(t0 - start);
    d.scale = 1.0f / (float)(end - start);
  } else {
    d.row = base + (k == n ? k - 1 : k);
    d.d0 = 0;
    d.scale = 0.0f;
  }
  return d;
}

__device__ __forceinline__ SegDesc describe_segment_rec(const PointStore &ps, int base, int n, int k, int64_t t0,
                                                        int64_t t_end) {
  if (ps.force_ramp) return describe_segment(ps, base, n, k, t0, t_end);
  const int allflat = (1 << ps.nbus) - 1;
  PointRec r, q;
  r.time = t_end;
  r.scale = 0.0f;
  r.flat = (uint32_t)allflat;
  q = r;
  if (k < n) r = ps.rec[base + k];
  if (k > 0) q = ps.rec[base + k - 1];
  const int fb = (k > 0 && k < n) ? ((int)r.flat & allflat) : allflat;
  const bool ramp = fb != allflat;
  const bool multi = k < n && r.time < t_end;
  const int r1 = min((int)((multi ? r.time : t_end) - t0), 511);
  SegDesc d;
  d.info = (k << 13) | (r1 << 4) | (fb << 2) | (multi ? kSegMulti : 0) | (ramp ? kSegRamp : 0);
  if (ramp) {
    d.row = base + k - 1;
    d.d0 = (int32_t)(t0 - q.time);
    d.scale = r.scale;
  } else {
    d.row = base + (k == n ? k - 1 : k);
    d.d0 = 0;
    d.scale = 0.0f;
  }
  return d;
}

struct LevelProbe {
  const float *in = nullptr;
  size_t in_stride = 0;
  int nsamples = 0;
  int every = 1;
  unsigned *level = nullptr;
  unsigned *obj_level = nullptr;
};
constexpr int kQuietBinades = 20;
constexpr int kPlainBinades = 8;
__host__ __device__ __forceinline__ bool level_is_quiet(unsigned obj_level, unsigned call_level) {
  return obj_level != 0u && call_level != 0u && (int)(obj_level >> 23) < (int)(call_level >> 23) - kQuietBinades;
}
constexpr int kProbeInstants = 64, kProbeObjects = 16;
static __global__ void __launch_bounds__(64 * kProbeObjects)
k_level_probe(const float *in, size_t in_stride, int nsamples, int M, unsigned *level, unsigned *obj_level, int cap, int nruns) {
  __shared__ unsigned wmax[kProbeObjects];
  const int lane = threadIdx.x & 63, wv = threadIdx.x >> 6, m = blockIdx.x * kProbeObjects + wv;
  const int nvec = nsamples >> 2, ninst = min(kProbeInstants, nvec);
  unsigned v = 0u;
  if (m < M && lane < ninst) {
    const unsigned sh = (unsigned)__builtin_ctz((unsigned)nruns), per = 64u >> sh;
    const unsigned nrun = max((unsigned)ninst / per, 1u), g = min((unsigned)lane / per, nrun - 1u), sub = (unsigned)lane & (per - 1u);
    const unsigned stretch = (unsigned)nvec / nrun;
    const unsigned h = ((unsigned)m * 2654435761u) ^ (g * 40503u);
    const unsigned room = stretch > per ? stretch - per + 1u : 1u;
    const int at = (int)min(g * stretch + __umulhi(h, room) + sub, (unsigned)nvec - 1u);
    const float4 px = *reinterpret_cast<const float4 *>(in + (size_t)m * in_stride + 4 * (size_t)at);
    v = max(max(__float_as_uint(px.x) & 0x7fffffffu, __float_as_uint(px.y) & 0x7fffffffu),
            max(__float_as_uint(px.z) & 0x7fffffffu, __float_as_uint(px.w) & 0x7fffffffu));
  }
  unsigned hi_v = v, lo_v = v ? v : 0xffffffffu;
#pragma unroll
  for (int d = 32; d >= 1; d >>= 1) {
    hi_v = max(hi_v, (unsigned)__shfl_xor((int)hi_v, d));
    lo_v = min(lo_v, (unsigned)__shfl_xor((int)lo_v, d));
  }
  if (lane == 0) {
    wmax[wv] = hi_v;
    if (m < M) {
      obj_level[m] = hi_v;
      obj_level[cap + m] = lo_v == 0xffffffffu ? 0u : lo_v;
    }
  }
  __syncthreads();
  if (threadIdx.x == 0) {
    unsigned he = 0u;
#pragma unroll
    for (int i = 0; i < kProbeObjects; i++) he = max(he, wmax[i]);
    he &= 0x7f800000u;
    if (he != 0 && he > __atomic_load_n(level, __ATOMIC_RELAXED)) atomicMax(level, he);
  }
}

constexpr int kHingeSpreadBinades = 16;
constexpr unsigned kGateHingeUnsafe = 2u;
constexpr int kGateQuietShift = 8;
__host__ __device__ __forceinline__ bool hinge_span_exceeded(unsigned word, int M) {
  const int limit = M / 64 > 4 ? M / 64 : 4;
  return (word & kGateHingeUnsafe) != 0u || (int)(word >> kGateQuietShift) > limit;
}
static __global__ void __launch_bounds__(256)
k_hinge_gate(const unsigned *obj_level, int cap, int M, const unsigned *level_cur, unsigned *gate, bool wide, bool count_quiet) {
  const int m = blockIdx.x * 256 + threadIdx.x;
  bool unsafe = false, quiet = false;
  if (m < M) {
    const unsigned hi = obj_level[m], lo = obj_level[cap + m], call = *level_cur;
    const bool exact_anyway = hi != 0u && call != 0u && (int)(hi >> 23) < (int)(call >> 23) - kHingeSpreadBinades;
    unsafe = !exact_anyway && lo != 0u && call != 0u && (int)(lo >> 23) < (int)(call >> 23) - kHingeSpreadBinades;
    quiet = exact_anyway;
  }
  if (__syncthreads_or(unsafe ? 1 : 0) && threadIdx.x == 0) atomicOr(gate, kGateHingeUnsafe);
  if (count_quiet) {
    const int nq = __syncthreads_count(quiet ? 1 : 0);
    if (nq > 0 && threadIdx.x == 0) atomicAdd(gate, (unsigned)nq << kGateQuietShift);
  }
  if (wide) {
    bool wd = false;
    if (m < M) {
      const unsigned lo = obj_level[cap + m], call = *level_cur;
      wd = lo != 0u && call != 0u && (int)(lo >> 23) < (int)(call >> 23) - kPlainBinades;
    }
    if (__syncthreads_or(wd ? 1 : 0) && threadIdx.x == 0) atomicOr(gate, 1u);
  }
}

struct QuietMark {
  const unsigned *obj_level = nullptr;
  int cap = 0;
  const unsigned *level = nullptr;
  unsigned *wide = nullptr;
};
template <int kPrepRun>
static __global__ void __launch_bounds__(256)
k_seg_prep(PointStore ps, int M, int ntiles, int tile_samples, int64_t t_call, int64_t t_call_end,
           SegDesc *desc, QuietMark qm, unsigned *tile_slow = nullptr) {
  __shared__ SegDesc sh[16 * kPrepRun][17];
  const int ti = threadIdx.x & 15, oi = threadIdx.x >> 4;
  const int tile0 = (blockIdx.x * 16 + ti) * kPrepRun, m = blockIdx.y * 16 + oi;
  bool quiet = false;
  if (qm.obj_level && m < M) {
    const unsigned call = *qm.level, lv = qm.obj_level[m], lo = qm.obj_level[qm.cap + m];
    quiet = level_is_quiet(lv, call);
    if (qm.wide && blockIdx.x == 0 && ti == 0 && lo != 0u && call != 0u && (int)(lo >> 23) < (int)(call >> 23) - kPlainBinades)
      atomicOr(qm.wide, 1u);
  }
  if (tile0 < ntiles && m < M) {
    const ObjHdr hd = ps.hdr[m];
    const int base = hd.off, n = hd.cnt;
    int k = 0;
#pragma unroll
    for (int j = 0; j < kPrepRun; j++) {
      const int tile = tile0 + j;
      if (tile >= ntiles) break;
      const int64_t t0 = t_call + (int64_t)tile * tile_samples;
      int64_t t_end = t0 + tile_samples;
      if (t_end > t_call_end) t_end = t_call_end;
      if (j == 0) {
        k = upper_bound_rec_window(ps.rec + base, n, hd.first, hd.last, t0);
      } else {
        while (k < n && ps.rec[base + k].time <= t0) k++;
      }
      SegDesc d = describe_segment_rec(ps, base, n, k, t0, t_end);
      if (quiet) d.info |= kSegQuiet;
      sh[ti * kPrepRun + j][oi] = d;
      if (tile_slow && (quiet || (d.info & kSegMulti))) atomicOr(&tile_slow[tile], 1u);
    }
  }
  __syncthreads();
#pragma unroll
  for (int j = 0; j < kPrepRun; j++) {
    const int to = (threadIdx.x >> 4) + 16 * j, oo = threadIdx.x & 15;
    const int tile_o = blockIdx.x * 16 * kPrepRun + to, m_o = blockIdx.y * 16 + oo;
    if (tile_o < ntiles && m_o < M) desc[(size_t)tile_o * M + m_o] = sh[to][oo];
  }
}

struct Slot {
  uint32_t mr;
  int32_t row;
  float alpha, beta;
};
static_assert(sizeof(Slot) == 16, "Slot is loaded as one dwordx4");
constexpr int kMaxSlotObjects = 1 << 16;
constexpr int kPlainSlots = 2;
constexpr int kMaskedSlots = 6;
constexpr int kTileSlots = kPlainSlots + kMaskedSlots;
struct SlotLists {
  Slot *slots;
  int *count;
  int *ovf;
  int M;
};
__host__ __device__ inline size_t desc_units(size_t M, size_t ntiles) {
  return (1 + kTileSlots) * M * ntiles + (16 * ntiles + 4 * M * ntiles + 15) / 16 + 1;
}

static __global__ void __launch_bounds__(256)
k_slot_list(PointStore ps, int M, int tile_samples, int64_t t_call, int64_t t_call_end,
            const SegDesc *desc, SlotLists sl) {
  __shared__ unsigned wsum[4];
  __shared__ int base_p, base_m, base_o, written_m, any_over;
  const int tile = blockIdx.x, tid = threadIdx.x, lane = tid & 63, wv = tid >> 6;
  const int64_t t0 = t_call + (int64_t)tile * tile_samples;
  int64_t t_end = t0 + tile_samples;
  if (t_end > t_call_end) t_end = t_call_end;
  Slot *plain = sl.slots + (size_t)tile * kTileSlots * M;
  Slot *masked = plain + kPlainSlots * (size_t)M;
  int *ovf = sl.ovf + (size_t)tile * M;
  if (tid == 0) {
    base_p = 0;
    base_m = 0;
    base_o = 0;
    written_m = 0;
  }
  __syncthreads();
  auto walk = [&](int m, SegDesc dk, Slot *op, Slot *om, int &cp, int &cm, SegDesc (&nx)[2], bool fill) {
    int base = 0, n = 0;
    if (dk.info & kSegMulti) {
      base = ps.off[m];
      n = ps.cnt[m];
    }
    int k = seg_k(dk.info), cur = 0, step = 0;
    cp = 0;
    cm = 0;
    for (;;) {
      const int r1 = seg_r1(dk.info);
      if (r1 > cur) {
        const bool ramp = dk.info & kSegRamp;
        const bool whole = cur == 0 && r1 == tile_samples;
        Slot a;
        a.mr = (uint32_t)m | ((uint32_t)cur << 16) | ((uint32_t)(r1 - 1) << 24);
        a.row = dk.row;
        const float p0 = (float)dk.d0 * dk.scale;
        a.alpha = ramp ? 1.0f - p0 : 1.0f;
        a.beta = ramp ? -dk.scale : 0.0f;
        Slot *o = whole ? op : om;
        int &c = whole ? cp : cm;
        if (o) o[c] = a;
        c++;
        if (ramp) {
          Slot b = a;
          b.row = dk.row + 1;
          b.alpha = p0;
          b.beta = dk.scale;
          if (o) o[c] = b;
          c++;
        }
        cur = r1;
      }
      if (!(dk.info & kSegMulti)) break;
      k++;
      if (step < 2 && !fill) {
        dk = nx[step];
      } else {
        dk = describe_segment(ps, base, n, k, t0, t_end);
        if (step < 2) nx[step] = dk;
      }
      step++;
    }
  };
  auto block_scan = [&](unsigned v, unsigned &total) {
#pragma unroll
    for (int o = 1; o < 64; o <<= 1) {
      const unsigned u = __shfl_up(v, o, 64);
      if (lane >= o) v += u;
    }
    if (lane == 63) wsum[wv] = v;
    __syncthreads();
    unsigned pre = 0, tot = 0;
#pragma unroll
    for (int w = 0; w < 4; w++) {
      const unsigned x = wsum[w];
      if (w < wv) pre += x;
      tot += x;
    }
    __syncthreads();
    total = tot;
    return v + pre;
  };
  for (int mb = 0; mb < M; mb += 256) {
    const int m = mb + tid;
    SegDesc d, nx[2];
    d.info = 0;
    int cp = 0, cm = 0;
    if (m < M) {
      if (desc) {
        d = desc[(size_t)tile * M + m];
      } else {
        const int base = ps.off[m], n = ps.cnt[m];
        d = describe_segment(ps, base, n, upper_bound_time_window(ps.time + base, n, t0), t0, t_end);
      }
      walk(m, d, nullptr, nullptr, cp, cm, nx, true);
    }
    unsigned last;
    const unsigned incl = block_scan((unsigned)cp | ((unsigned)cm << 10), last);
    const int off_p = base_p + (int)(incl & 1023u) - cp;
    const int off_m = base_m + (int)(incl >> 10) - cm;
    const bool over = cm > 0 && off_m + cm > kMaskedSlots * M;
    if (tid == 0) any_over = 0;
    __syncthreads();
    if (over) any_over = 1;
    __syncthreads();
    unsigned oincl = 0, olast = 0;
    if (any_over) oincl = block_scan(over ? 1u : 0u, olast);
    if (m < M) {
      if (over) {
        ovf[base_o + (int)oincl - 1] = m;
      } else if (cp + cm > 0) {
        int a, b;
        walk(m, d, plain + off_p, masked + off_m, a, b, nx, false);
        if (cm > 0) atomicMax(&written_m, off_m + cm);
      }
    }
    __syncthreads();
    if (tid == 0) {
      base_p += (int)(last & 1023u);
      base_m += (int)(last >> 10);
      base_o += (int)olast;
    }
    __syncthreads();
  }
  if (tid == 0) {
    sl.count[tile * 4 + 0] = base_p;
    sl.count[tile * 4 + 1] = written_m;
    sl.count[tile * 4 + 2] = base_o;
// ... 218 lines not shown
```

Baseline: 1.155 million.

## Cache segment descriptors across calls on a timeline and serve them to split kernels

Adds a per-curve-set timeline cache that holds segment descriptors and per-tile slow flags for the whole automation timeline. Only object groups whose curves changed are rebuilt. Calls that line up on the cached tiles reuse these descriptors and skip the per-call k_seg_prep launch. Per-object quiet state is now computed by a last-workgroup pass in the level probe and kept as bitmasks that the h2 kernels OR in, and extra probe workgroups prefetch the cached descriptors into cache. The cost is extra device memory (default 64 MB), more complex invalidation logic, and the quiet bit lookups in the hot mix kernels.

```diff
diff --git a/include/earhip.h b/include/earhip.h
--- a/include/earhip.h
+++ b/include/earhip.h
@@ -273,6 +273,7 @@
 int earhip_render_last_tail_blocks(const earhip_render *r, int *blocks);
 int earhip_render_last_host_chunks(const earhip_render *r, int *chunks);
 int earhip_render_scratch_bytes(const earhip_render *r, size_t *bytes);
+int earhip_render_last_desc_served(const earhip_render *r, int *served);
 
 typedef struct earhip_comm earhip_comm;
 int earhip_comm_unique_id(void *id128);
diff --git a/libear_amd/capi.py b/libear_amd/capi.py
--- a/libear_amd/capi.py
+++ b/libear_amd/capi.py
@@ -862,6 +862,11 @@
         check(load().earhip_render_last_list_layout(self.h, C.byref(v)))
         return None if v.value < 0 else bool(v.value)
 
+    def desc_served(self):
+        v = C.c_int(0)
+        check(load().earhip_render_last_desc_served(self.h, C.byref(v)))
+        return bool(v.value)
+
     def last_plan(self):
         out = (C.c_int * 4)()
         check(load().earhip_render_last_plan(self.h, out))
diff --git a/libear_amd/csrc/api_core.hip b/libear_amd/csrc/api_core.hip
--- a/libear_amd/csrc/api_core.hip
+++ b/libear_amd/csrc/api_core.hip
@@ -44,8 +44,9 @@
 void launch_gain_mix(earhip_ctx *ctx, const CurveSet &cs, const MixLaunch &ml, bool strict,
                      int64_t t_call, int nsamples, const float *in_dev, size_t in_stride,
                      float *out_dev, size_t out_stride, size_t part_stride, SegDesc *desc,
-                     hipEvent_t *ev) {
+                     hipEvent_t *ev, const CurveSet::DescServe *serve) {
   const ColumnPlan &cp = cs.plan();
+  const bool served = serve && serve->desc && (ml.split || ml.f32grid);
   const PointStore ps = cs.device();
   const int M = cs.M();
   const bool slots = ml.mfma && !ml.split && !ml.pieces && !ml.hinge && !ml.f32grid;
@@ -73,19 +74,30 @@
     ctx->last_wide_idx = wide_cur ? ctx->level_idx : -1;
     ctx->level_idx ^= 1;
     if (ctx->obj_level_cap < M) {
-      EARHIP_HIP(hipStreamSynchronize(ctx->stream));
-      ctx->obj_level_cap = M + M / 2 + 64;
-      ctx->obj_level.alloc_zero(2 * (size_t)ctx->obj_level_cap, ctx->stream);
+      reserve_obj_words(ctx, M);
       ctx->lazy_allocs++;
     }
     probe.obj_level = ctx->obj_level.p;
     probe.level = level_cur;
+    ProbeVerdict pv;
+    if (served && ml.split) {
+      const size_t W = ctx->quiet_words();
+      pv.count = ctx->obj_quiet.p + 2 * W + 2;
+      pv.quiet_obj = ctx->obj_quiet.p;
+      pv.quiet_any = ctx->obj_quiet.p + 2 * W;
+      pv.wide = wide_cur;
+      pv.warm = reinterpret_cast<const char *>(serve->desc);
+      pv.warm_lines = (unsigned)(((size_t)M * ml.ntiles * sizeof(SegDesc) + 127) / 128);
+    }
+    const unsigned nprobe = (unsigned)((M + kProbeObjects - 1) / kProbeObjects);
+    pv.nprobe = nprobe;
+    const unsigned nwarm = pv.warm ? std::min<unsigned>((pv.warm_lines + 64 * kProbeObjects - 1) / (64 * kProbeObjects), 2 * (unsigned)ctx->num_cus) : 0u;
     const int probe_runs = [&] {
       const int v = ctx->get(OPT_PROBE_RUNS);
       return v >= 1 && v <= 64 && (v & (v - 1)) == 0 ? v : 16;
     }();
-    hipLaunchKernelGGL(k_level_probe, dim3((M + kProbeObjects - 1) / kProbeObjects), dim3(64 * kProbeObjects), 0, ctx->stream, in_dev,
-                       in_stride, nsamples, M, level_cur, ctx->obj_level.p, ctx->obj_level_cap, probe_runs);
+    hipLaunchKernelGGL(k_level_probe, dim3(nprobe + nwarm), dim3(64 * kProbeObjects), 0, ctx->stream, in_dev,
+                       in_stride, nsamples, M, level_cur, ctx->obj_level.p, ctx->obj_level_cap, probe_runs, pv);
   }
   PieceLists pl;
   pl.pieces = reinterpret_cast<Piece *>(desc);
@@ -96,15 +108,29 @@
   pl.slots = cs.piece_cap(ptile, ml.paired);
   pl.count = reinterpret_cast<int *>(pl.pieces + (size_t)pl.cap() * pnt);
   pl.ovf = pl.count + (size_t)8 * pnt;
-  unsigned *slow_cur = nullptr, *slow_next = nullptr;
+  const unsigned *slow_cur = nullptr;
+  unsigned *slow_mine = nullptr, *slow_next = nullptr;
+  const unsigned *quiet_obj = nullptr, *quiet_any = nullptr;
   if (ml.split) {
+    if (ctx->obj_level_cap < M) {
+      reserve_obj_words(ctx, M);
+      ctx->lazy_allocs++;
+    }
+    const size_t W = ctx->quiet_words();
+    const bool verdicts = served && probe.obj_level;
+    quiet_obj = ctx->obj_quiet.p + (verdicts ? 0 : W);
+    quiet_any = ctx->obj_quiet.p + 2 * W + (verdicts ? 0 : 1);
+  }
+  if (ml.split && served) {
+    slow_cur = serve->slow;
+  } else if (ml.split) {
     if (ctx->tile_slow_cap < (size_t)ml.ntiles) {
       EARHIP_HIP(hipStreamSynchronize(ctx->stream));
       ctx->tile_slow_cap = std::max<size_t>(2 * (size_t)ml.ntiles, 1024);
       ctx->tile_slow.alloc_zero(2 * ctx->tile_slow_cap, ctx->stream);
       ctx->lazy_allocs++;
     }
-    slow_cur = ctx->tile_slow.p + (size_t)ctx->tile_slow_idx * ctx->tile_slow_cap;
+    slow_cur = slow_mine = ctx->tile_slow.p + (size_t)ctx->tile_slow_idx * ctx->tile_slow_cap;
     slow_next = ctx->tile_slow.p + (size_t)(ctx->tile_slow_idx ^ 1) * ctx->tile_slow_cap;
     ctx->tile_slow_idx ^= 1;
   }
@@ -178,7 +204,7 @@
     EARHIP_BUILD_CASE(1) EARHIP_BUILD_CASE(2) EARHIP_BUILD_CASE(4) EARHIP_BUILD_CASE(8)
 #undef EARHIP_BUILD_CASE
   }
-  if (!fused_prep && !one_pass) {
+  if (!fused_prep && !one_pass && !served) {
     const dim3 ogrid((M + 15) / 16);
     QuietMark qm;
     if (probe.obj_level) {
@@ -187,10 +213,10 @@
     }
     if (ml.ntiles >= 2048)
       hipLaunchKernelGGL(k_seg_prep<4>, dim3((ml.ntiles + 63) / 64, ogrid.x), dim3(256), 0, ctx->stream, ps, M,
-                         ml.ntiles, ml.tile(), t_call, t_call + nsamples, desc, qm, slow_cur);
+                         ml.ntiles, ml.tile(), t_call, t_call + nsamples, desc, qm, slow_mine);
     else
       hipLaunchKernelGGL(k_seg_prep<2>, dim3((ml.ntiles + 31) / 32, ogrid.x), dim3(256), 0, ctx->stream, ps, M,
-                         ml.ntiles, ml.tile(), t_call, t_call + nsamples, desc, qm, slow_cur);
+                         ml.ntiles, ml.tile(), t_call, t_call + nsamples, desc, qm, slow_mine);
   }
   SlotLists sl;
   sl.slots = reinterpret_cast<Slot *>(desc + (size_t)M * ml.ntiles);
@@ -210,7 +236,7 @@
   P.out = out_dev;
   P.out_stride = out_stride;
   P.part_stride = part_stride;
-  P.desc = desc;
+  P.desc = served ? const_cast<SegDesc *>(serve->desc) : desc;
   P.ps = ps;
   P.t_call = t_call;
   P.nsamples = nsamples;
@@ -290,10 +316,10 @@
     const bool two_launches = ctx->get(OPT_H2_PAIR, 0) != 0;
 #define EARHIP_H2_LAUNCH(NCT_, NW_, WIDE_)                                                                          \
   hipLaunchKernelGGL((k_gain_mix_h2<NCT_, NW_, WIDE_>), bgrid, dim3(64 * NW_), 0, ctx->stream, P, ps.zero_row, xs,  \
-                     gs, level_cur, level_next, slow_cur, slow_next, wide_cur, wide_next);
+                     gs, level_cur, level_next, slow_cur, slow_next, wide_cur, wide_next, quiet_obj, quiet_any);
 #define EARHIP_H2T1_LAUNCH(NCT_, NW_, WIDE_)                                                                        \
   hipLaunchKernelGGL((k_gain_mix_h2_t1<NCT_, NW_, WIDE_>), bgrid, dim3(64 * NW_), 0, ctx->stream, P, ps.zero_row, xs, \
-                     gs, level_cur, level_next, slow_cur, slow_next, wide_cur, wide_next);
+                     gs, level_cur, level_next, slow_cur, slow_next, wide_cur, wide_next, quiet_obj, quiet_any);
 #define EARHIP_H2_CASE(NCT_)                                                                                        \
   if (cp.nct == NCT_) {                                                                                             \
     if (ml.tile() == 512) {                                                                                         \
@@ -343,15 +369,20 @@
   EARHIP_HIP(hipGetLastError());
 }
 
+void reserve_obj_words(earhip_ctx *ctx, int M) {
+  if (ctx->obj_level_cap >= M) return;
+  EARHIP_HIP(hipStreamSynchronize(ctx->stream));
+  ctx->obj_level_cap = M + M / 2 + 64;
+  ctx->obj_level.alloc_zero(2 * (size_t)ctx->obj_level_cap, ctx->stream);
+  ctx->obj_quiet.alloc_zero(2 * ctx->quiet_words() + 3, ctx->stream);
+}
+
 void reserve_call_words(earhip_ctx *ctx, int M, size_t max_samples) {
   if (!ctx->level.p) ctx->level.alloc_zero(4, ctx->stream);
   const size_t ntiles = (max_samples + 255) / 256;
   const bool grow_obj = ctx->obj_level_cap < M, grow_tiles = ctx->tile_slow_cap < ntiles;
   if (grow_obj || grow_tiles) EARHIP_HIP(hipStreamSynchronize(ctx->stream));
-  if (grow_obj) {
-    ctx->obj_level_cap = M + M / 2 + 64;
-    ctx->obj_level.alloc_zero(2 * (size_t)ctx->obj_level_cap, ctx->stream);
-  }
+  if (grow_obj) reserve_obj_words(ctx, M);
   if (grow_tiles) {
     ctx->tile_slow_cap = std::max<size_t>(ntiles + ntiles / 4, 1024);
     ctx->tile_slow.alloc_zero(2 * ctx->tile_slow_cap, ctx->stream);
@@ -440,7 +471,7 @@
 
 static const char *const kOptNames[OPT_COUNT] = {
     "SPL", "MFMA", "XSCALE", "WAVES", "TPW", "NRT", "H2_TILE", "H2_WGS", "H2_RUNS", "P2_TILE", "P2_PAIRS", "P2_WGS", "HINGE", "HG_TILE", "HBUILD_TPW",
-    "BUILD_TPW", "K2_WG", "K2_OWN_BLOCK", "RUN", "GSPLIT", "PROBE_RUNS", "BLOCK_GROUPS", "DEBUG_TIMING", "TAILCUT", "HOST_CHUNK_MB", "HOST_THREADS", "HG_ROBUST", "BUILD_2K", "HOST_BIND", "HOST_NT", "HOST_FIRST", "H2_PAIR"};
+    "BUILD_TPW", "K2_WG", "K2_OWN_BLOCK", "RUN", "GSPLIT", "PROBE_RUNS", "BLOCK_GROUPS", "DEBUG_TIMING", "TAILCUT", "HOST_CHUNK_MB", "HOST_THREADS", "HG_ROBUST", "BUILD_2K", "HOST_BIND", "HOST_NT", "HOST_FIRST", "H2_PAIR", "DESC_CACHE_MB"};
 
 static int parse_option_value(const std::string &key, const char *text) {
   char *end = nullptr;
diff --git a/libear_amd/csrc/api_render.hip b/libear_amd/csrc/api_render.hip
--- a/libear_amd/csrc/api_render.hip
+++ b/libear_amd/csrc/api_render.hip
@@ -394,7 +394,11 @@
       EARHIP_HIP(hipStreamSynchronize(ctx->stream));
       desc.reserve(need + need / 4);
     }
-  }
+    const MixLaunch ml = plan_call((size_t)T, last_in_stride ? last_in_stride : (size_t)T * (size_t)B);
+    const size_t mb = (size_t)std::max(ctx->get(OPT_DESC_CACHE_MB, kDescCacheDefaultMB), 0);
+    curves->reserve_timeline(ctx, (ml.split || ml.f32grid) && !ctx->strict ? ml.tile() : 0, std::min(mb << 20, 4 * desc.n * sizeof(SegDesc)));
+  }
+  bool last_served = false;
 
   int resident_workgroups(const MixLaunch &ml) const {
     if (!(ml.split || ml.pieces || ml.hinge)) return 0;
@@ -460,7 +464,7 @@
         desc.reserve(need + need / 2);
         scratch_regrows++;
       }
-      last_scratch_bytes = need * 16;
+      last_scratch_bytes = need * 16 + curves->timeline_bytes();
     }
     const size_t bus_stride = ((size_t)nsamples + 3) & ~(size_t)3;
     const size_t part_stride = bus_stride * K * N;
@@ -480,14 +484,17 @@
       evp = pd.e;
     }
     const long lazy_before = ctx->lazy_allocs;
+    CurveSet::DescServe sv;
+    if ((ml.split || ml.f32grid) && nsamples % ml.tile() == 0) sv = curves->serve_timeline(ctx, ml.tile(), t, ml.ntiles);
+    if (!continues) last_served = sv.desc != nullptr;
     ctx->record_slot = rec.p + (continues ? 1 : 0);
     if (K == 1) {
       if (ml.gsplit == 1) {
         launch_gain_mix(ctx, *curves, ml, strict, t, nsamples, in_dev, in_stride, out_dev,
-                        out_stride, 0, desc.p, evp);
+                        out_stride, 0, desc.p, evp, &sv);
       } else {
         launch_gain_mix(ctx, *curves, ml, strict, t, nsamples, in_dev, in_stride, bus.p,
-                        bus_stride, part_stride, desc.p, evp);
+                        bus_stride, part_stride, desc.p, evp, &sv);
         hipLaunchKernelGGL(k_sum_parts, dim3((nsamples + 255) / 256, N), dim3(256), 0,
                            ctx->stream, bus.p, part_stride, ml.gsplit, bus_stride, N, nsamples,
                            out_dev, out_stride);
@@ -495,7 +502,7 @@
       }
     } else {
       launch_gain_mix(ctx, *curves, ml, strict, t, nsamples, in_dev, in_stride, bus.p,
-                      bus_stride, part_stride, desc.p, evp);
+                      bus_stride, part_stride, desc.p, evp, &sv);
       DecorParams P;
       P.bus = bus.p;
       P.bus_stride = bus_stride;
@@ -1267,6 +1274,13 @@
   });
 }
 
+int earhip_render_last_desc_served(const earhip_render *r, int *served) {
+  return guarded([&] {
+    require(r != nullptr && served != nullptr, "NULL argument");
+    *served = r->last_served ? 1 : 0;
+  });
+}
+
 int earhip_render_last_plan(const earhip_render *r, int out[4]) {
   return guarded([&] {
     require(r != nullptr && out != nullptr, "NULL argument");
diff --git a/libear_amd/csrc/common.h b/libear_amd/csrc/common.h
--- a/libear_amd/csrc/common.h
+++ b/libear_amd/csrc/common.h
@@ -117,8 +117,9 @@
   OPT_H2_TILE, OPT_H2_WGS, OPT_H2_RUNS, OPT_P2_TILE, OPT_P2_PAIRS, OPT_P2_WGS, OPT_HINGE, OPT_HG_TILE, OPT_HBUILD_TPW, OPT_BUILD_TPW,
   OPT_K2_WG, OPT_K2_OWN_BLOCK, OPT_RUN, OPT_GSPLIT,
   OPT_PROBE_RUNS, OPT_BLOCK_GROUPS, OPT_DEBUG_TIMING, OPT_TAILCUT, OPT_HOST_CHUNK_MB, OPT_HOST_THREADS, OPT_HG_ROBUST, OPT_BUILD_2K,
-  OPT_HOST_BIND, OPT_HOST_NT, OPT_HOST_FIRST, OPT_H2_PAIR, OPT_COUNT
+  OPT_HOST_BIND, OPT_HOST_NT, OPT_HOST_FIRST, OPT_H2_PAIR, OPT_DESC_CACHE_MB, OPT_COUNT
 };
+constexpr int kDescCacheDefaultMB = 64;
 struct OptVal {
   bool set = false;
   int v = 0;
@@ -148,6 +149,8 @@
   int tile_slow_idx = 0;
   earhip::DevBuf<unsigned> obj_level;
   int obj_level_cap = 0;
+  size_t quiet_words() const { return ((size_t)obj_level_cap + 63) / 64 * 2 + 2; }
+  earhip::DevBuf<unsigned> obj_quiet;
   long lazy_allocs = 0;
   unsigned *record_slot = nullptr;
   int max_waves = 4;
diff --git a/libear_amd/csrc/curves.h b/libear_amd/csrc/curves.h
--- a/libear_amd/csrc/curves.h
+++ b/libear_amd/csrc/curves.h
@@ -289,6 +289,13 @@
     }
     if (!staged_) EARHIP_HIP(hipEventCreateWithFlags(&staged_, hipEventDisableTiming));
     EARHIP_HIP(hipEventRecord(staged_, ctx->stream));
+    if (tl_tile_) {
+      for (int m : dirty_list_) {
+        const int g = m / 16;
+        if (!tl_group_dirty_[g]) tl_group_dirty_[g] = 1, tl_groups_.push_back(g);
+      }
+      tl_fresh_commit_ = true;
+    }
     for (int m : dirty_list_) obj_[m].dirty = false;
     dirty_list_.clear();
     uploaded_once_ = true;
@@ -363,6 +370,82 @@
   }
 
   const float *column_scales() const { return d_gcol_.p; }
+
+  struct DescServe {
+    const SegDesc *desc = nullptr;
+    const unsigned *slow = nullptr;
+  };
+  void reserve_timeline(earhip_ctx *ctx, int tile, size_t max_bytes) {
+    if (force_ramp_ || tile == 0 || max_bytes == 0) {
+      tl_tile_ = 0;
+      return;
+    }
+    int64_t tmin = obj_[0].t.front(), tmax = obj_[0].t.back();
+    for (int m = 1; m < M_; m++) tmin = std::min(tmin, obj_[m].t.front()), tmax = std::max(tmax, obj_[m].t.back());
+    auto floor_div = [](int64_t a, int64_t b) { return a >= 0 ? a / b : -((-a + b - 1) / b); };
+    int64_t k0 = floor_div(tmin, tile);
+    const int64_t k1 = std::max(floor_div(tmax + tile - 1, tile), k0 + 1);
+    bool all = tile != tl_tile_;
+    if (!all && k0 >= tl_k0_) k0 = tl_k0_;
+    all = all || k0 != tl_k0_;
+    const size_t per_tile = (size_t)M_ * sizeof(SegDesc) + sizeof(unsigned);
+    const int64_t n = std::min<int64_t>(k1 - k0, (int64_t)std::min<size_t>(max_bytes / per_tile, (size_t)1 << 24));
+    if (n <= 0) {
+      tl_tile_ = 0;
+      return;
+    }
+    if ((size_t)n > tl_cap_) {
+      EARHIP_HIP(hipStreamSynchronize(ctx->stream));
+      tl_cap_ = std::min<size_t>((size_t)n + (size_t)n / 2, std::max<size_t>(max_bytes / per_tile, (size_t)n));
+      tl_desc_.alloc(tl_cap_ * (size_t)M_);
+      tl_slow_.alloc(tl_cap_);
+      all = true;
+    }
+    if (tl_group_dirty_.empty()) tl_group_dirty_.assign((size_t)(M_ + 15) / 16, 0), tl_groups_.reserve((size_t)(M_ + 15) / 16);
+    all = all || n > tl_n_;
+    tl_tile_ = tile, tl_k0_ = k0, tl_n_ = n;
+    if (all) tl_all_ = true, tl_fresh_commit_ = true;
+  }
+  DescServe serve_timeline(earhip_ctx *ctx, int tile, int64_t t_call, int ntiles) {
+    DescServe sv;
+    const bool fresh = tl_fresh_commit_;
+    tl_fresh_commit_ = false;
+    if (!tl_tile_ || tile != tl_tile_ || t_call % tile != 0) return sv;
+    const int64_t k = t_call / tile;
+    if (k < tl_k0_ || k + ntiles > tl_k0_ + tl_n_) return sv;
+    if (tl_all_ || !tl_groups_.empty()) {
+      const bool all = tl_all_ || tl_groups_.size() > (size_t)kPrepGroupList;
+      const size_t pairs = (all ? (size_t)M_ : 16 * tl_groups_.size()) * (size_t)tl_n_;
+      if (fresh && pairs > (size_t)M_ * (size_t)ntiles) {
+        tl_fresh_commit_ = false;
+        return sv;
+      }
+      PrepGroups pg;
+      if (!all)
+        for (int g : tl_groups_) pg.g[pg.n++] = g;
+      else
+        EARHIP_HIP(hipMemsetAsync(tl_slow_.p, 0, sizeof(unsigned) * (size_t)tl_n_, ctx->stream));
+      const int64_t t0 = tl_k0_ * tile, t1 = (tl_k0_ + tl_n_) * tile;
+      const unsigned gy = all ? (unsigned)((M_ + 15) / 16) : (unsigned)pg.n;
+      const PointStore ps = device();
+      if (tl_n_ >= 2048)
+        hipLaunchKernelGGL(k_seg_prep<4>, dim3((unsigned)((tl_n_ + 63) / 64), gy), dim3(256), 0, ctx->stream, ps, M_, (int)tl_n_, tile, t0, t1,
+                           tl_desc_.p, QuietMark(), tl_slow_.p, pg);
+      else
+        hipLaunchKernelGGL(k_seg_prep<2>, dim3((unsigned)((tl_n_ + 31) / 32), gy), dim3(256), 0, ctx->stream, ps, M_, (int)tl_n_, tile, t0, t1,
+                           tl_desc_.p, QuietMark(), tl_slow_.p, pg);
+      EARHIP_HIP(hipGetLastError());
+      for (int g : tl_groups_) tl_group_dirty_[g] = 0;
+      tl_groups_.clear();
+      tl_all_ = false;
+      tl_fills_++;
+    }
+    sv.desc = tl_desc_.p + (size_t)(k - tl_k0_) * (size_t)M_;
+    sv.slow = tl_slow_.p + (size_t)(k - tl_k0_);
+    return sv;
+  }
+  size_t timeline_bytes() const { return tl_tile_ ? tl_desc_.n * sizeof(SegDesc) + tl_slow_.n * sizeof(unsigned) : 0; }
+  long timeline_fills() const { return tl_fills_; }
 
   PointStore device() const {
     PointStore ps;
@@ -593,6 +676,16 @@
   PinBuf<uint8_t> h_flat_;
   PinBuf<PointRec> h_rec_;
   hipEvent_t staged_ = nullptr;
+  DevBuf<SegDesc> tl_desc_;
+  DevBuf<unsigned> tl_slow_;
+  size_t tl_cap_ = 0;
+  int tl_tile_ = 0;
+  int64_t tl_k0_ = 0, tl_n_ = 0;
+  bool tl_all_ = true;
+  bool tl_fresh_commit_ = false;
+  std::vector<uint8_t> tl_group_dirty_;
+  std::vector<int> tl_groups_;
+  long tl_fills_ = 0;
 };
 
 struct MixLaunch {
@@ -709,6 +802,8 @@
 void launch_gain_mix(earhip_ctx *ctx, const CurveSet &cs, const MixLaunch &ml, bool strict,
                      int64_t t_call, int nsamples, const float *in_dev, size_t in_stride,
                      float *out_dev, size_t out_stride, size_t part_stride, SegDesc *desc,
-                     hipEvent_t *ev );
+                     hipEvent_t *ev ,
+                     const CurveSet::DescServe *serve = nullptr );
+void reserve_obj_words(earhip_ctx *ctx, int M);
 
 }
diff --git a/libear_amd/csrc/gain_h2.h b/libear_amd/csrc/gain_h2.h
--- a/libear_amd/csrc/gain_h2.h
+++ b/libear_amd/csrc/gain_h2.h
@@ -50,7 +50,8 @@
 template <int NCT, int NW, int FORM>
 __global__ void __launch_bounds__(64 * NW, NCT == 1 && NW == 8 ? 2 : (NW == 4 ? 2 : 1))
 k_gain_mix_h2(GainMixParams P, int zero_row, float x_scale, const float *__restrict__ gcol, const unsigned *level_cur,
-              unsigned *level_next, const unsigned *slow_cur, unsigned *slow_next, const unsigned *wide_cur, unsigned *wide_next) {
+              unsigned *level_next, const unsigned *slow_cur, unsigned *slow_next, const unsigned *wide_cur, unsigned *wide_next,
+              const unsigned *quiet_obj, const unsigned *quiet_any) {
   if (FORM != 2 && wide_cur && ((*wide_cur & 1u) != 0u) != (FORM == 1)) return;
   constexpr int NRT = 4, TS = 16 * NRT, CH = kSplitChunk;
   constexpr int NQ = CH / NW;
@@ -60,8 +61,9 @@
   __shared__ __attribute__((aligned(16))) float otile[NW][16 * OP];
   __shared__ float inv_gcol[16 * NCT];
   __shared__ unsigned long long redo_tiles[NW];
-  auto body = [&](auto wide_tag) __attribute__((always_inline)) {
+  auto body = [&](auto wide_tag, auto quiet_tag) __attribute__((always_inline)) {
   constexpr bool WIDE = decltype(wide_tag)::value;
+  constexpr bool QUIET = decltype(quiet_tag)::value;
   if (threadIdx.x < 16 * NCT) inv_gcol[threadIdx.x] = 1.0f / gcol[blockIdx.z * 16 * NCT + threadIdx.x];
   __syncthreads();
   const int lane = threadIdx.x & 63;
@@ -259,13 +261,20 @@
     };
     auto load_desc = [&](const Stage &st) {
       ConstDesc dp = (ConstDesc)(P.desc + (size_t)st.tile * P.M + chunk_base(st.c) + w * NQ);
+      unsigned long long qbits = 0ull;
+      if constexpr (QUIET) {
+        typedef const unsigned __attribute__((address_space(4))) *ConstQuiet;
+        const unsigned mq = (unsigned)(chunk_base(st.c) + w * NQ);
+        ConstQuiet qp = (ConstQuiet)(quiet_obj + (mq >> 5));
+        qbits = (((unsigned long long)qp[1] << 32) | qp[0]) >> (mq & 31u);
+      }
       ChunkDesc D;
 #pragma unroll
       for (int q = 0; q < NQ; q++) {
         D.d[q].row = dp[q].row;
         D.d[q].d0 = dp[q].d0;
         D.d[q].scale = dp[q].scale;
-        D.d[q].info = dp[q].info;
+                D.d[q].info = QUIET ? dp[q].info | (int)(((unsigned)(qbits >> q) & 1u) << 31) : dp[q].info;
       }
       return D;
     };
@@ -421,11 +430,15 @@
     auto tile_end = [&](int t) __attribute__((always_inline)) {
       {
         typedef const unsigned __attribute__((address_space(4))) *ConstWord;
-        const bool any_slow = !slow_cur || ((ConstWord)slow_cur)[t] != 0u;
+        const bool any_slow = QUIET || !slow_cur || ((ConstWord)slow_cur)[t] != 0u;
         if (slow_next && blockIdx.y == 0 && blockIdx.z == 0 && threadIdx.x == 0) slow_next[t] = 0u;
         for (int b0 = 0; any_slow && b0 < nobj; b0 += 64) {
           const int ol = opaque_lane();
-          const SegDesc db = (P.desc + (size_t)t * P.M)[min(m_lo + b0 + ol, m_hi - 1)];
+          SegDesc db = (P.desc + (size_t)t * P.M)[min(m_lo + b0 + ol, m_hi - 1)];
+          if constexpr (QUIET) {
+            const unsigned mb = (unsigned)min(m_lo + b0 + ol, m_hi - 1);
+            db.info |= (int)(((quiet_obj[mb >> 5] >> (mb & 31u)) & 1u) << 31);
+          }
           unsigned long long multi = __ballot((db.info & (kSegMulti | kSegQuiet)) && b0 + ol < nobj);
           while (multi) {
             const int j = __builtin_ctzll(multi);
@@ -473,11 +486,16 @@
     flush_tile(t, 1.0f, false);
   }
   };
+  const bool quiet = *quiet_any != 0u;
+  auto form = [&](auto wide_tag) __attribute__((always_inline)) {
+    if (quiet) body(wide_tag, std::true_type{});
+    else body(wide_tag, std::false_type{});
+  };
   if constexpr (FORM == 2) {
-    if (!wide_cur || (*wide_cur & 1u) != 0u) body(std::true_type{});
-    else body(std::false_type{});
+    if (!wide_cur || (*wide_cur & 1u) != 0u) form(std::true_type{});
+    else form(std::false_type{});
   } else {
-    body(std::integral_constant<bool, FORM == 1>{});
+    form(std::integral_constant<bool, FORM == 1>{});
   }
 }
 
diff --git a/libear_amd/csrc/gain_h2_t1.h b/libear_amd/csrc/gain_h2_t1.h
--- a/libear_amd/csrc/gain_h2_t1.h
+++ b/libear_amd/csrc/gain_h2_t1.h
@@ -7,7 +7,8 @@
 template <int NCT, int NW, bool WIDE>
 __global__ void __launch_bounds__(64 * NW, 2)
 k_gain_mix_h2_t1(GainMixParams P, int zero_row, float x_scale, const float *__restrict__ gcol, const unsigned *level_cur,
-              unsigned *level_next, const unsigned *slow_cur, unsigned *slow_next, const unsigned *wide_cur, unsigned *wide_next) {
+              unsigned *level_next, const unsigned *slow_cur, unsigned *slow_next, const unsigned *wide_cur, unsigned *wide_next,
+              const unsigned *quiet_obj, const unsigned *quiet_any) {
   if (wide_cur && ((*wide_cur & 1u) != 0u) != WIDE) return;
   constexpr int NRT = 4, TS = 16 * NRT, CH = kSplitChunk;
   constexpr int NQ = CH / NW;
@@ -34,7 +35,8 @@
     }
     if (blockIdx.x == 0 && blockIdx.y == 0 && blockIdx.z == 0 && threadIdx.x == 0) *level_next = 0;
   }
-  const bool any_slow = !slow_cur || slow_cur[wgtile] != 0u;
+  const bool quiet = *quiet_any != 0u;
+  const bool any_slow = !slow_cur || quiet || slow_cur[wgtile] != 0u;
   if (slow_next && blockIdx.y == 0 && blockIdx.z == 0 && threadIdx.x == 0) slow_next[wgtile] = 0u;
   const int nparts = gridDim.y;
   const int part = blockIdx.y;
@@ -140,13 +142,20 @@
     auto load_desc = [&](int c) {
       const int cc = min(c, nch - 1);
       ConstDesc dp = (ConstDesc)(dtile + chunk_base(cc) + w * NQ);
+      unsigned long long qbits = 0ull;
+      if (quiet) {
+        typedef const unsigned __attribute__((address_space(4))) *ConstQuiet;
+        const unsigned mq = (unsigned)(chunk_base(cc) + w * NQ);
+        ConstQuiet qp = (ConstQuiet)(quiet_obj + (mq >> 5));
+        qbits = (((unsigned long long)qp[1] << 32) | qp[0]) >> (mq & 31u);
+      }
       ChunkDesc D;
 #pragma unroll
       for (int q = 0; q < NQ; q++) {
         D.d[q].row = dp[q].row;
         D.d[q].d0 = dp[q].d0;
         D.d[q].scale = dp[q].scale;
-        D.d[q].info = dp[q].info;
+        D.d[q].info = dp[q].info | (int)(((unsigned)(qbits >> q) & 1u) << 31);
       }
       return D;
     };
@@ -301,7 +310,8 @@
     }
 
     for (int b0 = 0; any_slow && b0 < nobj; b0 += 64) {
-      const SegDesc db = dtile[min(m_lo + b0 + lane, m_hi - 1)];
+      SegDesc db = dtile[min(m_lo + b0 + lane, m_hi - 1)];
+      { const unsigned mb = (unsigned)min(m_lo + b0 + lane, m_hi - 1); db.info |= (int)(((quiet_obj[mb >> 5] >> (mb & 31u)) & 1u) << 31); }
       unsigned long long multi = __ballot((db.info & (kSegMulti | kSegQuiet)) && b0 + lane < nobj);
       while (multi) {
         const int j = __builtin_ctzll(multi);
diff --git a/libear_amd/csrc/gain_kernels.h b/libear_amd/csrc/gain_kernels.h
--- a/libear_amd/csrc/gain_kernels.h
+++ b/libear_amd/csrc/gain_kernels.h
@@ -129,9 +129,27 @@
   return obj_level != 0u && call_level != 0u && (int)(obj_level >> 23) < (int)(call_level >> 23) - kQuietBinades;
 }
 constexpr int kProbeInstants = 64, kProbeObjects = 16;
+struct ProbeVerdict {
+  unsigned *count = nullptr;
+  unsigned *quiet_obj = nullptr;
+  unsigned *quiet_any = nullptr;
+  unsigned *wide = nullptr;
+  const char *warm = nullptr;
+  unsigned warm_lines = 0, nprobe = 0;
+};
 static __global__ void __launch_bounds__(64 * kProbeObjects)
-k_level_probe(const float *in, size_t in_stride, int nsamples, int M, unsigned *level, unsigned *obj_level, int cap, int nruns) {
+k_level_probe(const float *in, size_t in_stride, int nsamples, int M, unsigned *level, unsigned *obj_level, int cap, int nruns,
+              ProbeVerdict pv = ProbeVerdict()) {
   __shared__ unsigned wmax[kProbeObjects];
+  __shared__ unsigned last_wg;
+  if (pv.count && blockIdx.x >= pv.nprobe) {
+    const unsigned nwarm = gridDim.x - pv.nprobe;
+    for (unsigned i = (blockIdx.x - pv.nprobe) * (64 * kProbeObjects) + threadIdx.x; i < pv.warm_lines; i += nwarm * (64 * kProbeObjects)) {
+      const unsigned v = *reinterpret_cast<const unsigned *>(pv.warm + (size_t)i * 128);
+      asm volatile("" ::"v"(v));
+    }
+    return;
+  }
   const int lane = threadIdx.x & 63, wv = threadIdx.x >> 6, m = blockIdx.x * kProbeObjects + wv;
   const int nvec = nsamples >> 2, ninst = min(kProbeInstants, nvec);
   unsigned v = 0u;
@@ -167,6 +185,36 @@
     he &= 0x7f800000u;
     if (he != 0 && he > __atomic_load_n(level, __ATOMIC_RELAXED)) atomicMax(level, he);
   }
+  if (!pv.count) return;
+  __syncthreads();
+  if (threadIdx.x == 0) {
+    __threadfence();
+    last_wg = atomicAdd(pv.count, 1u) == pv.nprobe - 1u ? 1u : 0u;
+  }
+  __syncthreads();
+  if (!last_wg) return;
+  __threadfence();
+  const unsigned call = __hip_atomic_load(level, __ATOMIC_RELAXED, __HIP_MEMORY_SCOPE_AGENT);
+  bool any_quiet = false, any_wide = false;
+  for (int i0 = 0; i0 < M; i0 += 64 * kProbeObjects) {
+    const int i = i0 + (int)threadIdx.x;
+    bool quiet = false;
+    if (i < M) {
+      const unsigned lv = __hip_atomic_load(obj_level + i, __ATOMIC_RELAXED, __HIP_MEMORY_SCOPE_AGENT);
+      const unsigned lo = __hip_atomic_load(obj_level + cap + i, __ATOMIC_RELAXED, __HIP_MEMORY_SCOPE_AGENT);
+      quiet = level_is_quiet(lv, call);
+      any_wide |= lo != 0u && call != 0u && (int)(lo >> 23) < (int)(call >> 23) - kPlainBinades;
+    }
+    const unsigned long long bits = __ballot(quiet);
+    if (lane == 0 && i < M) pv.quiet_obj[i >> 5] = (unsigned)bits, pv.quiet_obj[(i >> 5) + 1] = (unsigned)(bits >> 32);
+    any_quiet |= quiet;
+  }
+  const int q = __syncthreads_or(any_quiet ? 1 : 0), wd = __syncthreads_or(any_wide ? 1 : 0);
+  if (threadIdx.x == 0) {
+    *pv.quiet_any = q ? 1u : 0u;
+    if (pv.wide && wd) atomicOr(pv.wide, 1u);
+    *pv.count = 0u;
+  }
 }
 
 constexpr int kHingeSpreadBinades = 16;
@@ -207,13 +255,19 @@
   const unsigned *level = nullptr;
   unsigned *wide = nullptr;
 };
+constexpr int kPrepGroupList = 64;
+struct PrepGroups {
+  int n = 0;
+  int g[kPrepGroupList];
+};
 template <int kPrepRun>
 static __global__ void __launch_bounds__(256)
 k_seg_prep(PointStore ps, int M, int ntiles, int tile_samples, int64_t t_call, int64_t t_call_end,
-           SegDesc *desc, QuietMark qm, unsigned *tile_slow = nullptr) {
+           SegDesc *desc, QuietMark qm, unsigned *tile_slow = nullptr, PrepGroups groups = PrepGroups()) {
   __shared__ SegDesc sh[16 * kPrepRun][17];
   const int ti = threadIdx.x & 15, oi = threadIdx.x >> 4;
-  const int tile0 = (blockIdx.x * 16 + ti) * kPrepRun, m = blockIdx.y * 16 + oi;
+  const int by = groups.n ? groups.g[blockIdx.y] : (int)blockIdx.y;
+  const int tile0 = (blockIdx.x * 16 + ti) * kPrepRun, m = by * 16 + oi;
   bool quiet = false;
   if (qm.obj_level && m < M) {
     const unsigned call = *qm.level, lv = qm.obj_level[m], lo = qm.obj_level[qm.cap + m];
@@ -247,7 +301,7 @@
 #pragma unroll
   for (int j = 0; j < kPrepRun; j++) {
     const int to = (threadIdx.x >> 4) + 16 * j, oo = threadIdx.x & 15;
-    const int tile_o = blockIdx.x * 16 * kPrepRun + to, m_o = blockIdx.y * 16 + oo;
+    const int tile_o = blockIdx.x * 16 * kPrepRun + to, m_o = by * 16 + oo;
     if (tile_o < ntiles && m_o < M) desc[(size_t)tile_o * M + m_o] = sh[to][oo];
   }
 }
```

Result: no change. 1.155 million (-0.1%).
